# rvignav/diffusion-tts

Measured on AMD Instinct MI355X. Metric: candidate U-Net steps/sec, EDM ImageNet-64 eps-greedy N=64, higher is better.
Workload: dtype f16x3; 1 GPU; EDM ImageNet-64 (ADM 295.9M) eps-greedy search iteration, imagenet scorer, sigma step 5/18; candidates_total=64, candidates_per_gpu=64, scorer=imagenet, scorer_dtype=f16x3, denoiser_dtype=f16x3, graph_replay=True, parity_grade=True, parallelism=candidates sharded x1, 1 all-gather of rewards per step

## Files before the change

### diffusion_tts_amd/_lib.py

```python
import ctypes as C
import os

import torch

_HERE = os.path.dirname(os.path.abspath(__file__))
LIB_PATH = os.environ.get('DTS_LIB_PATH') or os.path.join(_HERE, 'libdts_hip.so')

DTS_F32, DTS_BF16, DTS_F16, DTS_F16X3 = 0, 1, 2, 3

_p, _i, _f, _d, _i64 = C.c_void_p, C.c_int, C.c_float, C.c_double, C.c_int64


class ConvArgs(C.Structure):
    _fields_ = [('x1', _p), ('c1', C.c_int32), ('x2', _p), ('c2', C.c_int32), ('w', _p), ('bias', _p),
                ('bias_nc', _p), ('ld_bias_nc', C.c_int32), ('residual', _p), ('out', _p),
                ('n', C.c_int32), ('hin', C.c_int32), ('win', C.c_int32), ('cout', C.c_int32),
                ('ksize', C.c_int32), ('up', C.c_int32), ('out_scale', C.c_float), ('dtype', C.c_int32),
                ('workspace', _p), ('workspace_bytes', C.c_int64), ('stats_out', _p), ('stats_written', C.c_int32),
                ('ev_start', _p), ('ev_stop', _p), ('gn_coef', _p), ('gn_silu', C.c_int32), ('acc_scale', C.c_float), ('out_split2', C.c_int32),
                ('skip_c', C.c_int32), ('skip_x', _p), ('skip_w', _p), ('skip_acc_scale', C.c_float), ('skip_up', C.c_int32)]


class ConvPlanInfo(C.Structure):
    _fields_ = [(f, C.c_int32) for f in ('kernel', 'tile', 'waves', 'stages', 'pf', 'gn', 'sk', 'dbg', 'splits', 'ks_per_split', 'n_ct', 'n_pt', 'nblk',
                                         'threads', 'lds_bytes', 'stats_in_kernel', 'stats_in_reduce', 'stats_written', 'epi_rows', 'fuses_gn',
                                         'folds_skip', 'refused', 'phases')]


SIGNATURES = {
    'dts_nchw_to_nhwc': [_p, _p, _i, _i, _i, _i, _i, _p],
    'dts_nhwc_to_nchw': [_p, _i, _p, _i, _i, _i, _i, _p],
    'dts_nchw_to_nhwc_pad': [_p, _p, _i, _i, _i, _i, _i, _i, _p],
    'dts_pack_conv_weight': [_p, _p, _i, _i, _i, _i, _i, _p, _p],
    'dts_conv2d': [C.POINTER(ConvArgs), _p],
    'dts_conv_in3': [_p, _p, _p, _p, _i, _i, _i, _i, _i, _p],
    'dts_conv_out3': [_p, _i, _p, _p, _p, _i, _i, _i, _i, _p],
    'dts_gn_coef': [_p, _i, _p, _i, _i, _i, _i, _i, _f, _p, _p, _p, _i, _p, _p, _p],
    'dts_gn_coef_strips': [_p, _i, _p, _i, _i, _i, _i, _i, _f, _p, _p, _p, _i, _p, _p],
    'dts_gn_apply': [_p, _i, _p, _i, _i, _p, _p, _i, _i, _i, _i, _i, _p],
    'dts_gn_apply_x3': [_p, _i, _p, _i, _p, _p, _p, _i, _i, _i, _i, _i, _p],
    'dts_gn_fused': [_p, _i, _p, _i, _i, _i, _i, _i, _f, _p, _p, _p, _i, _p, _i, _p],
    'dts_resample2x': [_p, _p, _i, _i, _i, _i, _i, _i, _p],
    'dts_resample_fir': [_p, _p, _i, _i, _i, _i, _i, _i, _i, _p],
    'dts_space_to_depth2': [_p, _i, _p, _i, _i, _i, _i, _i, _i, _i, _p],
    'dts_attention': [_p, _p, _i, _i, _i, _i, _i, _f, _p],
    'dts_attention_masked': [_p, _p, _i, _i, _i, _i, _i, _f, _i, _p, _p],
    'dts_cross_attention': [_p, _p, _p, _i, _p, _i, _i, _i, _i, _i, _i, _f, _p],
    'dts_layer_norm': [_p, _p, _i, _i64, _i, _f, _p, _p, _p],
    'dts_geglu': [_p, _p, _i, _i64, _i, _p],
    'dts_group_rows': [_p, _i, _i64, _p, _p, _p, _p, _p],
    'dts_patchify': [_p, _p, _i, _i, _i, _i, _i, _p],
    'dts_vit_tokens': [_p, _p, _p, _p, _i, _i, _i, _i, _p],
    'dts_text_tokens': [_p, _p, _p, _p, _i, _i, _i, _i, _i, _p],
    'dts_gelu': [_p, _p, _i, _i64, _i, _p],
    'dts_vit_head': [_p, _p, _i, _i, _i, _i, _f, _p, _p, _p],
    'dts_layer_norm_x3': [_p, _p, _p, _i64, _i, _f, _p, _p, _p],
    'dts_gelu_x3': [_p, _p, _i64, _i, _i, _p],
    'dts_patchify_x3': [_p, _p, _i, _i, _i, _i, _p],
    'dts_vit_tokens_f32': [_p, _p, _p, _p, _i, _i, _i, _p],
    'dts_vit_head_f32': [_p, _p, _i, _i, _i, _f, _p, _p, _p],
    'dts_linear': [_p, _i, _p, _p, _p, _i, _i, _i, _i, _i, _i, _i, _p],
    'dts_pos_embedding': [_p, _p, _p, _i, _i, _i, _p],
    'dts_edm_precond_in': [_p, _p, _i, _f, _p, _p, _i, _i, _p],
    'dts_edm_precond_out': [_p, _p, _p, _p, _i, _i, _p],
    'dts_split3_f16': [_p, _i, _p, _i, _p, _i64, _p],
    'dts_split2_f16': [_p, _i, _p, _i64, _p],
    'dts_attention_x3': [_p, _p, _i, _i, _i, _i, _i, _f, _p],
    'dts_cast_from_f32': [_p, _p, _i, _i64, _p],
    'dts_cast_to_f32': [_p, _i, _p, _i64, _p],
    'dts_heun_xhat': [_p, _i, _i, _p, _i, _d, _p, _i, _i, _p],
    'dts_heun_euler': [_p, _p, _d, _d, _p, _p, _i64, _p],
    'dts_heun_correct': [_p, _p, _p, _d, _d, _p, _i64, _p],
    'dts_quantize_u8': [_p, _i, _p, _i64, _p],
    'dts_brightness': [_p, _p, _i, _i, _p],
    'dts_u8_to_unit_f32': [_p, _p, _i64, _p],
    'dts_resample_u8': [_p, _p, _i, _i, _i, _i, _i, _p, _p, _i, _p],
    'dts_lut_u8_f32': [_p, _p, _p, _i, _i, _i, _p],
    'dts_jpeg_size': [_p, _p, _i, _i, _i, _p, _p, _i64, _p, _p],
    'dts_cosine_rows': [_p, _p, _i, _p, _i, _i, _p],
    'dts_attnpool_tokens': [_p, _p, _p, _i, _i, _i, _i, _p],
    'dts_take_token': [_p, _i, _p, _i, _i, _i, _i, _p],
    'dts_softmax_gather': [_p, _p, _p, _i, _i, _p],
    'dts_candidate_noise': [_p, _p, _p, _p, _p, _i, _i, _i, _p],
    'dts_candidate_noise_sd': [_p, _p, _p, _p, _p, _i, _i, _i64, _p],
    'dts_cfg_combine': [_p, _p, _f, _p, _i, _i64, _p],
    'dts_ddim_candidates': [_p, _p, _p, _p, _p, _i, _f, _f, _f, _i, _i64, _p],
}
OTHER = {'dts_version': ([], _i), 'dts_conv_fuses_gn': ([C.POINTER(ConvArgs)], _i), 'dts_conv_kernel': ([C.POINTER(ConvArgs)], _i), 'dts_conv_folds_skip': ([C.POINTER(ConvArgs)], _i), 'dts_conv_takes_phases': ([C.POINTER(ConvArgs)], _i), 'dts_conv_plan': ([C.POINTER(ConvArgs), C.POINTER(ConvPlanInfo)], _i), 'dts_set_tuning': ([_i, _i], _i), 'dts_get_tuning': ([_i], _i), 'dts_last_error': ([], C.c_char_p), 'dts_gn_ws_floats': ([_i, _i], _i64),
         'dts_jpeg_workspace_bytes': ([_i, _i, _i], _i64)}

_lib = None
ABI_VERSION = 120


def load():
    global _lib
    if _lib is not None:
        return _lib
    if not os.path.exists(LIB_PATH):
        raise RuntimeError(f'{LIB_PATH} not found: the HIP extension is required (no CPU fallback). '
                           f'Build it with `python -m diffusion_tts_amd.build` or __graft_entry__.build().')
    lib = C.CDLL(LIB_PATH)
    for name, argt in SIGNATURES.items():
        fn = getattr(lib, name)
        fn.argtypes, fn.restype = argt, _i
    for name, (argt, rest) in OTHER.items():
        fn = getattr(lib, name)
        fn.argtypes, fn.restype = argt, rest
    got = lib.dts_version()
    if got != ABI_VERSION or C.sizeof(ConvArgs) != 208:
        raise RuntimeError(f'{LIB_PATH} has ABI version {got}, this binding needs {ABI_VERSION}: rebuild with `python -m diffusion_tts_amd.build --force`')
    _lib = lib
    return lib


def check(status, what=''):
    if status != 0:
        msg = load().dts_last_error().decode(errors='replace')
        raise RuntimeError(f'libdts_hip {what} failed ({status}): {msg}')


KNOBS = {'att_xcd': 0, 'att_qt': 1, 'conv_tile': 2, 'conv_splits': 3, 'conv_variant': 4, 'gn_fuse': 5, 'att_db': 6, 'conv_stages': 7, 'conv_waves': 8, 'conv_half_round': 9, 'conv_epi32': 10, 'conv_skip_fold': 11, 'conv_up_phases': 12}


def set_tuning(name, value):
    check(load().dts_set_tuning(KNOBS[name], int(value)), 'dts_set_tuning')
```

### diffusion_tts_amd/classifier.py

```python
import math
from typing import Dict

import torch

from . import ops
from .config import ClassifierConfig, ClsLayer, classifier_layers


def _qkv_perm_legacy(heads: int, d: int) -> torch.Tensor:
    s, h, c = torch.meshgrid(torch.arange(3), torch.arange(heads), torch.arange(d), indexing='ij')
    return (h * 3 * d + s * d + c).reshape(-1).to(torch.int32)


class _P:
    pass


class EncoderUNetModel:
    def __init__(self, cfg: ClassifierConfig, state_dict: Dict[str, torch.Tensor], device='cuda', dtype=ops.F16X3):
        if not torch.cuda.is_available():
            raise RuntimeError('EncoderUNetModel (HIP) needs a GPU: there is no CPU fallback in this package')
        self.cfg, self.device, self.dtype = cfg, torch.device(device), dtype
        self.act_dtype = ops.act_dtype(dtype)
        self.x3 = dtype == ops.F16X3
        from .graphs import GraphCache
        self._graphs = GraphCache(self._device_forward)
        f = lambda t: t.detach().to(self.device, torch.float32).contiguous()
        sd, dt = state_dict, dtype
        mc = cfg.model_channels
        half = mc // 2
        self.freqs = torch.exp(-math.log(10000) * torch.arange(0, half, dtype=torch.float32) / half).to(self.device)
        self.te0_w, self.te0_b = f(sd['time_embed.0.weight']), f(sd['time_embed.0.bias'])
        self.te2_w, self.te2_b = f(sd['time_embed.2.weight']), f(sd['time_embed.2.bias'])
        self.layers, self.ch, self.res = classifier_layers(cfg)
        self.params: Dict[str, _P] = {}
        emb_w, emb_b, off = [], [], 0
        hc = cfg.num_head_channels
        for L in self.layers:
            P, p = _P(), L.prefix
            if L.kind == 'conv_in':
                P.w, P.b = f(sd[f'{p}.weight']), f(sd[f'{p}.bias'])
            elif L.kind == 'res':
                P.g0, P.b0 = f(sd[f'{p}.in_layers.0.weight']), f(sd[f'{p}.in_layers.0.bias'])
                P.w0, P.cb0 = ops.pack_conv_weight(f(sd[f'{p}.in_layers.2.weight']), dt), f(sd[f'{p}.in_layers.2.bias'])
                emb_w.append(sd[f'{p}.emb_layers.1.weight'])
                emb_b.append(sd[f'{p}.emb_layers.1.bias'])
                P.off, off = off, off + 2 * L.cout
                P.g1, P.b1 = f(sd[f'{p}.out_layers.0.weight']), f(sd[f'{p}.out_layers.0.bias'])
                P.w1, P.cb1 = ops.pack_conv_weight(f(sd[f'{p}.out_layers.3.weight']), dt), f(sd[f'{p}.out_layers.3.bias'])
                P.sw = P.sb = None
                if L.cin != L.cout:
                    P.sw, P.sb = ops.pack_conv_weight(f(sd[f'{p}.skip_connection.weight']), dt), f(sd[f'{p}.skip_connection.bias'])
                    P.cb1_skip = (P.cb1 + P.sb).contiguous()
            else:
                heads = L.cin // hc
                perm = _qkv_perm_legacy(heads, hc).to(self.device)
                P.g, P.b = f(sd[f'{p}.norm.weight']), f(sd[f'{p}.norm.bias'])
                P.wqkv = ops.pack_conv_weight(f(sd[f'{p}.qkv.weight']), dt, out_perm=perm)
                P.bqkv = f(sd[f'{p}.qkv.bias'])[perm.long()].contiguous()
                P.wproj, P.bproj = ops.pack_conv_weight(f(sd[f'{p}.proj_out.weight']), dt), f(sd[f'{p}.proj_out.bias'])
                P.heads = heads
            self.params[p] = P
        self.emb_w = ops.pack_conv_weight(f(torch.cat(emb_w, 0))[:, :, None, None].contiguous(), dt)
        self.emb_b = f(torch.cat(emb_b, 0))
        self.emb_total = off
        self.out_g, self.out_b = f(sd['out.0.weight']), f(sd['out.0.bias'])
        self.pos = f(sd['out.2.positional_embedding'])
        self.pool_wqkv = ops.pack_conv_weight(f(sd['out.2.qkv_proj.weight']), dt)
        self.pool_bqkv = f(sd['out.2.qkv_proj.bias'])
        self.cproj_w = f(sd['out.2.c_proj.weight']).reshape(cfg.out_channels, self.ch).contiguous()
        self.cproj_b = f(sd['out.2.c_proj.bias'])
        torch.cuda.synchronize(self.device)

    def _res(self, L: ClsLayer, x, emb_all):
        P = self.params[L.prefix]
        raw = self.x3 and P.sw is not None
        h = ops.group_norm(x, 32, 1e-5, P.g0, P.b0, silu=True, pool=L.down, split_out=self.x3, raw_split=raw)
        if raw:
            h, x = h
        elif L.down:
            x = ops.resample2x(x, up=False)
        h = ops.conv2d(h, P.w0, P.cb0, gn_stats=True)
        ss = emb_all[:, P.off:P.off + 2 * L.cout]
        h = ops.group_norm(h, 32, 1e-5, P.g1, P.b1, scale_shift=ss, silu=True, split_out=self.x3)
        if raw and ops.conv_folds_skip(h, P.w1, (x, P.sw, False)):
            return ops.conv2d(h, P.w1, P.cb1_skip, skip=(x, P.sw, False), gn_stats=True)
        sk = x if P.sw is None else ops.conv2d(x, P.sw, P.sb)
        return ops.conv2d(h, P.w1, P.cb1, residual=sk, gn_stats=True)

    def _attn(self, L: ClsLayer, x):
        P = self.params[L.prefix]
        n, hh, ww, c = x.shape
        hn = ops.group_norm(x, 32, 1e-5, P.g, P.b, silu=False, split_out=self.x3)
        fx3 = self.x3 and ops.attention_x3_ok(hh * ww, c // P.heads)
        qkv = ops.conv2d(hn, P.wqkv, P.bqkv, out_split2=fx3)
        a = ops.attention(qkv.view(n, hh * ww, 3 * c), P.heads, 1.0 / math.sqrt(c // P.heads), x3=self.x3, split_out=fx3)
        a = ops.SplitAct(a.data.view(n, hh, ww, 2 * c), c) if fx3 else a.view(n, hh, ww, c)
        return ops.conv2d(a, P.wproj, P.bproj, residual=x, gn_stats=True)

    @torch.no_grad()
    def __call__(self, x, timesteps):
        t = timesteps.to(self.device, torch.float32).contiguous()
        return self._graphs(x.to(self.device, torch.float32).contiguous(), t)

    @torch.no_grad()
    def _device_forward(self, x, t):
        n = x.shape[0]
        emb = ops.pos_embedding(t, self.freqs)
        emb = ops.linear(emb, self.te0_w, self.te0_b, act_out=True)
        emb = ops.linear(emb, self.te2_w, self.te2_b, act_out=True)
        e = ops.cast_from_f32(emb, self.act_dtype)
        emb_all = ops.conv2d(e.view(1, n, 1, -1), self.emb_w, self.emb_b).view(n, self.emb_total)
        h = None
        for L in self.layers:
            if L.kind == 'conv_in':
                P = self.params[L.prefix]
                h = ops.conv_in3(x.contiguous(), P.w, P.b, L.cout, self.act_dtype)
            elif L.kind == 'res':
                h = self._res(L, h, emb_all)
            else:
                h = self._attn(L, h)
        h = ops.group_norm(h, 32, 1e-5, self.out_g, self.out_b, silu=True)
        tok = ops.attnpool_tokens(h, self.pos)
        nt = tok.shape[1]
        qkv = ops.conv2d(tok.view(n, nt, 1, self.ch), self.pool_wqkv, self.pool_bqkv)
        heads = self.ch // self.cfg.num_head_channels
        a = ops.attention(qkv.view(n, nt, 3 * self.ch), heads, 1.0 / math.sqrt(self.cfg.num_head_channels), x3=self.x3)
        return ops.linear(ops.take_token(a, 0), self.cproj_w, self.cproj_b)
```

### diffusion_tts_amd/csrc/conv_igemm.hip

```cpp
#include "dts_common.h"
#include <hip/hip_ext.h>
#include <type_traits>

static_assert(sizeof(dts_conv_args) == 208, "dts_conv_args layout changed: bump DTS_ABI_VERSION and update the bindings (_lib.py ConvArgs)");

int dts_conv_launch_phase_form(const void* plan, const void* params, const void* call);

namespace {

struct ConvCall {
  hipStream_t st;
  hipEvent_t ev_start = nullptr, ev_stop = nullptr;
};

struct ConvP {
  const char* x1; const char* x2;
  const char* w;
  const float* bias;
  const char* bias_nc;
  const char* residual;
  char* out;
  int c1, c2, cin;
  int ld_bias_nc;
  int n, hin, win, hout, wout, cout;
  int taps;
  int up;
  int P;
  int n_ct;
  int n_pt;
  int splits;
  int ks_per_split;
  float* partial;
  float* stats;
  float out_scale;
  float acc_scale;
  int out_split2;
  int w_shift, hw_shift;
  const float* gn_coef;
  int gn_silu;
  int epi_rows;
  const char* sk_x; const char* sk_w;
  int sk_c, sk_up;
  float sk_ratio;
};

template <typename T> struct Mma;
template <> struct Mma<bf16_t> {
  static __device__ __forceinline__ void run(f32x4_t& acc, const uint4& a, const uint4& b) {
    acc = __builtin_amdgcn_mfma_f32_16x16x32_bf16(__builtin_bit_cast(bf16x8_t, a), __builtin_bit_cast(bf16x8_t, b), acc, 0, 0, 0);
  }
};
template <> struct Mma<f16_t> {
  static __device__ __forceinline__ void run(f32x4_t& acc, const uint4& a, const uint4& b) {
    acc = __builtin_amdgcn_mfma_f32_16x16x32_f16(__builtin_bit_cast(f16x8_t, a), __builtin_bit_cast(f16x8_t, b), acc, 0, 0, 0);
  }
};
template <> struct Mma<float> {
  static __device__ __forceinline__ void run(f32x4_t& acc, const uint4& a, const uint4& b) {
    acc = __builtin_amdgcn_mfma_f32_16x16x4f32(__builtin_bit_cast(float, a.x), __builtin_bit_cast(float, b.x), acc, 0, 0, 0);
    acc = __builtin_amdgcn_mfma_f32_16x16x4f32(__builtin_bit_cast(float, a.y), __builtin_bit_cast(float, b.y), acc, 0, 0, 0);
    acc = __builtin_amdgcn_mfma_f32_16x16x4f32(__builtin_bit_cast(float, a.z), __builtin_bit_cast(float, b.z), acc, 0, 0, 0);
    acc = __builtin_amdgcn_mfma_f32_16x16x4f32(__builtin_bit_cast(float, a.w), __builtin_bit_cast(float, b.w), acc, 0, 0, 0);
  }
};

__device__ __forceinline__ uint4 f16x8_mul_2m11(const uint4& v) {
  const f16x8_t h = __builtin_bit_cast(f16x8_t, v) * (_Float16)0x1p-11f;
  return __builtin_bit_cast(uint4, h);
}

template <typename T> struct Vec4;
template <> struct Vec4<float> {
  using type = float4;
  static __device__ __forceinline__ void unpack(const float4& v, float* f) { f[0] = v.x; f[1] = v.y; f[2] = v.z; f[3] = v.w; }
  static __device__ __forceinline__ float4 pack(const float* f) { return make_float4(f[0], f[1], f[2], f[3]); }
  static __device__ __forceinline__ void load(const float* p, float* f) {
    const float4 v = *reinterpret_cast<const float4*>(p);
    f[0] = v.x; f[1] = v.y; f[2] = v.z; f[3] = v.w;
  }
  static __device__ __forceinline__ void store(float* p, const float* f) {
    *reinterpret_cast<float4*>(p) = make_float4(f[0], f[1], f[2], f[3]);
  }
};
template <> struct Vec4<bf16_t> {
  using type = uint2;
  static __device__ __forceinline__ uint2 pack(const float* f) {
    return make_uint2(pack2_bf16(f[0], f[1]), pack2_bf16(f[2], f[3]));
  }
  static __device__ __forceinline__ void unpack(const uint2& v, float* f) {
    f[0] = __builtin_bit_cast(float, v.x << 16); f[1] = __builtin_bit_cast(float, v.x & 0xffff0000u);
    f[2] = __builtin_bit_cast(float, v.y << 16); f[3] = __builtin_bit_cast(float, v.y & 0xffff0000u);
  }
  static __device__ __forceinline__ void load(const bf16_t* p, float* f) {
    const uint2 v = *reinterpret_cast<const uint2*>(p);
    f[0] = bf16_bits_to_f32(v.x & 0xffffu); f[1] = bf16_bits_to_f32(v.x >> 16);
    f[2] = bf16_bits_to_f32(v.y & 0xffffu); f[3] = bf16_bits_to_f32(v.y >> 16);
  }
  static __device__ __forceinline__ void store(bf16_t* p, const float* f) {
    *reinterpret_cast<uint2*>(p) = make_uint2(pack2_bf16(f[0], f[1]), pack2_bf16(f[2], f[3]));
  }
};
template <> struct Vec4<f16_t> {
  using type = uint2;
  static __device__ __forceinline__ uint2 pack(const float* f) {
    return make_uint2(pack2_f16(f[0], f[1]), pack2_f16(f[2], f[3]));
  }
  static __device__ __forceinline__ void unpack(const uint2& v, float* f) {
    f[0] = f16_bits_to_f32(v.x & 0xffffu); f[1] = f16_bits_to_f32(v.x >> 16);
    f[2] = f16_bits_to_f32(v.y & 0xffffu); f[3] = f16_bits_to_f32(v.y >> 16);
  }
  static __device__ __forceinline__ void load(const f16_t* p, float* f) {
    const uint2 v = *reinterpret_cast<const uint2*>(p);
    f[0] = f16_bits_to_f32(v.x & 0xffffu); f[1] = f16_bits_to_f32(v.x >> 16);
    f[2] = f16_bits_to_f32(v.y & 0xffffu); f[3] = f16_bits_to_f32(v.y >> 16);
  }
  static __device__ __forceinline__ void store(f16_t* p, const float* f) {
    *reinterpret_cast<uint2*>(p) = make_uint2(pack2_f16(f[0], f[1]), pack2_f16(f[2], f[3]));
  }
};

#ifdef DTS_STAMPS
__device__ unsigned long long g_stamps[8192 * 8];
#define DTS_STAMP(slot_)                                                                                       \
  if (threadIdx.x == 0 && (blockIdx.x + blockIdx.y * gridDim.x) < 8192) {                                       \
    unsigned long long t_;                                                                                      \
    asm volatile("s_memtime %0\n\ts_waitcnt lgkmcnt(0)" : "=s"(t_)::"memory");                                 \
    g_stamps[(blockIdx.x + blockIdx.y * gridDim.x) * 8 + (slot_)] = t_;                                         \
  }
#define DTS_STAMP_RT(slot_)                                                                                    \
  if (threadIdx.x == 0 && (blockIdx.x + blockIdx.y * gridDim.x) < 8192) {                                       \
    unsigned long long t_;                                                                                      \
    asm volatile("s_memrealtime %0\n\ts_waitcnt lgkmcnt(0)" : "=s"(t_)::"memory");                             \
    g_stamps[(blockIdx.x + blockIdx.y * gridDim.x) * 8 + (slot_)] = t_;                                         \
  }
#define DTS_SEG_DECL unsigned long long seg_t_ = 0, seg_acc_[6] = {0, 0, 0, 0, 0, 0};
#define DTS_SEG_START { asm volatile("s_memtime %0\n\ts_waitcnt lgkmcnt(0)" : "=s"(seg_t_)::"memory"); }
#define DTS_SEG_MARK(i_)                                                                                       \
  {                                                                                                            \
    __builtin_amdgcn_sched_barrier(0);                                                                         \
    unsigned long long n_;                                                                                     \
    asm volatile("s_memtime %0\n\ts_waitcnt lgkmcnt(0)" : "=s"(n_)::"memory");                                \
    seg_acc_[i_] += n_ - seg_t_;                                                                               \
    seg_t_ = n_;                                                                                               \
    __builtin_amdgcn_sched_barrier(0);                                                                         \
  }
#define DTS_SEG_STORE                                                                                          \
  if ((threadIdx.x & 255) == 0 && (blockIdx.x + blockIdx.y * gridDim.x) < 4096) {                              \
    unsigned long long* d_ = g_seg + ((blockIdx.x + blockIdx.y * gridDim.x) * 2 + (threadIdx.x >> 8)) * 8;     \
    for (int i_ = 0; i_ < 6; ++i_) d_[i_] = seg_acc_[i_];                                                      \
  }
__device__ unsigned long long g_seg[4096 * 2 * 8];
#else
#define DTS_STAMP(slot_)
#define DTS_STAMP_RT(slot_)
#define DTS_SEG_DECL
#define DTS_SEG_START
#define DTS_SEG_MARK(i_)
#define DTS_SEG_STORE
#endif

__device__ uint4 g_zero16[2048];

__device__ __forceinline__ void glds16(const char* g, uint32_t lds_off) {
  asm volatile("s_mov_b32 m0, %1\n\ts_nop 0\n\tglobal_load_lds_dwordx4 %0, off" : : "v"(g), "s"(lds_off) : "memory", "m0");
}

typedef int dts_i32x4 __attribute__((ext_vector_type(4)));
__device__ __forceinline__ dts_i32x4 make_rsrc(const void* base, uint32_t bytes) {
  const uint64_t a = (uint64_t)(uintptr_t)base;
  return dts_i32x4{(int)(uint32_t)a, (int)(uint32_t)(a >> 32), (int)bytes, 0x00020000};
}
__device__ __forceinline__ void bdma16(uint32_t voff, dts_i32x4 rsrc, uint32_t soff, uint32_t lds_off) {
  asm volatile("s_mov_b32 m0, %3\n\ts_nop 0\n\tbuffer_load_dwordx4 %0, %1, %2 offen lds"
               : : "v"(voff), "s"(rsrc), "s"(soff), "s"(lds_off) : "memory", "m0");
}
#ifndef PP_LOAD_ORDER
#define PP_LOAD_ORDER 2
#endif
constexpr uint32_t DTS_OOR = 0x80000000u;

__device__ __forceinline__ int swz(int row, int chunk) { return row * 128 + ((chunk ^ (row & 7)) << 4); }

struct TileMap {
  int pn0;
  int patch;
  int porg;
  int w;
  int strip0;
  __device__ __forceinline__ int pix(int r) const { return patch ? porg + (r >> 4) * w + (r & 15) : pn0 + r; }
  __device__ __forceinline__ int strip(int wn) const { return strip0 + wn; }
};
__device__ __forceinline__ TileMap linear_tile(int pn0) { return TileMap{pn0, 0, 0, 0, pn0 >> 6}; }

struct PhaseTileMap {
  int pn0;
  int py, px;
// ... 12 lines not shown
      y = rem / lw; x = rem - y * lw;
    }
    return n * 4 * lhw + (2 * y + py) * 2 * lw + 2 * x + px;
  }
  __device__ __forceinline__ int strip(int wn) const {
    const int S = lhw >> 6, gs = (pn0 >> 6) + wn, n = gs / S;
    return n * 4 * S + (2 * py + px) * S + (gs - n * S);
  }
};

template <int BM, int NTHR>
__device__ __forceinline__ void issue_residual_pieces(const ConvP& kp, int cm0, const TileMap& tm, uint32_t stage, int tid, int u0, int u1) {
  constexpr int CPR = BM / 8;
  const char* resb = kp.residual + (size_t)cm0 * 2;
  const size_t rstride = (size_t)kp.cout * 2;
  const uint32_t wave_dst = __builtin_amdgcn_readfirstlane(stage + (tid >> 6) * 1024);
  for (int u = u0; u < u1; ++u) {
    const int slot = u * NTHR + tid, row = slot / CPR, c = slot - row * CPR;
    glds16(resb + (size_t)tm.pix(row) * rstride + ((c ^ (row & 7)) << 4), wave_dst + u * (NTHR * 16));
  }
}

__device__ __forceinline__ float row16_sum(float v) {
  v += __builtin_bit_cast(float, __builtin_amdgcn_update_dpp(0, __builtin_bit_cast(int, v), 0xB1, 0xf, 0xf, false));
  v += __builtin_bit_cast(float, __builtin_amdgcn_update_dpp(0, __builtin_bit_cast(int, v), 0x4E, 0xf, 0xf, false));
  v += __builtin_bit_cast(float, __builtin_amdgcn_update_dpp(0, __builtin_bit_cast(int, v), 0x141, 0xf, 0xf, false));
  v += __builtin_bit_cast(float, __builtin_amdgcn_update_dpp(0, __builtin_bit_cast(int, v), 0x140, 0xf, 0xf, false));
  return v;
}
__device__ __forceinline__ void row16_sum8(float (&a)[4], float (&b)[4]) {
#define DTS_DPP_STEP(ctrl_)                                                                     \
  "v_add_f32_dpp %0, %0, %0 " ctrl_ " row_mask:0xf bank_mask:0xf\n\t"                           \
  "v_add_f32_dpp %1, %1, %1 " ctrl_ " row_mask:0xf bank_mask:0xf\n\t"                           \
  "v_add_f32_dpp %2, %2, %2 " ctrl_ " row_mask:0xf bank_mask:0xf\n\t"                           \
  "v_add_f32_dpp %3, %3, %3 " ctrl_ " row_mask:0xf bank_mask:0xf\n\t"                           \
  "v_add_f32_dpp %4, %4, %4 " ctrl_ " row_mask:0xf bank_mask:0xf\n\t"                           \
  "v_add_f32_dpp %5, %5, %5 " ctrl_ " row_mask:0xf bank_mask:0xf\n\t"                           \
  "v_add_f32_dpp %6, %6, %6 " ctrl_ " row_mask:0xf bank_mask:0xf\n\t"                           \
  "v_add_f32_dpp %7, %7, %7 " ctrl_ " row_mask:0xf bank_mask:0xf\n\t"
  asm volatile("s_nop 1\n\t"
               DTS_DPP_STEP("quad_perm:[1,0,3,2]") DTS_DPP_STEP("quad_perm:[2,3,0,1]") DTS_DPP_STEP("row_half_mirror") DTS_DPP_STEP("row_mirror")
               : "+v"(a[0]), "+v"(a[1]), "+v"(a[2]), "+v"(a[3]), "+v"(b[0]), "+v"(b[1]), "+v"(b[2]), "+v"(b[3]));
#undef DTS_DPP_STEP
}

template <typename T, int MT, int NT, int BM, int BN, bool RES, bool BNC, bool STATS, int NTHR>
__device__ __forceinline__ void conv_epilogue_fast(const ConvP& kp, f32x4_t (&acc)[MT][NT], int cm0, const TileMap& tm, int wm, int wn, int lrow,
                                                   int lq, char* smem_ring, bool bias_in_acc, int stage_off, int early_u0,
                                                   int early_u1) {
  char* smem = smem_ring + stage_off;
  using V4 = typename Vec4<T>::type;
  constexpr int ROWB = BM * 2, CPR = BM / 8, DR = NTHR / CPR, DC = NTHR - DR * CPR, ITERS = BN * CPR / NTHR;
  static_assert(BN * CPR % NTHR == 0 && CPR % 8 == 0, "staged tile trips / swizzle groups");
  const int p_cout = kp.cout;
  const int prow0 = wn * 16 * NT + lrow;
  const int col0 = wm * 16 * MT + lq * 4;
  const T* __restrict__ bnc = reinterpret_cast<const T*>(kp.bias_nc);
  const size_t rstride = (size_t)p_cout * 2;
  const int tid = threadIdx.x;
  if constexpr (RES) {
    const uint32_t stage = (uint32_t)(uintptr_t)(__attribute__((address_space(3))) char*)smem;
    issue_residual_pieces<BM, NTHR>(kp, cm0, tm, stage, tid, 0, early_u0);
    issue_residual_pieces<BM, NTHR>(kp, cm0, tm, stage, tid, early_u1, ITERS);
  }
  float4 bv[MT];
#pragma unroll
  for (int mt = 0; mt < MT; ++mt) bv[mt] = make_float4(0.f, 0.f, 0.f, 0.f);
  (void)bias_in_acc; (void)bv;
  const T* np[NT];
  if constexpr (BNC) {
    const int hw = kp.hout * kp.wout;
#pragma unroll
    for (int nt = 0; nt < NT; ++nt) {
      const int pp = tm.pix(prow0 + nt * 16);
      np[nt] = bnc + (size_t)(kp.hw_shift >= 0 ? pp >> kp.hw_shift : pp / hw) * kp.ld_bias_nc + cm0 + col0;
    }
  }
  constexpr bool want_stats = STATS && NT == 4;
  float* sp = want_stats ? kp.stats + ((size_t)tm.strip(wn) * p_cout + cm0 + col0) * 2 : nullptr;
  char* sw = smem + prow0 * ROWB + (lq & 1) * 8;
  int coff[MT];
#pragma unroll
  for (int mt = 0; mt < MT; ++mt) coff[mt] = (((wm * 2 * MT + 2 * mt + (lq >> 1)) ^ (lrow & 7)) << 4);
  const float osc = kp.out_scale;
  if constexpr (RES) {
    if (early_u0 > 0 || early_u1 < ITERS) {
      asm volatile("s_waitcnt vmcnt(0)" ::: "memory");
      __syncthreads();
    }
  }
#pragma unroll
  for (int mt = 0; mt < MT; ++mt) {
    V4 nv[NT], rv[NT];
    if constexpr (BNC) {
#pragma unroll
      for (int nt = 0; nt < NT; ++nt) nv[nt] = *reinterpret_cast<const V4*>(np[nt] + mt * 16);
    }
    if constexpr (RES) {
#pragma unroll
      for (int nt = 0; nt < NT; ++nt) rv[nt] = *reinterpret_cast<const V4*>(sw + nt * 16 * ROWB + coff[mt]);
    }
    typedef float f32x2 __attribute__((ext_vector_type(2)));
    f32x2 ssa = {0.f, 0.f}, ssb = {0.f, 0.f}, sqa = {0.f, 0.f}, sqb = {0.f, 0.f};
#pragma unroll
    for (int nt = 0; nt < NT; ++nt) {
      f32x2 va = {acc[mt][nt][0], acc[mt][nt][1]}, vb = {acc[mt][nt][2], acc[mt][nt][3]};
      if constexpr (BNC) {
        float f[4];
        Vec4<T>::unpack(nv[nt], f);
        va += f32x2{f[0], f[1]}; vb += f32x2{f[2], f[3]};
      }
      if constexpr (RES) {
        float f[4];
        Vec4<T>::unpack(rv[nt], f);
        va += f32x2{f[0], f[1]}; vb += f32x2{f[2], f[3]};
      }
      va *= osc; vb *= osc;
      const float v[4] = {va.x, va.y, vb.x, vb.y};
      const V4 pk = Vec4<T>::pack(v);
      *reinterpret_cast<V4*>(sw + nt * 16 * ROWB + coff[mt]) = pk;
      if constexpr (want_stats) {
        float f[4];
        Vec4<T>::unpack(pk, f);
        const f32x2 fa = {f[0], f[1]}, fb = {f[2], f[3]};
        ssa += fa; ssb += fb;
        sqa = __builtin_elementwise_fma(fa, fa, sqa); sqb = __builtin_elementwise_fma(fb, fb, sqb);
      }
    }
    if constexpr (want_stats) {
      float ss4[4] = {ssa.x, ssa.y, ssb.x, ssb.y}, sq4[4] = {sqa.x, sqa.y, sqb.x, sqb.y};
      row16_sum8(ss4, sq4);
      if (lrow == 0) {
        float4* d = reinterpret_cast<float4*>(sp + mt * 32);
        d[0] = make_float4(ss4[0], sq4[0], ss4[1], sq4[1]);
        d[1] = make_float4(ss4[2], sq4[2], ss4[3], sq4[3]);
      }
    }
  }
  DTS_STAMP(6);
  __syncthreads();
  DTS_STAMP(7);
  int row = tid / CPR, c = tid - row * CPR;
  char* outb = kp.out + (size_t)cm0 * 2;
  typedef unsigned int u32x4_nt __attribute__((ext_vector_type(4)));
#pragma unroll
  for (int u = 0; u < ITERS; ++u) {
    const u32x4_nt v_ = *reinterpret_cast<const u32x4_nt*>(smem + row * ROWB + c * 16);
    __builtin_nontemporal_store(v_, reinterpret_cast<u32x4_nt*>(outb + (size_t)tm.pix(row) * rstride + ((c ^ (row & 7)) << 4)));
    row += DR; c += DC;
    if (c >= CPR) { c -= CPR; ++row; }
  }
}

template <int MT, int NT, typename TM = TileMap>
__device__ __forceinline__ void conv_epilogue_rows_f32(const ConvP& kp, f32x4_t (&acc)[MT][NT], int cm0, const TM& tm, int wm, int wn,
                                                       int lrow, int lq, char* smem, int wave) {
  static_assert(NT == 4, "64-pixel wave strips");
  constexpr int CW = 16 * MT;
  constexpr int LPR = 4 * MT;
  constexpr int RPI = LPR <= 8 ? 8 : (LPR <= 16 ? 4 : 2);
  constexpr int ITERS = 32 / RPI;
  constexpr int ROWB = CW * 4 + 16;
  char* const ws = smem + (size_t)wave * (32 * ROWB);
  const int lane = threadIdx.x & 63;
  const int rsub = lane / LPR, c4 = lane - rsub * LPR;
  const bool act = rsub < RPI;
  const int p_cout = kp.cout;
  const int co = cm0 + wm * CW + c4 * 4;
  const float* __restrict__ res = reinterpret_cast<const float*>(kp.residual);
  if (tm.pix(wn * 64) >= kp.P) return;
  float4 b4 = make_float4(0.f, 0.f, 0.f, 0.f), n4 = make_float4(0.f, 0.f, 0.f, 0.f);
  if (act) {
    if (kp.bias) b4 = *reinterpret_cast<const float4*>(kp.bias + co);
    if (kp.bias_nc) {
      const int pp0 = tm.pix(wn * 64), hw = kp.hout * kp.wout;
      n4 = *reinterpret_cast<const float4*>(reinterpret_cast<const float*>(kp.bias_nc) + (size_t)(kp.hw_shift >= 0 ? pp0 >> kp.hw_shift : pp0 / hw) * kp.ld_bias_nc + co);
    }
  }
  const float asc = kp.acc_scale, osc = kp.out_scale;
  const bool want_stats = kp.stats != nullptr;
  float ss4[4] = {0.f, 0.f, 0.f, 0.f}, sq4[4] = {0.f, 0.f, 0.f, 0.f};
  typedef float f32x4_nt __attribute__((ext_vector_type(4)));
  constexpr int CH = ITERS < 8 ? ITERS : 8;
#pragma unroll
  for (int half = 0; half < 2; ++half) {
#pragma unroll
    for (int n2 = 0; n2 < 2; ++n2)
#pragma unroll
      for (int mt = 0; mt < MT; ++mt)
        *reinterpret_cast<f32x4_t*>(ws + (n2 * 16 + lrow) * ROWB + (mt * 16 + lq * 4) * 4) = acc[mt][half * 2 + n2];
#pragma unroll
   for (int u0 = 0; u0 < ITERS; u0 += CH) {
    size_t prow[CH];
    float4 rv[CH];
#pragma unroll
    for (int u = 0; u < CH; ++u) {
      prow[u] = (size_t)tm.pix(wn * 64 + half * 32 + (u0 + u) * RPI + (act ? rsub : 0)) * p_cout + co;
      rv[u] = make_float4(0.f, 0.f, 0.f, 0.f);
      if (res && act) rv[u] = *reinterpret_cast<const float4*>(res + prow[u]);
    }
#pragma unroll
    for (int u = 0; u < CH; ++u) {
      if (!act) continue;
      const f32x4_t a = *reinterpret_cast<const f32x4_t*>(ws + ((u0 + u) * RPI + rsub) * ROWB + c4 * 16);
      float v[4] = {a[0] * asc + b4.x, a[1] * asc + b4.y, a[2] * asc + b4.z, a[3] * asc + b4.w};
      if (kp.bias_nc) { v[0] += n4.x; v[1] += n4.y; v[2] += n4.z; v[3] += n4.w; }
      if (res) { v[0] += rv[u].x; v[1] += rv[u].y; v[2] += rv[u].z; v[3] += rv[u].w; }
#pragma unroll
      for (int r = 0; r < 4; ++r) v[r] *= osc;
      if (kp.out_split2) {
        float hi[4], lo[4];
#pragma unroll
        for (int r = 0; r < 4; ++r) x2_split(v[r], hi[r], lo[r]);
        const uint2 h = make_uint2(pack2_f16(hi[0], hi[1]), pack2_f16(hi[2], hi[3])), l = make_uint2(pack2_f16(lo[0], lo[1]), pack2_f16(lo[2], lo[3]));
        const bool odd = (c4 & 1) != 0;
        const uint32_t rx = (uint32_t)__builtin_amdgcn_update_dpp(0, (int)(odd ? h.x : l.x), 0xB1, 0xf, 0xf, false);
        const uint32_t ry = (uint32_t)__builtin_amdgcn_update_dpp(0, (int)(odd ? h.y : l.y), 0xB1, 0xf, 0xf, false);
        if (kp.epi_rows == 2) {
          f16_t* o8 = reinterpret_cast<f16_t*>(kp.out) + 2 * (prow[u] - co) + co;
          *reinterpret_cast<uint2*>(o8) = h;
          *reinterpret_cast<uint2*>(o8 + p_cout) = l;
          continue;
        }
        f16_t* orow = reinterpret_cast<f16_t*>(kp.out) + 2 * (prow[u] - co) + (odd ? co - 4 + p_cout : co);
        *reinterpret_cast<uint4*>(orow) = odd ? make_uint4(rx, ry, l.x, l.y) : make_uint4(h.x, h.y, rx, ry);
      } else {
        const f32x4_nt o = {v[0], v[1], v[2], v[3]};
        __builtin_nontemporal_store(o, reinterpret_cast<f32x4_nt*>(reinterpret_cast<float*>(kp.out) + prow[u]));
      }
      if (want_stats) {
#pragma unroll
        for (int r = 0; r < 4; ++r) { ss4[r] += v[r]; sq4[r] += v[r] * v[r]; }
      }
    }
   }
  }
  if (want_stats) {
#pragma unroll
    for (int r = 0; r < 4; ++r) {
      float s_ = ss4[r], q_ = sq4[r];
#pragma unroll
      for (int k = 1; k < RPI; ++k) { s_ += __shfl(ss4[r], c4 + k * LPR, 64); q_ += __shfl(sq4[r], c4 + k * LPR, 64); }
      ss4[r] = s_; sq4[r] = q_;
    }
    if (rsub == 0) {
      float4* d = reinterpret_cast<float4*>(kp.stats + ((size_t)tm.strip(wn) * p_cout + co) * 2);
      d[0] = make_float4(ss4[0], sq4[0], ss4[1], sq4[1]);
      d[1] = make_float4(ss4[2], sq4[2], ss4[3], sq4[3]);
    }
  }
}

template <typename T, int MT, int NT, int BM, int BN, int NTHR, int RING, typename TM = TileMap>
__device__ __forceinline__ void conv_epilogue(const ConvP& kp, f32x4_t (&acc)[MT][NT], int cm0, const TM& tm, int split, int wm, int wn,
                                              int lrow, int lq, char* smem, bool bias_in_acc, int stage_off, int early_u0, int early_u1) {
  const int p_P = kp.P, p_cout = kp.cout, p_hout = kp.hout, p_wout = kp.wout;
  if (kp.splits > 1) {
    float* part = kp.partial + (size_t)split * p_P * p_cout;
#pragma unroll
    for (int nt = 0; nt < NT; ++nt) {
      const int pp = tm.pix(wn * 16 * NT + nt * 16 + lrow);
      if (pp >= p_P) continue;
#pragma unroll
      for (int mt = 0; mt < MT; ++mt) {
        const int co = cm0 + wm * 16 * MT + mt * 16 + lq * 4;
        *reinterpret_cast<float4*>(part + (size_t)pp * p_cout + co) =
            make_float4(acc[mt][nt][0], acc[mt][nt][1], acc[mt][nt][2], acc[mt][nt][3]);
      }
    }
    return;
  }
  if constexpr (sizeof(T) == 4 && NT == 4) {
    constexpr int NWV = NTHR / 64;
    static_assert(NWV * 32 * (16 * MT * 4 + 16) <= RING, "the waves' private transpose slices must fit the caller's LDS ring");
    if (kp.epi_rows && (p_hout * p_wout) % 64 == 0) {
      conv_epilogue_rows_f32<MT, NT>(kp, acc, cm0, tm, wm, wn, lrow, lq, smem, (int)(threadIdx.x >> 6));
      return;
    }
  }
  if constexpr (sizeof(T) == 2) {
    if (tm.pn0 + BN <= p_P) {
      const bool r_ = kp.residual != nullptr, b_ = kp.bias_nc != nullptr, s_ = NT == 4 && kp.stats != nullptr;
#define DTS_EPI(R_, B_, S_) conv_epilogue_fast<T, MT, NT, BM, BN, R_, B_, S_, NTHR>(kp, acc, cm0, tm, wm, wn, lrow, lq, smem, bias_in_acc, stage_off, early_u0, early_u1)
      if (r_) { if (b_) { if (s_) DTS_EPI(true, true, true); else DTS_EPI(true, true, false); }
                else    { if (s_) DTS_EPI(true, false, true); else DTS_EPI(true, false, false); } }
      else    { if (b_) { if (s_) DTS_EPI(false, true, true); else DTS_EPI(false, true, false); }
                else    { if (s_) DTS_EPI(false, false, true); else DTS_EPI(false, false, false); } }
#undef DTS_EPI
      return;
    }
  }
  const T* __restrict__ res = reinterpret_cast<const T*>(kp.residual);
  const T* __restrict__ bnc = reinterpret_cast<const T*>(kp.bias_nc);
  T* __restrict__ out = reinterpret_cast<T*>(kp.out);
  const int hw = p_hout * p_wout;
  using V4 = typename Vec4<T>::type;
  int ppv[NT], nsv[NT];
#pragma unroll
  for (int nt = 0; nt < NT; ++nt) {
    const int pp = tm.pix(wn * 16 * NT + nt * 16 + lrow);
    ppv[nt] = pp < p_P ? pp : -1;
    nsv[nt] = pp < p_P ? pp / hw : 0;
  }
  constexpr int RG = (sizeof(T) == 4 && MT > 4) ? 2 : MT;
  static_assert(MT % RG == 0, "residual slice groups");
  V4 rv[RG][NT], nv[NT];
  float4 bv[MT];
#pragma unroll
  for (int mt = 0; mt < MT; ++mt)
    bv[mt] = (kp.bias && !bias_in_acc) ? *reinterpret_cast<const float4*>(kp.bias + cm0 + wm * 16 * MT + mt * 16 + lq * 4) : make_float4(0.f, 0.f, 0.f, 0.f);
  const float asc = kp.acc_scale;
  constexpr bool VIA_LDS = sizeof(T) == 2;
  constexpr int ROWP = BM * 2 + 16;
  static_assert(!VIA_LDS || BN * ROWP <= RING, "staged tile must fit the caller's LDS ring");
  const bool want_stats = NT == 4 && kp.stats != nullptr;
  float* sp = want_stats ? kp.stats + ((size_t)tm.strip(wn) * p_cout) * 2 : nullptr;
#pragma unroll
  for (int mt = 0; mt < MT; ++mt) {
    const int co = cm0 + wm * 16 * MT + mt * 16 + lq * 4;
    const float4 bcur = bv[mt];
    if (res && mt % RG == 0) {
#pragma unroll
      for (int m2 = 0; m2 < RG; ++m2) {
        const int co_ = cm0 + wm * 16 * MT + (mt + m2) * 16 + lq * 4;
#pragma unroll
        for (int nt = 0; nt < NT; ++nt)
          if (ppv[nt] >= 0) rv[m2][nt] = *reinterpret_cast<const V4*>(res + (size_t)ppv[nt] * p_cout + co_);
      }
    }
    if (bnc) {
#pragma unroll
      for (int nt = 0; nt < NT; ++nt)
        if (ppv[nt] >= 0) nv[nt] = *reinterpret_cast<const V4*>(bnc + (size_t)nsv[nt] * kp.ld_bias_nc + co);
    }
    float ss4[4] = {0.f, 0.f, 0.f, 0.f}, sq4[4] = {0.f, 0.f, 0.f, 0.f};
#pragma unroll
    for (int nt = 0; nt < NT; ++nt) {
      if (ppv[nt] < 0) continue;
      float v[4];
      v[0] = acc[mt][nt][0] * asc + bcur.x; v[1] = acc[mt][nt][1] * asc + bcur.y;
      v[2] = acc[mt][nt][2] * asc + bcur.z; v[3] = acc[mt][nt][3] * asc + bcur.w;
      if (bnc) {
        float f[4];
        Vec4<T>::unpack(nv[nt], f);
#pragma unroll
        for (int r = 0; r < 4; ++r) v[r] += f[r];
      }
      if (res) {
        float f[4];
        Vec4<T>::unpack(rv[mt % RG][nt], f);
#pragma unroll
        for (int r = 0; r < 4; ++r) v[r] += f[r];
      }
#pragma unroll
      for (int r = 0; r < 4; ++r) v[r] *= kp.out_scale;
      const V4 pk = Vec4<T>::pack(v);
      if constexpr (VIA_LDS)
        *reinterpret_cast<V4*>(smem + (wn * 16 * NT + nt * 16 + lrow) * ROWP + (wm * 16 * MT + mt * 16 + lq * 4) * 2) = pk;
      else if (sizeof(T) == 4 && kp.out_split2) {
        float hi[4], lo[4];
#pragma unroll
        for (int r = 0; r < 4; ++r) x2_split(v[r], hi[r], lo[r]);
        f16_t* orow = reinterpret_cast<f16_t*>(kp.out) + (size_t)ppv[nt] * 2 * p_cout + co;
        *reinterpret_cast<uint2*>(orow) = make_uint2(pack2_f16(hi[0], hi[1]), pack2_f16(hi[2], hi[3]));
        *reinterpret_cast<uint2*>(orow + p_cout) = make_uint2(pack2_f16(lo[0], lo[1]), pack2_f16(lo[2], lo[3]));
      } else
        *reinterpret_cast<V4*>(out + (size_t)ppv[nt] * p_cout + co) = pk;
      if (want_stats) {
        float f[4];
        Vec4<T>::unpack(pk, f);
#pragma unroll
        for (int r = 0; r < 4; ++r) { ss4[r] += f[r]; sq4[r] += f[r] * f[r]; }
      }
    }
    if (want_stats) {
#pragma unroll
      for (int r = 0; r < 4; ++r) {
#pragma unroll
        for (int o = 1; o < 16; o <<= 1) { ss4[r] += __shfl_xor(ss4[r], o, 64); sq4[r] += __shfl_xor(sq4[r], o, 64); }
      }
      if (lrow == 0 && tm.pix(wn * 64) < p_P) {
        float4* d = reinterpret_cast<float4*>(sp + (size_t)co * 2);
        d[0] = make_float4(ss4[0], sq4[0], ss4[1], sq4[1]);
        d[1] = make_float4(ss4[2], sq4[2], ss4[3], sq4[3]);
      }
    }
  }
  if constexpr (VIA_LDS) {
// ... 838 lines not shown
  const int dev = current_device();
  if (!attr_done[dev]) {
    (void)hipFuncSetAttribute(reinterpret_cast<const void*>(KERNEL), hipFuncAttributeMaxDynamicSharedMemorySize, pl.lds_bytes);
    attr_done[dev] = true;
  }
  const dim3 grid(pl.nblk, pl.splits), block(pl.threads);
  if (call.ev_start != nullptr && call.ev_stop != nullptr)
    hipExtLaunchKernelGGL(KERNEL, grid, block, (size_t)pl.lds_bytes, call.st, call.ev_start, call.ev_stop, 0, q);
  else
    hipLaunchKernelGGL(KERNEL, grid, block, (size_t)pl.lds_bytes, call.st, q);
  DTS_CHECK_LAUNCH(pl.kernel != 0 ? "dts_conv2d(ping-pong)" : "dts_conv2d");
  return DTS_OK;
}

template <typename T, typename OT, int MT, int WM, int WN, bool PF, bool PH = false>
int conv_launch_igemm(const ConvPlan& pl, const ConvP& q, const ConvCall& call) {
#define DTS_IGEMM(MT_, WM_, STAGES_) conv_launch<&conv_igemm_kernel<T, MT_, 4, WM_, WN, PF, STAGES_, OT, PH>>(pl, q, call)
  if constexpr (sizeof(T) == 2) {
    if (pl.waves == 8) return pl.stages == 3 ? DTS_IGEMM(MT / 2, WM * 2, 3) : DTS_IGEMM(MT / 2, WM * 2, 2);
    if (pl.stages == 3) return DTS_IGEMM(MT, WM, 3);
    if constexpr (std::is_same<T, OT>::value)
      if (pl.stages == 4) return DTS_IGEMM(MT, WM, 4);
  }
  return DTS_IGEMM(MT, WM, 2);
#undef DTS_IGEMM
}

int igemm_splits(int nblk, int nk, double slab, bool can8, bool x3, bool ws, long long ws_bytes, int forced) {
  const int slots = 512;
  int splits = 1;
  if (ws && nblk < (slots * 3) / 4 && nk >= 16) {
    int smax = 8;
    if (smax > nk / 8) smax = nk / 8;
    while (smax > 1 && (long long)smax * (long long)slab > ws_bytes) --smax;
    if (smax < 1) smax = 1;
    const double KS = x3 ? 1.5 : 1.0;
    auto est = [&](int s_) {
      const int steps = (nk + s_ - 1) / s_;
      double t;
      if (can8 && (long long)nblk * s_ <= 256) t = 5.0 + steps * 0.75 * KS;
      else t = (double)((nblk * s_ + slots - 1) / slots) * (5.5 + steps * 1.25 * KS);
      if (s_ > 1) t += 3.0 + (s_ + 0.5) * slab / 4.0e6;
      return t;
    };
    int best = 1;
    for (int s_ = 2; s_ <= smax; ++s_)
      if (est(s_) < est(best)) best = s_;
    splits = best;
  }
  const int f8 = forced > 8 ? 8 : forced;
  if (f8 > 0 && ws && nk >= 2 * f8 && (long long)f8 * (long long)slab <= ws_bytes) splits = f8;
  return splits;
}

inline bool pp_considers_split(long long nblk) { return nblk < 192; }

int pp_splits(int nblk, int nk, double slab, bool x3, bool ws, long long ws_bytes, int forced) {
  int splits = 1;
  if (!ws || nk < 16) return splits;
  if (forced > 0) splits = forced;
  else if (pp_considers_split(nblk)) {
    const int nchunk = nk / 9;
    double best = 1e30;
    for (int s_ = 1; s_ <= 8 && s_ <= nchunk; ++s_) {
      const int cps = (nchunk + s_ - 1) / s_, se = (nchunk + cps - 1) / cps;
      if (se != s_ || nblk * se > 256) continue;
      double t = 5.0 + cps * 9 * (x3 ? 1.4 : 1.05);
      if (se > 1) t += 3.0 + (se + 0.5) * slab / 4.0e6;
      if (t < best) { best = t; splits = se; }
    }
  }
  if (splits > 8) splits = 8;
  if (forced > 0 && splits > nk / 8) splits = nk / 8;
  if (splits > nk / 9) splits = nk / 9;
  while (splits > 1 && (long long)splits * (long long)slab > ws_bytes) --splits;
  if (splits < 1) splits = 1;
  return splits;
}

bool conv_pp_eligible(int dtype, int ksize, int cout, int c1, int c2, int n, int hin, int win, int up) {
  const int ho = up ? 2 * hin : hin, wo = up ? 2 * win : win;
  const long long P = (long long)n * ho * wo;
  return dtype != DTS_F32 && cout % 192 == 0 && ho == wo && wo >= 16 && (wo & (wo - 1)) == 0 && P % 256 == 0 && P < (1ll << 30) &&
         (long long)n * hin * win * (c1 > c2 ? c1 : c2) * 2 < (1ll << 31) && (long long)cout * ksize * ksize * (c1 + c2) * 2 < (1ll << 31) &&
         (c1 % 64 == 0) && (c2 % 64 == 0);
}

int conv_pick_pp(const ConvKnobs& k, bool f32, const ConvP& p, bool x3) {
  if (f32 || k.variant == 0 || k.tile > 0) return 0;
  if (p.taps != 9) return 0;
  const int mt = p.cout % 192 == 0 ? 6 : (p.cout % 128 == 0 ? 4 : 0);
  if (mt == 0 || !conv_pp_eligible(DTS_BF16, 3, 192, p.c1, p.c2, p.n, p.hin, p.win, p.up)) return 0;
  if ((long long)p.cout * p.taps * p.cin * 2 >= (1ll << 31)) return 0;
  if (p.gn_coef != nullptr) return (mt == 6 && !p.up) ? 6 : 0;
  if (k.variant >= 1) return mt;
  const long long blocks_pp = (long long)(p.cout / (32 * mt)) * ((p.P + 255) / 256);
  const bool short_small = blocks_pp <= 128 && p.taps * (p.cin / 64) <= 27;
  const bool half_round_128 = mt == 4 && blocks_pp > 64 && blocks_pp <= 128 && p.wout >= 32 && p.cout <= 256 && (x3 ? k.half_round == 1 : k.half_round != 0);
  const bool auto_pp = !short_small && !half_round_128;
  return (auto_pp && blocks_pp >= 64) ? mt : 0;
}

int conv_pp_dbg(int variant) {
  if (variant <= 1) return 0;
#ifdef DTS_DIAG_KERNELS
  const int d = variant / 10;
  return (variant % 10 == 1 && d >= 1 && d <= 9 && d != 3) ? d : 0;
#else
  return -1;
#endif
}

template <typename T, typename OT = T>
int conv_launch_plan(const ConvPlan& pl, const ConvP& q, const ConvCall& call) {
  if constexpr (sizeof(T) == 2) {
#define DTS_PP(DBG_, GN_, MT_, SK_) conv_launch<&conv_pp_kernel<T, 9, DBG_, GN_, MT_, OT, SK_>>(pl, q, call)
    if constexpr (!std::is_same<T, OT>::value) {
      if (pl.phases) return dts_conv_launch_phase_form(&pl, &q, &call);
      if (pl.kernel == 6 && pl.sk) return DTS_PP(0, false, 6, true);
      if (pl.kernel == 4 && pl.sk) return DTS_PP(0, false, 4, true);
    } else if (pl.kernel == 6) {
      if (pl.gn) return DTS_PP(0, true, 6, false);
#ifdef DTS_DIAG_KERNELS
      switch (pl.dbg) {
        case 1: return DTS_PP(1, false, 6, false);
        case 2: return DTS_PP(2, false, 6, false);
        case 4: return DTS_PP(4, false, 6, false);
        case 5: return DTS_PP(5, false, 6, false);
        case 6: return DTS_PP(6, false, 6, false);
        case 7: return DTS_PP(7, false, 6, false);
        case 8: return DTS_PP(8, false, 6, false);
        case 9: return DTS_PP(9, false, 6, false);
      }
#endif
    }
    if (pl.kernel == 6) return DTS_PP(0, false, 6, false);
    if (pl.kernel == 4) return DTS_PP(0, false, 4, false);
#undef DTS_PP
  }
  switch (pl.tile) {
    case 192: return pl.pf ? conv_launch_igemm<T, OT, 6, 2, 2, true>(pl, q, call) : conv_launch_igemm<T, OT, 6, 2, 2, false>(pl, q, call);
    case 128: return pl.pf ? conv_launch_igemm<T, OT, 4, 2, 2, true>(pl, q, call) : conv_launch_igemm<T, OT, 4, 2, 2, false>(pl, q, call);
    default: return pl.pf ? conv_launch_igemm<T, OT, 4, 1, 4, true>(pl, q, call) : conv_launch_igemm<T, OT, 4, 1, 4, false>(pl, q, call);
  }
}

void conv_shape_from_args(const dts_conv_args* a, ConvP& p) {
  p.c1 = a->c1; p.c2 = a->c2; p.cin = a->c1 + a->c2;
  p.n = a->n; p.hin = a->hin; p.win = a->win;
  p.hout = a->up ? 2 * a->hin : a->hin; p.wout = a->up ? 2 * a->win : a->win;
  p.cout = a->cout; p.taps = a->ksize * a->ksize; p.up = a->up;
  p.P = (int)((long long)p.n * p.hout * p.wout);
  p.residual = (const char*)a->residual; p.gn_coef = a->gn_coef;
  p.out_split2 = a->out_split2;
}

ConvPlan conv_plan(const dts_conv_args* a) {
  ConvPlan pl{};
  pl.kernel = -1; pl.splits = 1;
  auto refuse = [&](const char* fmt, int v0 = 0, int v1 = 0, int v2 = 0) { pl.refused = 1; snprintf(pl.refuse, sizeof(pl.refuse), fmt, v0, v1, v2); return pl; };
  if (a == nullptr) return refuse("dts_conv2d: null args");
  const ConvKnobs k = conv_knobs();
  const bool f32 = a->dtype == DTS_F32, x3 = a->dtype == DTS_F16X3;
  pl.fuses_gn = a->ksize == 3 && k.variant != 0 && k.tile <= 0 && !a->up &&
                conv_pp_eligible(a->dtype, a->ksize, a->cout, a->c1, a->c2, a->n, a->hin, a->win, a->up) &&
                (k.variant == 1 || (long long)(a->cout / 192) * (((long long)a->n * a->hin * a->win + 255) / 256) >= 64);
  if (a->ksize != 1 && a->ksize != 3) return refuse("dts_conv2d: ksize %d", a->ksize);
  if (a->n <= 0 || a->hin <= 0 || a->win <= 0) return refuse("dts_conv2d: bad shape");
  if (a->cout <= 0) return refuse("dts_conv2d: cout %d must be a multiple of 64", a->cout);
  if ((long long)a->n * a->hin * a->win * (a->up ? 4 : 1) >= (1ll << 30)) return refuse("dts_conv2d: too many pixels");
  ConvP p;
  conv_shape_from_args(a, p);
  const bool ph = a->up == 2;
  if (ph) p.taps = 4;
  const int mt = ph ? 0 : conv_pick_pp(k, f32, p, x3);
  pl.kernel = mt;
  int unit = 1;
  if (mt != 0) {
    pl.n_ct = p.cout / (32 * mt); pl.n_pt = (p.P + 255) / 256;
    pl.threads = 512;
    pl.lds_bytes = (6 * 16 * mt + 2 * 328) * 128;
    unit = 9;
  } else {
    pl.tile = (p.cout % 192 == 0) ? 192 : (p.cout % 128 == 0 ? 128 : 64);
    if (f32 && pl.tile == 192 && !k.f32_tile192) pl.tile = (p.cout % 128 == 0) ? 128 : 64;
    if (k.tile > 0 && p.cout % k.tile == 0) pl.tile = (k.tile == 192 || k.tile == 128) ? k.tile : 64;
    pl.n_ct = p.cout / pl.tile; pl.n_pt = (p.P + (pl.tile == 64 ? 255 : 127)) / (pl.tile == 64 ? 256 : 128);
    if (ph) pl.n_pt = (p.P / 4 + 127) / 128;
    pl.pf = a->ksize == 3 && !f32;
  }
  pl.nblk = pl.n_ct * pl.n_pt * (ph ? 4 : 1);
  const int bke = f32 ? 32 : 64, nk = p.taps * (p.cin / bke);
  pl.gn = a->gn_coef != nullptr;
  {
    const int su = a->skip_up ? 1 : 0;
    pl.folds_skip = x3 && mt != 0 && !a->up && a->residual == nullptr && !a->out_split2 && a->gn_coef == nullptr &&
                    a->skip_c > 0 && a->skip_c % 64 == 0 && k.skip_fold != 0 && k.splits <= 0 && !(su && ((a->hin | a->win) & 1)) &&
                    (!pp_considers_split(pl.nblk) || k.variant == 1) &&
                    (long long)a->n * (a->hin >> su) * (a->win >> su) * a->skip_c * 2 < (1ll << 31) && (long long)a->cout * a->skip_c * 2 < (1ll << 31);
  }
  if (a->cout % 64 != 0) return refuse("dts_conv2d: cout %d must be a multiple of 64", a->cout);
  if (a->c1 <= 0 || a->c1 % bke != 0 || a->c2 % bke != 0) return refuse("dts_conv2d: channels (%d,%d) must be multiples of %d", a->c1, a->c2, bke);
  if ((long long)p.cin * (f32 ? 4 : 2) + 128 > (long long)sizeof(g_zero16))
    return refuse("dts_conv2d: %d input channels exceed the zero-row page (%d bytes)", p.cin, (int)sizeof(g_zero16));
  if (p.hout >= 32768 || p.wout >= 32768) return refuse("dts_conv2d: spatial size too large");
  if (a->out_split2 && !(x3 && a->stats_out == nullptr)) return refuse("dts_conv2d: out_split2 is the split-precision mode's, without strip statistics");
  if (a->acc_scale != 0.f && a->acc_scale != 1.f && !x3) return refuse("dts_conv2d: acc_scale is the split-precision mode's (DTS_F16X3)");
  if (pl.gn && !pl.fuses_gn) return refuse("dts_conv2d: gn_coef given for a launch that cannot fuse the GroupNorm apply (ask dts_conv_fuses_gn first)");
  if (a->skip_c != 0 || a->skip_w != nullptr || a->skip_x != nullptr) {
    if (a->skip_w == nullptr || a->skip_x == nullptr || !pl.folds_skip)
      return refuse("dts_conv2d: skip_* given for a launch that cannot fold the 1x1 skip convolution (ask dts_conv_folds_skip first)");
    pl.sk = true;
  }
  if (pl.gn && x3) return refuse("dts_conv2d: gn_coef is not available in the split-precision mode");
  if (a->dtype < DTS_F32 || a->dtype > DTS_F16X3) return refuse("bad dtype %d", a->dtype);
  if (ph) {
    if (!x3) return refuse("dts_conv2d: up = 2 (phase-packed weights) is the split-precision mode's (DTS_F16X3), dtype %d", a->dtype);
    if (a->ksize != 3) return refuse("dts_conv2d: up = 2 needs ksize 3, got %d", a->ksize);
    if (a->c2 != 0 || a->x2 != nullptr) return refuse("dts_conv2d: up = 2 takes no second input");
    if (a->gn_coef != nullptr || pl.sk || a->out_split2) return refuse("dts_conv2d: up = 2 takes no gn_coef, skip_* or out_split2");
    if (pl.tile == 64) return refuse("dts_conv2d: up = 2 needs cout %d to be a multiple of 128 or 192", a->cout);
    if (a->stats_out != nullptr && (a->hin * a->win) % 64 != 0)
      return refuse("dts_conv2d: up = 2 with strip statistics needs hin*win = %d to be a multiple of 64 (a wave's strip is 64 low-resolution pixels)", a->hin * a->win);
    if (k.up_phases == 0) return refuse("dts_conv2d: up = 2 while DTS_CONV_UP_PHASES=0");
  }
  if (mt == 6 && !x3 && !pl.gn) {
    pl.dbg = conv_pp_dbg(k.variant);
    if (pl.dbg < 0) return refuse("dts_conv2d: DTS_CONV_VARIANT=%d selects a diagnostic kernel that this library was built without (-DDTS_DIAG_KERNELS)", k.variant);
  }
  const bool ws = a->workspace != nullptr && !a->out_split2 && !pl.sk;
  const double slab = (double)p.P * p.cout * 4.0;
  pl.splits = mt != 0 ? pp_splits(pl.nblk, nk, slab, x3, ws, (long long)a->workspace_bytes, k.splits)
                      : igemm_splits(pl.nblk, nk, slab, !f32, x3, ws, (long long)a->workspace_bytes, k.splits);
  {
    const int nunit = nk / unit, per = (nunit + pl.splits - 1) / pl.splits;
    pl.ks_per_split = per * unit;
    pl.splits = (nunit + per - 1) / per;
  }
  if (ph) {
    if (pl.splits > 1) return refuse("dts_conv2d: up = 2 with a K split of %d (the phase form takes none: use the fused-gather route)", pl.splits);
    pl.phases = 1;
  }
  pl.stats_in_kernel = a->stats_out != nullptr && pl.splits == 1;
  pl.stats_in_reduce = a->stats_out != nullptr && pl.splits > 1 && (p.hout * p.wout) % 64 == 0 && p.cout % 4 == 0;
  pl.stats_written = pl.stats_in_kernel || pl.stats_in_reduce;
  pl.epi_rows = k.epi32 < 0 ? (x3 ? 1 : 0) : (k.epi32 == 2 ? 2 : (k.epi32 != 0));
  if (ph && (a->hin * a->win) % 64 != 0) pl.epi_rows = 0;
  if (mt != 0) return pl;
  const bool one_per_cu = (long long)pl.nblk * pl.splits <= 256;
  pl.stages = (one_per_cu && pl.ks_per_split >= 3) ? 3 : 2;
  if (k.stages >= 2 && k.stages <= 4) pl.stages = k.stages;
  if (f32) pl.stages = 2;
  const int stage_bytes = (pl.tile + (pl.tile == 64 ? 256 : 128)) * 128;
  if (pl.stages * stage_bytes > 160 * 1024) pl.stages = 3;
  pl.waves = (!f32 && (k.waves == 8 || (k.waves != 4 && one_per_cu))) ? 8 : 4;
  if (pl.stages == 4 && (pl.waves == 8 || x3)) pl.stages = 3;
  pl.threads = 64 * pl.waves;
  pl.lds_bytes = pl.stages * stage_bytes;
  return pl;
}

}

#ifdef DTS_CONV_PHASE_TU
int dts_conv_launch_phase_form(const void* plan, const void* params, const void* call) {
  const ConvPlan& pl = *static_cast<const ConvPlan*>(plan);
  const ConvP& q = *static_cast<const ConvP*>(params);
  const ConvCall& c = *static_cast<const ConvCall*>(call);
  return pl.tile == 192 ? conv_launch_igemm<f16_t, float, 6, 2, 2, true, true>(pl, q, c) : conv_launch_igemm<f16_t, float, 4, 2, 2, true, true>(pl, q, c);
}
#else

#ifdef DTS_STAMPS
extern "C" int dts_debug_read_stamps(unsigned long long* host, int count) {
  return (int)hipMemcpyFromSymbol(host, HIP_SYMBOL(g_stamps), sizeof(unsigned long long) * (size_t)count);
}
extern "C" int dts_debug_clear_stamps(void) {
  void* p = nullptr;
  if (hipGetSymbolAddress(&p, HIP_SYMBOL(g_stamps)) != hipSuccess) return -1;
  if (hipMemset(p, 0, sizeof(g_stamps)) != hipSuccess) return -1;
  if (hipGetSymbolAddress(&p, HIP_SYMBOL(g_seg)) != hipSuccess) return -1;
  return (int)hipMemset(p, 0, sizeof(g_seg));
}
extern "C" int dts_debug_read_segments(unsigned long long* host, int count) {
  return (int)hipMemcpyFromSymbol(host, HIP_SYMBOL(g_seg), sizeof(unsigned long long) * (size_t)count);
}
#endif

extern "C" int dts_conv_kernel(const dts_conv_args* a) { return conv_plan(a).kernel; }

extern "C" int dts_conv_fuses_gn(const dts_conv_args* a) { return conv_plan(a).fuses_gn ? 1 : 0; }

extern "C" int dts_conv_folds_skip(const dts_conv_args* a) { return conv_plan(a).folds_skip ? 1 : 0; }

extern "C" int dts_conv_takes_phases(const dts_conv_args* a) {
  if (a == nullptr || a->up != 2) return 0;
  const ConvPlan pl = conv_plan(a);
  return (!pl.refused && pl.phases) ? 1 : 0;
}

extern "C" int dts_conv_plan(const dts_conv_args* a, dts_conv_plan_info* out) {
  DTS_CHECK_ARG(out != nullptr, "dts_conv_plan: null output");
  const ConvPlan pl = conv_plan(a);
  *out = pl;
  if (pl.refused) dts_set_error("%s", pl.refuse);
  return pl.kernel < 0 ? DTS_ERR_ARG : DTS_OK;
}

extern "C" int dts_conv2d(dts_conv_args* a, dts_stream s) {
  const ConvPlan pl = conv_plan(a);
  DTS_CHECK_ARG(!pl.refused, "%s", pl.refuse);
  DTS_CHECK_ARG(a->x1 && a->w && a->out, "dts_conv2d: null tensor");
  DTS_CHECK_ARG(a->c2 == 0 || a->x2 != nullptr, "dts_conv2d: c2 without x2");
  DTS_CHECK_ARG(a->bias_nc == nullptr || a->ld_bias_nc >= a->cout, "dts_conv2d: ld_bias_nc");
  ConvP p;
  conv_shape_from_args(a, p);
  if (pl.phases) p.taps = 4;
  DTS_CHECK_ARG(a->stats_out == nullptr || ((p.hout * p.wout) % 64 == 0 && (uintptr_t)a->stats_out % 16 == 0),
                "dts_conv2d: strip statistics need hout*wout to be a multiple of 64 and a 16-byte aligned buffer");
  DTS_CHECK_ARG(a->workspace == nullptr || ((uintptr_t)a->workspace % 16 == 0 && a->workspace_bytes >= 0), "dts_conv2d: workspace");
  p.x1 = (const char*)a->x1; p.x2 = (const char*)a->x2; p.w = (const char*)a->w;
  p.bias = a->bias; p.bias_nc = (const char*)a->bias_nc; p.out = (char*)a->out;
  p.ld_bias_nc = a->ld_bias_nc;
  p.out_scale = a->out_scale; p.acc_scale = a->acc_scale == 0.f ? 1.f : a->acc_scale;
  p.w_shift = p.hw_shift = -1;
  {
    const int hw = p.hout * p.wout;
    if ((p.wout & (p.wout - 1)) == 0 && (hw & (hw - 1)) == 0) { p.w_shift = __builtin_ctz(p.wout); p.hw_shift = __builtin_ctz(hw); }
  }
  p.gn_silu = a->gn_silu;
  p.sk_x = p.sk_w = nullptr; p.sk_c = p.sk_up = 0; p.sk_ratio = 1.f;
  if (pl.sk) {
    const float ss = a->skip_acc_scale == 0.f ? 1.f : a->skip_acc_scale;
    p.sk_x = (const char*)a->skip_x; p.sk_w = (const char*)a->skip_w; p.sk_c = a->skip_c; p.sk_up = a->skip_up ? 1 : 0;
    p.sk_ratio = p.acc_scale / ss; p.acc_scale = ss;
  }
  p.n_ct = pl.n_ct; p.n_pt = pl.n_pt; p.splits = pl.splits; p.ks_per_split = pl.ks_per_split; p.epi_rows = pl.epi_rows;
  p.partial = (float*)a->workspace;
  p.stats = pl.stats_in_kernel ? a->stats_out : nullptr;
  ConvCall call;
  call.st = to_stream(s); call.ev_start = (hipEvent_t)a->ev_start; call.ev_stop = (hipEvent_t)a->ev_stop;
  int rc = DTS_OK;
  if (a->dtype == DTS_F16X3) rc = conv_launch_plan<f16_t, float>(pl, p, call);
  else DTS_DISPATCH_DTYPE(a->dtype, rc = conv_launch_plan<T>(pl, p, call));
  if (rc == DTS_OK && pl.splits > 1) {
    if (pl.stats_in_reduce) p.stats = a->stats_out;
    DTS_DISPATCH_DTYPE(a->dtype == DTS_F16X3 ? DTS_F32 : a->dtype, rc = launch_reduce<T>(p, pl.stats_in_reduce, call.st));
  }
  a->stats_written = pl.stats_written ? 1 : 0;
  return rc;
}
#endif
```

### diffusion_tts_amd/csrc/conv_small.hip

```cpp
#include "dts_common.h"
#include <type_traits>

namespace {

template <typename T>
__global__ __launch_bounds__(256) void conv_in3_kernel(const float* __restrict__ x, const float* __restrict__ w,
                                                        const float* __restrict__ bias, T* __restrict__ out, int n_total, int h,
                                                        int wd, int cout) {
  constexpr int EPV = ET<T>::EPV;
  extern __shared__ float sw[];
  for (int i = threadIdx.x; i < 27 * cout; i += blockDim.x) {
    const int co = i / 27, k = i - co * 27;
    sw[k * cout + co] = w[i];
  }
  for (int i = threadIdx.x; i < cout; i += blockDim.x) sw[27 * cout + i] = bias ? bias[i] : 0.f;
  __syncthreads();
  const int nchunk = cout / EPV;
  const long long npix = (long long)n_total * h * wd;
  constexpr int GRP = 8;
  char* stage = reinterpret_cast<char*>(sw + 28 * cout);
  for (long long pbase = (long long)blockIdx.x * 256; pbase < npix; pbase += (long long)gridDim.x * 256) {
    const long long pix0 = pbase + threadIdx.x;
    const bool live = pix0 < npix;
    long long pix = live ? pix0 : 0;
    const int xo = (int)(pix % wd); pix /= wd;
    const int yo = (int)(pix % h);
    const int n = (int)(pix / h);
    float in[27];
#pragma unroll
    for (int ci = 0; ci < 3; ++ci)
#pragma unroll
      for (int kh = 0; kh < 3; ++kh)
#pragma unroll
        for (int kw = 0; kw < 3; ++kw) {
          const int yy = yo + kh - 1, xx = xo + kw - 1;
          float v = 0.f;
          if (live && (unsigned)yy < (unsigned)h && (unsigned)xx < (unsigned)wd) v = x[(((size_t)n * 3 + ci) * h + yy) * wd + xx];
          in[ci * 9 + kh * 3 + kw] = v;
        }
    for (int c0 = 0; c0 < nchunk; c0 += GRP) {
      __syncthreads();
#pragma unroll
      for (int g = 0; g < GRP; ++g) {
        const int chunk = c0 + g;
        if (chunk >= nchunk) break;
        float acc[EPV];
#pragma unroll
        for (int e = 0; e < EPV; ++e) acc[e] = sw[27 * cout + chunk * EPV + e];
#pragma unroll
        for (int k = 0; k < 27; ++k) {
          const float* wr = sw + k * cout + chunk * EPV;
#pragma unroll
          for (int e = 0; e < EPV; ++e) acc[e] += in[k] * wr[e];
        }
        *reinterpret_cast<uint4*>(stage + threadIdx.x * (GRP * 16) + (((g + threadIdx.x) % GRP) << 4)) = pack16<T>(acc);
      }
      __syncthreads();
      const int ng = min(GRP, nchunk - c0);
      for (int t = threadIdx.x; t < 256 * ng; t += 256) {
        const int pl = t / ng, g = t - pl * ng;
        const long long pg = pbase + pl;
        if (pg < npix)
          *reinterpret_cast<uint4*>(out + (size_t)pg * cout + (size_t)(c0 + g) * EPV) =
              *reinterpret_cast<const uint4*>(stage + pl * (GRP * 16) + (((g + pl) % GRP) << 4));
      }
    }
  }
}

template <typename T, int NT>
__global__ __launch_bounds__(256) void conv_in3_mfma_kernel(const float* __restrict__ x, const float* __restrict__ w,
                                                             const float* __restrict__ bias, T* __restrict__ out, int nseg, int h,
                                                             int wd) {
  constexpr int ES = sizeof(T) == 4 ? 4 : 2;
  constexpr int COUT = NT * 16, ROWB = COUT * ES + 16, TG = 4;
  static_assert(NT % TG == 0, "tile groups");
  __shared__ __attribute__((aligned(16))) char stage_all[4 * 16 * ROWB];
  const int lane = threadIdx.x & 63, wave = threadIdx.x >> 6, p = lane & 15, kq = lane >> 4;
  char* stage = stage_all + wave * 16 * ROWB;
  float a[NT][7];
  int dci[7], dy[7], dx[7];
#pragma unroll
  for (int s = 0; s < 7; ++s) {
    const int k = 4 * s + kq;
    const int kk = k < 27 ? k : 0;
    dci[s] = k < 27 ? kk / 9 : -1;
    dy[s] = (kk % 9) / 3 - 1;
    dx[s] = kk % 3 - 1;
#pragma unroll
    for (int t = 0; t < NT; ++t) a[t][s] = k < 27 ? w[(16 * t + p) * 27 + k] : 0.f;
  }
  f32x4_t b0[NT];
#pragma unroll
  for (int t = 0; t < NT; ++t) {
    const float4 q = bias ? *reinterpret_cast<const float4*>(bias + 16 * t + 4 * kq) : make_float4(0.f, 0.f, 0.f, 0.f);
    b0[t][0] = q.x; b0[t][1] = q.y; b0[t][2] = q.z; b0[t][3] = q.w;
  }
  const int spr = wd >> 4;
  const size_t plane = (size_t)h * wd;
  for (int seg = blockIdx.x * 4 + wave; seg < nseg; seg += gridDim.x * 4) {
    const int xs = seg % spr, rest = seg / spr;
    const int y = rest % h, n = rest / h;
    float bv[7];
#pragma unroll
    for (int s = 0; s < 7; ++s) {
      const int yy = y + dy[s], xx = xs * 16 + p + dx[s];
      const bool ok = dci[s] >= 0 && (unsigned)yy < (unsigned)h && (unsigned)xx < (unsigned)wd;
      const size_t idx = ok ? ((size_t)n * 3 + dci[s]) * plane + (size_t)yy * wd + xx : 0;
      const float v = x[idx];
      bv[s] = ok ? v : 0.f;
    }
#pragma unroll
    for (int t0 = 0; t0 < NT; t0 += TG) {
      f32x4_t acc[TG];
#pragma unroll
      for (int u = 0; u < TG; ++u) acc[u] = b0[t0 + u];
#pragma unroll
      for (int s = 0; s < 7; ++s)
#pragma unroll
        for (int u = 0; u < TG; ++u) acc[u] = __builtin_amdgcn_mfma_f32_16x16x4f32(a[t0 + u][s], bv[s], acc[u], 0, 0, 0);
#pragma unroll
      for (int u = 0; u < TG; ++u) {
        if constexpr (std::is_same<T, float>::value) {
          *reinterpret_cast<f32x4_t*>(stage + p * ROWB + (16 * (t0 + u) + 4 * kq) * 4) = acc[u];
        } else {
          uint2 o;
          if (std::is_same<T, bf16_t>::value) { o.x = pack2_bf16(acc[u][0], acc[u][1]); o.y = pack2_bf16(acc[u][2], acc[u][3]); }
          else { o.x = pack2_f16(acc[u][0], acc[u][1]); o.y = pack2_f16(acc[u][2], acc[u][3]); }
          *reinterpret_cast<uint2*>(stage + p * ROWB + (16 * (t0 + u) + 4 * kq) * 2) = o;
        }
      }
    }
    char* dst = reinterpret_cast<char*>(out + (size_t)seg * 16 * COUT);
#pragma unroll
    for (int c = lane; c < COUT * ES; c += 64) {
      const int px = c / (COUT * ES / 16), ch = c - px * (COUT * ES / 16);
      *reinterpret_cast<uint4*>(dst + (size_t)c * 16) = *reinterpret_cast<const uint4*>(stage + px * ROWB + ch * 16);
    }
  }
}

template <typename T>
__global__ __launch_bounds__(256) void conv_out3_kernel(const T* __restrict__ x, const float* __restrict__ w,
                                                         const float* __restrict__ bias, float* __restrict__ out, int n_total, int h,
                                                         int wd, int c) {
  constexpr int EPV = ET<T>::EPV;
  extern __shared__ float sw[];
  for (int i = threadIdx.x; i < 27 * c; i += blockDim.x) sw[i] = w[i];
  __syncthreads();
  const int nchunk = c / EPV;
  const long long npix = (long long)n_total * h * wd;
  const int sub = threadIdx.x & 3;
  for (long long pix0 = ((long long)blockIdx.x * blockDim.x + threadIdx.x) >> 2; pix0 < ((npix + 63) / 64) * 64;
       pix0 += ((long long)gridDim.x * blockDim.x) >> 2) {
    const bool valid = pix0 < npix;
    long long pix = valid ? pix0 : 0;
    const int xo = (int)(pix % wd); pix /= wd;
    const int yo = (int)(pix % h);
    const int n = (int)(pix / h);
    float a0 = 0.f, a1 = 0.f, a2 = 0.f;
    if (valid) {
      for (int kh = 0; kh < 3; ++kh) {
        const int yy = yo + kh - 1;
        if ((unsigned)yy >= (unsigned)h) continue;
        for (int kw = 0; kw < 3; ++kw) {
          const int xx = xo + kw - 1;
          if ((unsigned)xx >= (unsigned)wd) continue;
          const T* row = x + (((size_t)n * h + yy) * wd + xx) * c;
          const float* w0 = sw + (kh * 3 + kw) * c;
          for (int ch = sub; ch < nchunk; ch += 4) {
            const uint4 v = *reinterpret_cast<const uint4*>(row + ch * EPV);
            float f[EPV];
            unpack16<T>(v, f);
#pragma unroll
            for (int e = 0; e < EPV; ++e) {
              a0 += f[e] * w0[ch * EPV + e];
              a1 += f[e] * w0[9 * c + ch * EPV + e];
              a2 += f[e] * w0[18 * c + ch * EPV + e];
            }
          }
        }
      }
    }
    a0 += __shfl_xor(a0, 1, 64); a0 += __shfl_xor(a0, 2, 64);
    a1 += __shfl_xor(a1, 1, 64); a1 += __shfl_xor(a1, 2, 64);
    a2 += __shfl_xor(a2, 1, 64); a2 += __shfl_xor(a2, 2, 64);
    if (valid && sub == 0) {
      const size_t hw = (size_t)h * wd;
      float* o = out + (size_t)n * 3 * hw + (size_t)yo * wd + xo;
      o[0] = a0 + (bias ? bias[0] : 0.f);
      o[hw] = a1 + (bias ? bias[1] : 0.f);
      o[2 * hw] = a2 + (bias ? bias[2] : 0.f);
    }
  }
}

template <typename T>
__global__ __launch_bounds__(256) void conv_out3_tiled_kernel(const T* __restrict__ x, const float* __restrict__ w, const float* __restrict__ bias,
                                                               float* __restrict__ out, int h, int wd, int c) {
  constexpr int EPV = ET<T>::EPV, VPC = 4, CC = VPC * EPV;
  static_assert(CC == VPC * EPV, "chunk = 4 vectors");
  constexpr int PITCH = VPC * 16 + 16;
  __shared__ __attribute__((aligned(16))) char halo[18 * 18 * PITCH];
  const int tpr = wd >> 4, tin = blockIdx.x % (tpr * (h >> 4)), n = blockIdx.x / (tpr * (h >> 4));
  const int y0 = (tin / tpr) << 4, x0 = (tin % tpr) << 4;
  const int ty = threadIdx.x >> 4, tx = threadIdx.x & 15;
  float a0 = 0.f, a1 = 0.f, a2 = 0.f;
  for (int c0 = 0; c0 < c; c0 += CC) {
    __syncthreads();
    for (int i = threadIdx.x; i < 18 * 18 * VPC; i += 256) {
      const int hp = i / VPC, v = i - hp * VPC;
      const int hy = hp / 18, hx = hp - hy * 18;
      const int yy = y0 + hy - 1, xx = x0 + hx - 1;
      uint4 val = make_uint4(0, 0, 0, 0);
      if ((unsigned)yy < (unsigned)h && (unsigned)xx < (unsigned)wd)
        val = *reinterpret_cast<const uint4*>(x + (((size_t)n * h + yy) * wd + xx) * c + c0 + v * EPV);
      *reinterpret_cast<uint4*>(halo + hp * PITCH + v * 16) = val;
    }
    __syncthreads();
#pragma unroll
    for (int kh = 0; kh < 3; ++kh)
#pragma unroll
      for (int kw = 0; kw < 3; ++kw) {
        const char* hp = halo + ((ty + kh) * 18 + tx + kw) * PITCH;
        const float* w0 = w + (size_t)(kh * 3 + kw) * c + c0;
#pragma unroll
        for (int v = 0; v < VPC; ++v) {
          float f[EPV];
          unpack16<T>(*reinterpret_cast<const uint4*>(hp + v * 16), f);
#pragma unroll
          for (int e = 0; e < EPV; ++e) {
            a0 += f[e] * w0[v * EPV + e];
            a1 += f[e] * w0[(size_t)9 * c + v * EPV + e];
            a2 += f[e] * w0[(size_t)18 * c + v * EPV + e];
          }
        }
      }
  }
  const size_t hw = (size_t)h * wd;
  float* o = out + (size_t)n * 3 * hw + (size_t)(y0 + ty) * wd + x0 + tx;
  o[0] = a0 + (bias ? bias[0] : 0.f);
  o[hw] = a1 + (bias ? bias[1] : 0.f);
  o[2 * hw] = a2 + (bias ? bias[2] : 0.f);
}

}

extern "C" int dts_conv_in3(const float* x, const float* w, const float* bias, void* out, int dtype, int n, int h, int w_, int cout,
                            dts_stream s) {
  DTS_CHECK_ARG(x && w && out, "dts_conv_in3: null pointer");
  DTS_CHECK_ARG(n > 0 && h > 0 && w_ > 0 && cout % 8 == 0 && cout <= 512, "dts_conv_in3: bad shape (cout=%d)", cout);
  hipStream_t st = to_stream(s);
  const long long nseg = (long long)n * h * (w_ / 16);
  if (w_ % 16 == 0 && (cout == 192 || cout == 128 || cout == 64) && nseg < (1ll << 31) &&
      (bias == nullptr || ((uintptr_t)bias & 15) == 0)) {
    long long spw = nseg / 2048;
    if (spw < 1) spw = 1;
    if (spw > 8) spw = 8;
    long long g = (nseg + 4 * spw - 1) / (4 * spw);
    if (g > 2048) g = 2048;
#define DTS_IN3_MFMA(TT, NT_)                                                                                                    \
  hipLaunchKernelGGL((conv_in3_mfma_kernel<TT, NT_>), dim3((int)g), dim3(256), 0, st, x, w, bias, (TT*)out, (int)nseg, h, w_)
    if (dtype == DTS_BF16) {
      if (cout == 192) DTS_IN3_MFMA(bf16_t, 12); else if (cout == 128) DTS_IN3_MFMA(bf16_t, 8); else DTS_IN3_MFMA(bf16_t, 4);
    } else if (dtype == DTS_F32) {
      if (cout == 192) DTS_IN3_MFMA(float, 12); else if (cout == 128) DTS_IN3_MFMA(float, 8); else DTS_IN3_MFMA(float, 4);
    } else {
      if (cout == 192) DTS_IN3_MFMA(f16_t, 12); else if (cout == 128) DTS_IN3_MFMA(f16_t, 8); else DTS_IN3_MFMA(f16_t, 4);
    }
#undef DTS_IN3_MFMA
    DTS_CHECK_LAUNCH("dts_conv_in3");
    return DTS_OK;
  }
  DTS_DISPATCH_DTYPE(dtype, {
    const long long total = (long long)n * h * w_;
    long long g = (total + 255) / 256;
    if (g > 4096) g = 4096;
    hipLaunchKernelGGL((conv_in3_kernel<T>), dim3((int)g), dim3(256), 28 * cout * sizeof(float) + 256 * 8 * 16, st, x, w, bias, (T*)out, n,
                       h, w_, cout);
    DTS_CHECK_LAUNCH("dts_conv_in3");
  });
  return DTS_OK;
}

extern "C" int dts_conv_out3(const void* x, int dtype, const float* w, const float* bias, float* out, int n, int h, int w_, int c,
                             dts_stream s) {
  DTS_CHECK_ARG(x && w && out, "dts_conv_out3: null pointer");
  DTS_CHECK_ARG(n > 0 && h > 0 && w_ > 0 && c % 8 == 0 && 27 * c * 4 <= 64 * 1024, "dts_conv_out3: bad shape (c=%d)", c);
  hipStream_t st = to_stream(s);
  if (h % 16 == 0 && w_ % 16 == 0 && c % (dtype == DTS_F32 ? 16 : 32) == 0 && (long long)n * (h / 16) * (w_ / 16) < (1ll << 31)) {
    DTS_DISPATCH_DTYPE(dtype, {
      hipLaunchKernelGGL((conv_out3_tiled_kernel<T>), dim3((unsigned)(n * (h / 16) * (w_ / 16))), dim3(256), 0, st, (const T*)x, w, bias, out, h, w_, c);
      DTS_CHECK_LAUNCH("dts_conv_out3");
    });
    return DTS_OK;
  }
  DTS_DISPATCH_DTYPE(dtype, {
    const long long total = (long long)n * h * w_ * 4;
    long long g = (total + 255) / 256;
    if (g > 8192) g = 8192;
    hipLaunchKernelGGL((conv_out3_kernel<T>), dim3((int)g), dim3(256), 27 * c * sizeof(float), st, (const T*)x, w, bias, out, n, h,
                       w_, c);
    DTS_CHECK_LAUNCH("dts_conv_out3");
  });
  return DTS_OK;
}
```

### diffusion_tts_amd/csrc/dts_common.h

```cpp
#pragma once
#include <hip/hip_runtime.h>
#include <stdint.h>
#include <stdio.h>
#include "../../include/dts.h"

typedef __attribute__((ext_vector_type(8))) __bf16 bf16x8_t;
typedef __attribute__((ext_vector_type(8))) _Float16 f16x8_t;
typedef __attribute__((ext_vector_type(4))) float f32x4_t;
typedef __attribute__((ext_vector_type(4))) short s16x4_t;

struct bf16_t { uint16_t v; };
struct f16_t { uint16_t v; };

void dts_set_error(const char* fmt, ...);

#define DTS_CHECK_ARG(cond, ...)                 \
  do {                                           \
    if (!(cond)) {                               \
      dts_set_error(__VA_ARGS__);                \
      return DTS_ERR_ARG;                        \
    }                                            \
  } while (0)

#define DTS_CHECK_LAUNCH(what)                                              \
  do {                                                                      \
    hipError_t e__ = hipGetLastError();                                     \
    if (e__ != hipSuccess) {                                                \
      dts_set_error("%s: launch failed: %s", what, hipGetErrorString(e__)); \
      return DTS_ERR_LAUNCH;                                                \
    }                                                                       \
  } while (0)

static inline hipStream_t to_stream(dts_stream s) { return reinterpret_cast<hipStream_t>(s); }

enum dts_knob {
  DTS_KNOB_ATT_XCD = 0,
  DTS_KNOB_ATT_QT = 1,
  DTS_KNOB_CONV_TILE = 2,
  DTS_KNOB_CONV_SPLITS = 3,
  DTS_KNOB_CONV_VARIANT = 4,
  DTS_KNOB_GN_FUSE = 5,
  DTS_KNOB_ATT_DB = 6,
  DTS_KNOB_CONV_STAGES = 7,
  DTS_KNOB_CONV_WAVES = 8,
  DTS_KNOB_CONV_HALF_ROUND = 9,
  DTS_KNOB_CONV_EPI32 = 10,
  DTS_KNOB_CONV_SKIP_FOLD = 11,
  DTS_KNOB_CONV_UP_PHASES = 12,
  DTS_KNOB_COUNT = 16
};
int dts_knob_get(int knob);

template <typename T> struct ET;
template <> struct ET<float> {
  static constexpr int EPV = 4;
  static constexpr int DT = DTS_F32;
};
template <> struct ET<bf16_t> {
  static constexpr int EPV = 8;
  static constexpr int DT = DTS_BF16;
};
template <> struct ET<f16_t> {
  static constexpr int EPV = 8;
  static constexpr int DT = DTS_F16;
};

__device__ __forceinline__ float bf16_bits_to_f32(uint32_t b) { return __builtin_bit_cast(float, b << 16); }
__device__ __forceinline__ uint32_t f32_to_bf16_bits(float f) {
  __bf16 h = (__bf16)f;
  return (uint32_t)__builtin_bit_cast(uint16_t, h);
}
typedef __bf16 dts_bf16x2_t __attribute__((ext_vector_type(2)));
typedef _Float16 dts_f16x2_t __attribute__((ext_vector_type(2)));
typedef float dts_f32x2_t __attribute__((ext_vector_type(2)));
__device__ __forceinline__ uint32_t pack2_bf16(float lo, float hi) {
  const dts_f32x2_t v = {lo, hi};
  return __builtin_bit_cast(uint32_t, __builtin_convertvector(v, dts_bf16x2_t));
}
__device__ __forceinline__ uint32_t pack2_f16(float lo, float hi) {
  const dts_f32x2_t v = {lo, hi};
  return __builtin_bit_cast(uint32_t, __builtin_convertvector(v, dts_f16x2_t));
}
__device__ __forceinline__ float f16_bits_to_f32(uint32_t b) {
  return (float)__builtin_bit_cast(_Float16, (uint16_t)b);
}
__device__ __forceinline__ uint32_t f32_to_f16_bits(float f) {
  _Float16 h = (_Float16)f;
  return (uint32_t)__builtin_bit_cast(uint16_t, h);
}

__device__ __forceinline__ void x3_split(float x, float& hi, float& lo) {
  if (fabsf(x) > 65504.0f) x = copysignf(65504.0f, x);
  float h = (float)(_Float16)x;
  if (fabsf(h) < 6.103515625e-05f) h = 0.f;
  hi = h;
  lo = (x - h) * 2048.0f;
}
__device__ __forceinline__ int x3_off(int c) { return ((c >> 5) << 6) + (c & 31); }
__device__ __forceinline__ void x2_split(float x, float& hi, float& lo) {
  float y = x * 64.0f;
  if (fabsf(y) > 65504.0f) y = copysignf(65504.0f, y);
  hi = (float)(_Float16)y;
  lo = y - hi;
}

template <typename T> __device__ __forceinline__ float ld1(const T* p);
template <> __device__ __forceinline__ float ld1<float>(const float* p) { return *p; }
template <> __device__ __forceinline__ float ld1<bf16_t>(const bf16_t* p) { return bf16_bits_to_f32(p->v); }
template <> __device__ __forceinline__ float ld1<f16_t>(const f16_t* p) { return f16_bits_to_f32(p->v); }
template <typename T> __device__ __forceinline__ void st1(T* p, float f);
template <> __device__ __forceinline__ void st1<float>(float* p, float f) { *p = f; }
template <> __device__ __forceinline__ void st1<bf16_t>(bf16_t* p, float f) { p->v = (uint16_t)f32_to_bf16_bits(f); }
template <> __device__ __forceinline__ void st1<f16_t>(f16_t* p, float f) { p->v = (uint16_t)f32_to_f16_bits(f); }

template <typename T> __device__ __forceinline__ void unpack16(const uint4& v, float* f);
template <> __device__ __forceinline__ void unpack16<float>(const uint4& v, float* f) {
  f[0] = __builtin_bit_cast(float, v.x); f[1] = __builtin_bit_cast(float, v.y);
  f[2] = __builtin_bit_cast(float, v.z); f[3] = __builtin_bit_cast(float, v.w);
}
template <> __device__ __forceinline__ void unpack16<bf16_t>(const uint4& v, float* f) {
  f[0] = bf16_bits_to_f32(v.x & 0xffffu); f[1] = bf16_bits_to_f32(v.x >> 16);
  f[2] = bf16_bits_to_f32(v.y & 0xffffu); f[3] = bf16_bits_to_f32(v.y >> 16);
  f[4] = bf16_bits_to_f32(v.z & 0xffffu); f[5] = bf16_bits_to_f32(v.z >> 16);
  f[6] = bf16_bits_to_f32(v.w & 0xffffu); f[7] = bf16_bits_to_f32(v.w >> 16);
}
template <> __device__ __forceinline__ void unpack16<f16_t>(const uint4& v, float* f) {
  f[0] = f16_bits_to_f32(v.x & 0xffffu); f[1] = f16_bits_to_f32(v.x >> 16);
  f[2] = f16_bits_to_f32(v.y & 0xffffu); f[3] = f16_bits_to_f32(v.y >> 16);
  f[4] = f16_bits_to_f32(v.z & 0xffffu); f[5] = f16_bits_to_f32(v.z >> 16);
  f[6] = f16_bits_to_f32(v.w & 0xffffu); f[7] = f16_bits_to_f32(v.w >> 16);
}
template <typename T> __device__ __forceinline__ uint4 pack16(const float* f);
template <> __device__ __forceinline__ uint4 pack16<float>(const float* f) {
  return make_uint4(__builtin_bit_cast(uint32_t, f[0]), __builtin_bit_cast(uint32_t, f[1]),
                    __builtin_bit_cast(uint32_t, f[2]), __builtin_bit_cast(uint32_t, f[3]));
}
template <> __device__ __forceinline__ uint4 pack16<bf16_t>(const float* f) {
  return make_uint4(pack2_bf16(f[0], f[1]), pack2_bf16(f[2], f[3]), pack2_bf16(f[4], f[5]), pack2_bf16(f[6], f[7]));
}
template <> __device__ __forceinline__ uint4 pack16<f16_t>(const float* f) {
  return make_uint4(pack2_f16(f[0], f[1]), pack2_f16(f[2], f[3]), pack2_f16(f[4], f[5]), pack2_f16(f[6], f[7]));
}

__device__ __forceinline__ float silu_f(float x) { return x / (1.0f + __expf(-x)); }

template <typename F> __device__ __forceinline__ F wave_sum(F v) {
#pragma unroll
  for (int o = 32; o > 0; o >>= 1) v += __shfl_xor(v, o, 64);
  return v;
}

#define DTS_DISPATCH_DTYPE(dtype, ...)                                   \
  switch (dtype) {                                                       \
    case DTS_F32: { using T = float; __VA_ARGS__; } break;               \
    case DTS_BF16: { using T = bf16_t; __VA_ARGS__; } break;             \
    case DTS_F16: { using T = f16_t; __VA_ARGS__; } break;               \
    default: dts_set_error("bad dtype %d", (int)(dtype)); return DTS_ERR_ARG; \
  }
```

### diffusion_tts_amd/csrc/groupnorm.hip

```cpp
#include "dts_common.h"

namespace {

constexpr int GN_SPLITS = 32;

template <typename T>
__global__ __launch_bounds__(256) void gn_partial_kernel(const T* __restrict__ x1, int c1, const T* __restrict__ x2, int c2,
                                                          int hw, int groups, int splits, float* __restrict__ partial) {
  constexpr int EPV = ET<T>::EPV;
  extern __shared__ float sm[];
  const int C = c1 + c2, cg = C / groups;
  const int nchunk = C / EPV;
  const int slots = nchunk < 256 ? nchunk : 256;
  const int planes = 256 / slots;
  const int n = blockIdx.y, split = blockIdx.x;
  const int per = (hw + splits - 1) / splits;
  const int p0 = split * per, p1 = min(hw, p0 + per);
  const int tid = threadIdx.x;
  const int plane = tid / slots, slot = tid - plane * slots;
  if (plane < planes) {
    for (int chunk = slot; chunk < nchunk; chunk += slots) {
      float s[EPV], ss[EPV];
#pragma unroll
      for (int e = 0; e < EPV; ++e) s[e] = ss[e] = 0.f;
// ... 208 lines not shown
#pragma unroll
    for (int e = 0; e < EPV; ++e) { const float y0 = f0[e] * A[e] + B[e]; f0[e] = silu ? silu_t<T>(y0) : y0; }
    if constexpr (SPLIT) DTS_STORE_SPLIT(dst3 + (size_t)p * 2 * C, f0)
    else *reinterpret_cast<uint4*>(dst + (size_t)p * C) = pack16<T>(f0);
  }
}
#undef DTS_STORE_SPLIT

template <typename T, bool POOL, bool SPLIT = false>
__global__ __launch_bounds__(256) void gn_apply_kernel(const T* __restrict__ x1, int c1, const T* __restrict__ x2, int c2,
                                                        const float* __restrict__ coef, T* __restrict__ out,
                                                        int n_total, int h, int w, int silu, f16_t* __restrict__ raw = nullptr) {
  constexpr int EPV = ET<T>::EPV;
  const int C = c1 + c2, nchunk = C / EPV;
  const int ho = POOL ? h / 2 : h, wo = POOL ? w / 2 : w;
  const long long total = (long long)n_total * ho * wo * nchunk;
  for (long long idx = (long long)blockIdx.x * blockDim.x + threadIdx.x; idx < total; idx += (long long)gridDim.x * blockDim.x) {
    const int chunk = (int)(idx % nchunk);
    long long pix = idx / nchunk;
    const int xo = (int)(pix % wo); pix /= wo;
    const int yo = (int)(pix % ho);
    const int n = (int)(pix / ho);
    const int c0 = chunk * EPV;
    const T* base; int cs, co;
    if (c0 < c1) { base = x1; cs = c1; co = c0; } else { base = x2; cs = c2; co = c0 - c1; }
    float A[EPV], B[EPV];
#pragma unroll
    for (int e = 0; e < EPV; e += 2) {
      const float4 q = *reinterpret_cast<const float4*>(coef + ((size_t)n * C + c0 + e) * 2);
      A[e] = q.x; B[e] = q.y; A[e + 1] = q.z; B[e + 1] = q.w;
    }
    float r[EPV], rr[EPV];
    if (!POOL) {
      const uint4 v = *reinterpret_cast<const uint4*>(base + (((size_t)n * h + yo) * w + xo) * cs + co);
      float f[EPV];
      unpack16<T>(v, f);
#pragma unroll
      for (int e = 0; e < EPV; ++e) { rr[e] = f[e]; const float y = f[e] * A[e] + B[e]; r[e] = silu ? silu_t<T>(y) : y; }
    } else {
#pragma unroll
      for (int e = 0; e < EPV; ++e) { r[e] = 0.f; rr[e] = 0.f; }
#pragma unroll
      for (int dy = 0; dy < 2; ++dy)
#pragma unroll
        for (int dx = 0; dx < 2; ++dx) {
          const uint4 v = *reinterpret_cast<const uint4*>(base + (((size_t)n * h + 2 * yo + dy) * w + 2 * xo + dx) * cs + co);
          float f[EPV];
          unpack16<T>(v, f);
#pragma unroll
          for (int e = 0; e < EPV; ++e) { rr[e] += 0.25f * f[e]; const float y = f[e] * A[e] + B[e]; r[e] += 0.25f * (silu ? silu_t<T>(y) : y); }
        }
    }
    if constexpr (SPLIT) {
      store_split4(reinterpret_cast<f16_t*>(out) + (((size_t)n * ho + yo) * wo + xo) * 2 * C, c0, r);
      if (raw) store_split4(raw + (((size_t)n * ho + yo) * wo + xo) * 2 * C, c0, rr);
    } else
      *reinterpret_cast<uint4*>(out + (((size_t)n * ho + yo) * wo + xo) * C + c0) = pack16<T>(r);
  }
}

template <typename T> struct Pair;
template <> struct Pair<float> {
  static __device__ __forceinline__ void load(const float* p, float& a, float& b) { const float2 v = *reinterpret_cast<const float2*>(p); a = v.x; b = v.y; }
  static __device__ __forceinline__ void store(float* p, float a, float b) { *reinterpret_cast<float2*>(p) = make_float2(a, b); }
};
template <> struct Pair<bf16_t> {
  static __device__ __forceinline__ void load(const bf16_t* p, float& a, float& b) {
    const uint32_t v = *reinterpret_cast<const uint32_t*>(p); a = bf16_bits_to_f32(v & 0xffffu); b = bf16_bits_to_f32(v >> 16);
  }
  static __device__ __forceinline__ void store(bf16_t* p, float a, float b) {
    *reinterpret_cast<uint32_t*>(p) = pack2_bf16(a, b);
  }
};
template <> struct Pair<f16_t> {
  static __device__ __forceinline__ void load(const f16_t* p, float& a, float& b) {
    const uint32_t v = *reinterpret_cast<const uint32_t*>(p); a = f16_bits_to_f32(v & 0xffffu); b = f16_bits_to_f32(v >> 16);
  }
  static __device__ __forceinline__ void store(f16_t* p, float a, float b) {
    *reinterpret_cast<uint32_t*>(p) = pack2_f16(a, b);
  }
};

template <typename T>
__global__ __launch_bounds__(256) void gn_fused_kernel(const T* __restrict__ x1, int c1, const T* __restrict__ x2, int c2, int hw,
                                                        int groups, float eps, const float* __restrict__ gamma,
                                                        const float* __restrict__ beta, const T* __restrict__ ss, int ld_ss,
                                                        T* __restrict__ out, int silu) {
  __shared__ double red[2][4];
  __shared__ float sAB[2][64];
  const int C = c1 + c2, cg = C / groups, hp = cg / 2;
  const int g = blockIdx.x, n = blockIdx.y, tid = threadIdx.x;
  const int npair = hw * hp;
  float s = 0.f, q = 0.f;
  for (int e = tid; e < npair; e += 256) {
    const int p = e / hp, c = g * cg + (e - p * hp) * 2;
    const T* src = c < c1 ? x1 + ((size_t)n * hw + p) * c1 + c : x2 + ((size_t)n * hw + p) * c2 + (c - c1);
    float a, b;
    Pair<T>::load(src, a, b);
    s += a + b;
    q += a * a + b * b;
  }
  double ds = wave_sum((double)s), dq = wave_sum((double)q);
  if ((tid & 63) == 0) { red[0][tid >> 6] = ds; red[1][tid >> 6] = dq; }
  __syncthreads();
  if (tid < cg) {
    const double cnt = (double)hw * cg;
    const double mean = (red[0][0] + red[0][1] + red[0][2] + red[0][3]) / cnt;
    double var = (red[1][0] + red[1][1] + red[1][2] + red[1][3]) / cnt - mean * mean;
    if (var < 0.0) var = 0.0;
    const float rstd = (float)(1.0 / sqrt(var + (double)eps));
    const int c = g * cg + tid;
    float A = rstd * (gamma ? gamma[c] : 1.f);
    float B = (beta ? beta[c] : 0.f) - (float)mean * A;
    if (ss) {
      const float sc = 1.f + ld1<T>(ss + (size_t)n * ld_ss + c);
      const float sh = ld1<T>(ss + (size_t)n * ld_ss + C + c);
      A = A * sc;
      B = B * sc + sh;
    }
    sAB[0][tid] = A;
    sAB[1][tid] = B;
  }
  __syncthreads();
  for (int e = tid; e < npair; e += 256) {
    const int p = e / hp, cl = (e - p * hp) * 2, c = g * cg + cl;
    const T* src = c < c1 ? x1 + ((size_t)n * hw + p) * c1 + c : x2 + ((size_t)n * hw + p) * c2 + (c - c1);
    float a, b;
    Pair<T>::load(src, a, b);
    a = a * sAB[0][cl] + sAB[1][cl];
    b = b * sAB[0][cl + 1] + sAB[1][cl + 1];
    if (silu) { a = silu_t<T>(a); b = silu_t<T>(b); }
    Pair<T>::store(out + ((size_t)n * hw + p) * C + c, a, b);
  }
}

template <typename T>
__global__ __launch_bounds__(256) void resample_kernel(const T* __restrict__ x, T* __restrict__ out, int n_total, int h, int w,
                                                        int c, int mode) {
  constexpr int EPV = ET<T>::EPV;
  const int nchunk = c / EPV;
  const int ho = mode ? 2 * h : h / 2, wo = mode ? 2 * w : w / 2;
  const long long total = (long long)n_total * ho * wo * nchunk;
  for (long long idx = (long long)blockIdx.x * blockDim.x + threadIdx.x; idx < total; idx += (long long)gridDim.x * blockDim.x) {
    const int chunk = (int)(idx % nchunk);
    long long pix = idx / nchunk;
    const int xo = (int)(pix % wo); pix /= wo;
    const int yo = (int)(pix % ho);
    const int n = (int)(pix / ho);
    uint4 o;
    if (mode) {
      o = *reinterpret_cast<const uint4*>(x + (((size_t)n * h + (yo >> 1)) * w + (xo >> 1)) * c + chunk * EPV);
    } else {
      float r[EPV];
#pragma unroll
      for (int e = 0; e < EPV; ++e) r[e] = 0.f;
#pragma unroll
      for (int dy = 0; dy < 2; ++dy)
#pragma unroll
        for (int dx = 0; dx < 2; ++dx) {
          const uint4 v = *reinterpret_cast<const uint4*>(x + (((size_t)n * h + 2 * yo + dy) * w + 2 * xo + dx) * c + chunk * EPV);
          float f[EPV];
          unpack16<T>(v, f);
#pragma unroll
          for (int e = 0; e < EPV; ++e) r[e] += 0.25f * f[e];
        }
      o = pack16<T>(r);
    }
    *reinterpret_cast<uint4*>(out + (((size_t)n * ho + yo) * wo + xo) * c + chunk * EPV) = o;
  }
}

inline int gn_splits(int hw) {
  int s = hw / 64;
  if (s < 1) s = 1;
  if (s > GN_SPLITS) s = GN_SPLITS;
  return s;
}

inline int grid_for(long long total, int block) {
  long long g = (total + block - 1) / block;
  if (g > 256 * 16) g = 256 * 16;
  if (g < 1) g = 1;
  return (int)g;
}

}

extern "C" int64_t dts_gn_ws_floats(int n, int groups) { return (int64_t)n * GN_SPLITS * groups * 2; }

extern "C" int dts_gn_coef(const void* x1, int c1, const void* x2, int c2, int dtype, int n, int hw, int groups, float eps,
                           const float* gamma, const float* beta, const void* scale_shift, int ld_ss,
                           float* coef, float* ws, dts_stream s) {
  const int C = c1 + c2;
  DTS_CHECK_ARG(x1 && coef && ws, "dts_gn_coef: null pointer");
  DTS_CHECK_ARG(n > 0 && hw > 0 && groups > 0 && C % groups == 0, "dts_gn_coef: C=%d groups=%d", C, groups);
  DTS_CHECK_ARG(c2 == 0 || x2, "dts_gn_coef: c2 without x2");
  const int epv = dtype == DTS_F32 ? 4 : 8;
  DTS_CHECK_ARG(c1 % epv == 0 && c2 % epv == 0, "dts_gn_coef: channels (%d,%d) unsupported", c1, c2);
  DTS_CHECK_ARG(scale_shift == nullptr || ld_ss >= 2 * C, "dts_gn_coef: ld_ss=%d < 2*C=%d", ld_ss, 2 * C);
  const int splits = gn_splits(hw);
  hipStream_t st = to_stream(s);
  DTS_DISPATCH_DTYPE(dtype, {
    const int nchunk = C / ET<T>::EPV;
    const int planes = 256 / (nchunk < 256 ? nchunk : 256);
    const size_t lds = (size_t)planes * C * 2 * sizeof(float);
    hipLaunchKernelGGL((gn_partial_kernel<T>), dim3(splits, n), dim3(256), lds, st, (const T*)x1, c1, (const T*)x2, c2, hw,
                       groups, splits, ws);
    DTS_CHECK_LAUNCH("dts_gn_coef(partial)");
    const int total = n * C;
    hipLaunchKernelGGL((gn_coef_kernel<T>), dim3((total + 255) / 256), dim3(256), 0, st, ws, splits, groups, C, hw, eps, gamma,
                       beta, (const T*)scale_shift, ld_ss, coef, n);
    DTS_CHECK_LAUNCH("dts_gn_coef(coef)");
  });
  return DTS_OK;
}

extern "C" int dts_gn_coef_strips(const float* st1, int c1, const float* st2, int c2, int dtype, int n, int hw, int groups, float eps,
                                  const float* gamma, const float* beta, const void* scale_shift, int ld_ss, float* coef,
                                  dts_stream s) {
  const int C = c1 + c2;
  DTS_CHECK_ARG(st1 && coef, "dts_gn_coef_strips: null pointer");
  DTS_CHECK_ARG(n > 0 && hw > 0 && hw % 64 == 0 && groups > 0 && C % groups == 0, "dts_gn_coef_strips: hw=%d C=%d groups=%d", hw, C,
                groups);
  DTS_CHECK_ARG(c2 == 0 || st2, "dts_gn_coef_strips: c2 without st2");
  DTS_CHECK_ARG(C / groups <= 128, "dts_gn_coef_strips: %d channels per group (max 128)", C / groups);
  DTS_CHECK_ARG(scale_shift == nullptr || ld_ss >= 2 * C, "dts_gn_coef_strips: ld_ss=%d < 2*C=%d", ld_ss, 2 * C);
  DTS_CHECK_ARG(n <= 65535, "dts_gn_coef_strips: n too large for grid.y");
  hipStream_t st = to_stream(s);
  DTS_DISPATCH_DTYPE(dtype, {
    const int threads = (long long)(hw / 64) * (C / groups) > 4096 ? 256 : 64;
    hipLaunchKernelGGL((gn_coef_strips_kernel<T>), dim3(groups, n), dim3(threads), 0, st, st1, c1, st2, c2, hw / 64, groups, hw, eps,
                       gamma, beta, (const T*)scale_shift, ld_ss, coef);
    DTS_CHECK_LAUNCH("dts_gn_coef_strips");
  });
  return DTS_OK;
}

static int gn_apply_impl(const void* x1, int c1, const void* x2, int c2, int dtype, const float* coef, void* out, int n, int h,
                         int w, int silu, int pool, bool split, dts_stream s, void* raw_out = nullptr);
extern "C" int dts_gn_apply(const void* x1, int c1, const void* x2, int c2, int dtype, const float* coef, void* out, int n, int h,
                            int w, int silu, int pool, dts_stream s) {
  return gn_apply_impl(x1, c1, x2, c2, dtype, coef, out, n, h, w, silu, pool, false, s);
}
extern "C" int dts_gn_apply_x3(const float* x1, int c1, const float* x2, int c2, const float* coef, void* out, void* raw_out, int n, int h,
                               int w, int silu, int pool, dts_stream s) {
  DTS_CHECK_ARG((c1 + c2) % 32 == 0, "dts_gn_apply_x3: %d channels are not a multiple of 32", c1 + c2);
  return gn_apply_impl(x1, c1, x2, c2, DTS_F32, coef, out, n, h, w, silu, pool, true, s, raw_out);
}
static int gn_apply_impl(const void* x1, int c1, const void* x2, int c2, int dtype, const float* coef, void* out, int n, int h,
                         int w, int silu, int pool, bool split, dts_stream s, void* raw_out) {
  const int C = c1 + c2;
  DTS_CHECK_ARG(x1 && coef && out, "dts_gn_apply: null pointer");
  DTS_CHECK_ARG(n > 0 && h > 0 && w > 0 && C > 0, "dts_gn_apply: n=%d h=%d w=%d C=%d", n, h, w, C);
  DTS_CHECK_ARG(c2 == 0 || x2, "dts_gn_apply: c2 without x2");
  const int epv = dtype == DTS_F32 ? 4 : 8;
  DTS_CHECK_ARG(c1 % epv == 0 && c2 % epv == 0, "dts_gn_apply: channels (%d,%d) unsupported", c1, c2);
  DTS_CHECK_ARG(!pool || (h % 2 == 0 && w % 2 == 0), "dts_gn_apply: pool needs even h,w");
  hipStream_t st = to_stream(s);
  const long long total = (long long)n * (pool ? h / 2 : h) * (pool ? w / 2 : w) * (C / epv);
  if (split) {
    using T = float;
    if (pool)
      hipLaunchKernelGGL((gn_apply_kernel<T, true, true>), dim3(grid_for(total, 256)), dim3(256), 0, st, (const T*)x1, c1, (const T*)x2,
                         c2, coef, (T*)out, n, h, w, silu, (f16_t*)raw_out);
    else if (C / epv <= 256 && n <= 65535) {
      const int nchunk = C / epv, k = 256 / nchunk, hw = h * w;
      long long ppb = ((long long)n * hw + 4095) / 4096;
      ppb = ((ppb + 2 * k - 1) / (2 * k)) * (2 * k);
      if (c1 % 8 == 0 && dts_knob_get(DTS_KNOB_GN_FUSE) != 2)
        hipLaunchKernelGGL((gn_apply_rows_kernel<T, true, true>), dim3((unsigned)((hw + ppb - 1) / ppb), n), dim3(k * nchunk), 0, st, (const T*)x1, c1,
                           (const T*)x2, c2, coef, (T*)out, hw, (int)ppb, silu, (f16_t*)raw_out);
      else
      hipLaunchKernelGGL((gn_apply_rows_kernel<T, true>), dim3((unsigned)((hw + ppb - 1) / ppb), n), dim3(k * nchunk), 0, st, (const T*)x1, c1,
                         (const T*)x2, c2, coef, (T*)out, hw, (int)ppb, silu, (f16_t*)raw_out);
    } else
      hipLaunchKernelGGL((gn_apply_kernel<T, false, true>), dim3(grid_for(total, 256)), dim3(256), 0, st, (const T*)x1, c1, (const T*)x2,
                         c2, coef, (T*)out, n, h, w, silu, (f16_t*)raw_out);
    DTS_CHECK_LAUNCH("dts_gn_apply_x3");
    return DTS_OK;
  }
  DTS_DISPATCH_DTYPE(dtype, {
    if (pool)
      hipLaunchKernelGGL((gn_apply_kernel<T, true>), dim3(grid_for(total, 256)), dim3(256), 0, st, (const T*)x1, c1, (const T*)x2,
                         c2, coef, (T*)out, n, h, w, silu);
    else if (C / epv <= 256 && n <= 65535) {
      const int nchunk = C / epv, k = 256 / nchunk, hw = h * w;
      long long ppb = ((long long)n * hw + 4095) / 4096;
      ppb = ((ppb + 2 * k - 1) / (2 * k)) * (2 * k);
      hipLaunchKernelGGL((gn_apply_rows_kernel<T>), dim3((unsigned)((hw + ppb - 1) / ppb), n), dim3(k * nchunk), 0, st, (const T*)x1, c1,
                         (const T*)x2, c2, coef, (T*)out, hw, (int)ppb, silu);
    } else
      hipLaunchKernelGGL((gn_apply_kernel<T, false>), dim3(grid_for(total, 256)), dim3(256), 0, st, (const T*)x1, c1, (const T*)x2,
                         c2, coef, (T*)out, n, h, w, silu);
    DTS_CHECK_LAUNCH("dts_gn_apply");
  });
  return DTS_OK;
}

extern "C" int dts_gn_fused(const void* x1, int c1, const void* x2, int c2, int dtype, int n, int hw, int groups, float eps,
                            const float* gamma, const float* beta, const void* scale_shift, int ld_ss, void* out, int silu,
                            dts_stream s) {
  const int C = c1 + c2;
  DTS_CHECK_ARG(x1 && out, "dts_gn_fused: null pointer");
  DTS_CHECK_ARG(n > 0 && hw > 0 && groups > 0 && C % groups == 0, "dts_gn_fused: C=%d groups=%d", C, groups);
  const int cg = C / groups;
  DTS_CHECK_ARG(cg % 2 == 0 && cg <= 64 && c1 % 2 == 0, "dts_gn_fused: channels per group %d unsupported", cg);
  DTS_CHECK_ARG(c2 == 0 || x2, "dts_gn_fused: c2 without x2");
  DTS_CHECK_ARG(scale_shift == nullptr || ld_ss >= 2 * C, "dts_gn_fused: ld_ss=%d < 2*C=%d", ld_ss, 2 * C);
  DTS_CHECK_ARG(n <= 65535, "dts_gn_fused: n too large for grid.y");
  hipStream_t st = to_stream(s);
  DTS_DISPATCH_DTYPE(dtype, {
    hipLaunchKernelGGL((gn_fused_kernel<T>), dim3(groups, n), dim3(256), 0, st, (const T*)x1, c1, (const T*)x2, c2, hw, groups, eps,
                       gamma, beta, (const T*)scale_shift, ld_ss, (T*)out, silu);
    DTS_CHECK_LAUNCH("dts_gn_fused");
  });
  return DTS_OK;
}

// ... 14 lines not shown
```

### diffusion_tts_amd/networks.py

```python
import math
import os
from typing import Dict, Optional

import numpy as np
import torch

from . import ops
from .config import EDMConfig, Block, edm_blocks


def _qkv_perm_edm(heads: int, d: int) -> torch.Tensor:
    s, h, c = torch.meshgrid(torch.arange(3), torch.arange(heads), torch.arange(d), indexing='ij')
    return (h * 3 * d + c * 3 + s).reshape(-1).to(torch.int32)


class _BlockParams:
    pass


class EDMPrecond:

    def __init__(self, cfg: EDMConfig, state_dict: Dict[str, torch.Tensor], device='cuda', dtype=ops.F16X3):
        if not torch.cuda.is_available():
            raise RuntimeError('EDMPrecond (HIP) needs a GPU: there is no CPU fallback in this package')
# ... 12 lines not shown
            if cfg.embedding_type not in ('positional', 'fourier') or cfg.encoder_type not in ('standard', 'residual') \
                    or list(cfg.resample_filter) not in ([1, 1], [1, 3, 3, 1]):
                raise NotImplementedError(f'SongUNet options embedding_type={cfg.embedding_type!r}, encoder_type={cfg.encoder_type!r}, '
                                          f'resample_filter={cfg.resample_filter!r}')
        self.fir = (not self.adm) and cfg.fir
        self.evals = 0
        self.fuse_gn = os.environ.get('DTS_GN_FUSE', '0') == '1'
        from .graphs import GraphCache
        self._graphs = GraphCache(self._device_forward)
        sd = {k[len('model.'):]: v for k, v in state_dict.items() if k.startswith('model.')}
        self._load(sd)

    def _dev(self, t):
        return t.detach().to(self.device, torch.float32).contiguous()

    def _load(self, sd):
        cfg, dev, dt = self.cfg, self.device, self.dtype
        f = self._dev
        mc = cfg.model_channels
        self.map0_w, self.map0_b = f(sd['map_layer0.weight']), f(sd['map_layer0.bias'])
        self.map1_w, self.map1_b = f(sd['map_layer1.weight']), f(sd['map_layer1.bias'])
        if cfg.label_dim:
            self.label_w = f(sd['map_label.weight'])
            self.label_b = f(sd['map_label.bias']) if 'map_label.bias' in sd else None
        if not self.adm and cfg.embedding_type == 'fourier':
            if 'map_noise.freqs' not in sd:
                raise KeyError('map_noise.freqs: a Fourier-embedding network carries its frequencies in the state dict')
            self.freqs = (2 * np.pi * sd['map_noise.freqs'].detach().to('cpu', torch.float32)).to(dev).contiguous()
            if self.freqs.numel() != cfg.noise_channels // 2:
                raise ValueError(f'map_noise.freqs has {self.freqs.numel()} entries, expected {cfg.noise_channels // 2}')
        else:
            half = mc // 2
            freqs = torch.arange(0, half, dtype=torch.float32)
            freqs = freqs / (half - (0 if self.adm else 1))
            self.freqs = ((1 / 10000) ** freqs).to(dev)
        enc, dec, cfin = edm_blocks(cfg)
        self.enc, self.dec = enc, dec
        first = enc[0]
        self.conv_in_w, self.conv_in_b = f(sd[f'{first.name}.weight']), f(sd[f'{first.name}.bias'])
        self.blocks: Dict[str, _BlockParams] = {}
        aff_w, aff_b, off = [], [], 0
        for b in enc[1:] + dec:
            P = _BlockParams()
            n = b.name
            g = lambda k: sd[f'{n}.{k}']
            if b.kind == 'aux_residual':
                P.cpad = -(-4 * b.cin // ops.conv_cin_granule(dt)) * ops.conv_cin_granule(dt)
                P.w = ops.pack_conv_weight(ops.fused_down_weight(f(g('weight')), list(cfg.resample_filter), cpad=P.cpad), dt)
                P.b = f(g('bias'))
                self.blocks[n] = P
                continue
            P.g0, P.b0 = f(g('norm0.weight')), f(g('norm0.bias'))
            ph0 = self.x3 and b.up and not self.fir
            P.w0, P.cb0 = ops.pack_conv_weight(f(g('conv0.weight')), dt, up_phases=ph0), f(g('conv0.bias'))
            caff = b.cout * (2 if self.adm else 1)
            aff_w.append(g('affine.weight'))
            aff_b.append(g('affine.bias'))
            P.aff_off, P.caff = off, caff
            off += caff
            P.g1, P.b1 = f(g('norm1.weight')), f(g('norm1.bias'))
            P.w1, P.cb1 = ops.pack_conv_weight(f(g('conv1.weight')), dt), f(g('conv1.bias'))
            P.skip_w = P.skip_b = None
            if f'{n}.skip.weight' in sd:
                P.skip_w, P.skip_b = ops.pack_conv_weight(f(g('skip.weight')), dt), f(g('skip.bias'))
                P.cb1_skip = (P.cb1 + P.skip_b).contiguous()
            if b.heads:
                d = b.cout // b.heads
                perm = _qkv_perm_edm(b.heads, d).to(dev)
                P.g2, P.b2 = f(g('norm2.weight')), f(g('norm2.bias'))
                P.wqkv = ops.pack_conv_weight(f(g('qkv.weight')), dt, out_perm=perm)
                P.bqkv = f(g('qkv.bias'))[perm.long()].contiguous()
                P.wproj, P.bproj = ops.pack_conv_weight(f(g('proj.weight')), dt), f(g('proj.bias'))
            self.blocks[n] = P
        self.aff_w = ops.pack_conv_weight(f(torch.cat(aff_w, 0))[:, :, None, None].contiguous(), dt)
        self.aff_b = f(torch.cat(aff_b, 0))
        self.aff_total = off
        r = cfg.img_resolution
        on, oc = ('out_norm', 'out_conv') if self.adm else (f'dec.{r}x{r}_aux_norm', f'dec.{r}x{r}_aux_conv')
        self.out_g, self.out_b = f(sd[f'{on}.weight']), f(sd[f'{on}.bias'])
        self.out_w = f(sd[f'{oc}.weight']).permute(0, 2, 3, 1).contiguous()
        self.out_cb = f(sd[f'{oc}.bias'])
        self.cfin = cfin
        torch.cuda.synchronize(dev)

    def to(self, device):
        return self

    def eval(self):
        return self

    def round_sigma(self, sigma):
        return torch.as_tensor(sigma)

    @staticmethod
    def _groups(c):
        return min(32, c // 4)

    def _embedding(self, c_noise, class_labels, n):
        cfg = self.cfg
        emb = ops.pos_embedding(c_noise, self.freqs, swap=not self.adm)
        if self.adm:
            h = ops.linear(emb, self.map0_w, self.map0_b, act_out=True)
            if not cfg.label_dim:
                return ops.linear(h, self.map1_w, self.map1_b, act_out=True)
            h = ops.linear(h, self.map1_w, self.map1_b)
            lab = self._labels(class_labels, n)
            return ops.linear(lab, self.label_w, None, out=h, accumulate=True, act_out=True)
        if cfg.label_dim:
            lab = self._labels(class_labels, n) * math.sqrt(cfg.label_dim)
            ops.linear(lab.contiguous(), self.label_w, self.label_b, out=emb, accumulate=True)
        h = ops.linear(emb, self.map0_w, self.map0_b, act_out=True)
        return ops.linear(h, self.map1_w, self.map1_b, act_out=True)

    def _labels(self, class_labels, n):
        L = self.cfg.label_dim
        if class_labels is None:
            lab = torch.zeros([1, L], device=self.device)
        else:
            lab = class_labels.to(self.device, torch.float32).reshape(-1, L)
        if lab.shape[0] == 1 and n > 1:
            lab = lab.expand(n, L)
        if lab.shape[0] != n:
            raise ValueError(f'class_labels rows {lab.shape[0]} != batch {n}')
        return lab.contiguous()

    def _block(self, b: Block, x1, x2, aff):
        P = self.blocks[b.name]
        G = self._groups
        ss = aff[:, P.aff_off:P.aff_off + P.caff]
        bnc = None if self.adm else ss
        skip_src = None
        fir = self.fir and (b.up or b.down)
        up = b.up and not fir
        if fir:
            h = ops.group_norm(x1, G(b.cin), self.eps, P.g0, P.b0, x2=x2, silu=True)
            h = ops.conv2d(ops.resample_fir(h, b.up, split_out=self.x3), P.w0, P.cb0, bias_nc=bnc, gn_stats=True)
            if x2 is not None:
                raise NotImplementedError('a resampling block with a concatenated input')
            skip_src = ops.resample_fir(x1, b.up, split_out=self.x3)
        elif self.fuse_gn and not b.down and ops.conv_fuses_gn(x1, P.w0, x2=x2, up=b.up):
            coef = ops.gn_coefficients(x1, G(b.cin), self.eps, P.g0, P.b0, x2=x2)
            h = ops.conv2d(x1, P.w0, P.cb0, x2=x2, up=b.up, bias_nc=bnc, gn_stats=True, gn_coef=coef, gn_silu=True)
        else:
            raw = self.x3 and P.skip_w is not None and os.environ.get('DTS_X3_RAW_SPLIT', '1') != '0'
            h = ops.group_norm(x1, G(b.cin), self.eps, P.g0, P.b0, x2=x2, silu=True, pool=b.down, split_out=self.x3, raw_split=raw)
            if raw:
                h, skip_src = h
            h = ops.conv2d(h, P.w0, P.cb0, up=b.up, bias_nc=bnc, gn_stats=True)
        fuse1 = self.fuse_gn and ops.conv_fuses_gn(h, P.w1)
        if fuse1:
            coef1 = ops.gn_coefficients(h, G(b.cout), self.eps, P.g1, P.b1, scale_shift=ss if self.adm else None)
        else:
            h = ops.group_norm(h, G(b.cout), self.eps, P.g1, P.b1, scale_shift=ss if self.adm else None, silu=True, split_out=self.x3)
        if P.skip_w is not None and skip_src is not None and ops.conv_folds_skip(h, P.w1, (skip_src, P.skip_w, up)):
            sk = None
        elif P.skip_w is not None and skip_src is not None:
            sk = ops.conv2d(skip_src, P.skip_w, P.skip_b, up=up)
        elif P.skip_w is not None:
            src1, src2 = (ops.resample2x(x1, up=False), None) if b.down else (x1, x2)
            sk = ops.conv2d(src1, P.skip_w, P.skip_b, x2=src2, up=b.up)
        elif b.up or b.down:
            sk = ops.resample2x(x1, up=b.up)
        else:
            sk = x1
        if sk is None:
            x = ops.conv2d(h, P.w1, P.cb1_skip, skip=(skip_src, P.skip_w, up), out_scale=self.skip_scale, gn_stats=True)
        else:
            x = ops.conv2d(h, P.w1, P.cb1, residual=sk, out_scale=self.skip_scale, gn_stats=True,
                           gn_coef=coef1 if fuse1 else None, gn_silu=True)
        if b.heads:
            n, hh, ww, c = x.shape
            hn = ops.group_norm(x, G(c), self.eps, P.g2, P.b2, silu=False, split_out=self.x3)
            fx3 = self.x3 and ops.attention_x3_ok(hh * ww, c // b.heads)
            qkv = ops.conv2d(hn, P.wqkv, P.bqkv, out_split2=fx3)
            a = ops.attention(qkv.view(n, hh * ww, 3 * c), b.heads, 1.0 / math.sqrt(c // b.heads), x3=self.x3, split_out=fx3)
            a = ops.SplitAct(a.data.view(n, hh, ww, 2 * c), c) if fx3 else a.view(n, hh, ww, c)
            x = ops.conv2d(a, P.wproj, P.bproj, residual=x, out_scale=self.skip_scale, gn_stats=True)
        return x

    @torch.no_grad()
    def unet(self, xin, c_noise, class_labels):
        n = xin.shape[0]
        emb = self._embedding(c_noise, class_labels, n)
        e = ops.cast_from_f32(emb, self.act_dtype)
        aff = ops.conv2d(e.view(1, n, 1, -1), self.aff_w, self.aff_b).view(n, self.aff_total)
        x = ops.conv_in3(xin, self.conv_in_w, self.conv_in_b, self.enc[0].cout, self.act_dtype)
        skips = [x]
        aux, aux_nchw = xin, True
        for b in self.enc[1:]:
            if b.kind == 'aux_residual':
                P = self.blocks[b.name]
                s2d = ops.space_to_depth2(aux, self.dtype, nchw=aux_nchw, cpad=P.cpad)
                x = ops.conv2d(s2d, P.w, P.b, residual=x, out_scale=math.sqrt(0.5), gn_stats=True)
                skips[-1] = aux = x
                aux_nchw = False
                continue
            x = self._block(b, x, None, aff)
            skips.append(x)
        for b in self.dec:
            x2 = skips.pop() if x.shape[-1] != b.cin else None
            x = self._block(b, x, x2, aff)
        h = ops.group_norm(x, self._groups(self.cfin), 1e-5 if self.adm else 1e-6, self.out_g, self.out_b, silu=True)
        return ops.conv_out3(h, self.out_w, self.out_cb)

    @torch.no_grad()
    def _device_forward(self, x, sigma, class_labels):
        xin, coef = ops.edm_precond_in(x, sigma, self.sigma_data)
        F = self.unet(xin, coef[:, 3].contiguous(), class_labels)
        return ops.edm_precond_out(x, F, coef)

    @torch.no_grad()
    def __call__(self, x, sigma, class_labels=None, force_fp32=False, **model_kwargs):
        if force_fp32 and self.dtype == torch.float16:
            raise ValueError('force_fp32=True: this network was built with dtype=float16; build it with dtype=ops.F16X3 (default) or float32')
        aug = model_kwargs.pop('augment_labels', None)
        if aug is not None:
            raise NotImplementedError('augment_labels: training-time augmentation conditioning is outside the sampling path (networks.py:330-331)')
        if model_kwargs:
            raise TypeError(f'unexpected keyword arguments {sorted(model_kwargs)} (the reference U-Nets would raise too)')
        x = x.to(self.device, torch.float64).contiguous()
        n = x.shape[0]
        sigma = torch.as_tensor(sigma).to(self.device, torch.float64).reshape(-1).contiguous()
        if sigma.numel() not in (1, n):
            raise ValueError(f'sigma has {sigma.numel()} entries for batch {n}')
        if class_labels is not None:
            class_labels = class_labels.to(self.device, torch.float32).contiguous()
        self.evals += n
        return self._graphs(x, sigma, class_labels)
```

### diffusion_tts_amd/ops.py

```python
import ctypes as C
import math
import os

import torch

from . import _lib as L

_DT = {torch.float32: L.DTS_F32, torch.bfloat16: L.DTS_BF16, torch.float16: L.DTS_F16}

F16X3 = 'f16x3'


def act_dtype(dtype):
    return torch.float32 if dtype == F16X3 else dtype


def dtype_name(dtype):
    return dtype if isinstance(dtype, str) else {torch.float32: 'f32', torch.bfloat16: 'bf16', torch.float16: 'f16'}[dtype]


class X3Weight:

    def __init__(self, packed, acc_scale, shape):
        self.packed, self.acc_scale, self.shape = packed, float(acc_scale), tuple(shape)
# ... 67 lines not shown
    if not t.is_cuda:
        raise RuntimeError(f'{name} must be a GPU tensor (the HIP path has no CPU fallback)')
    if t.dim() != 2 or t.stride(1) != 1 or t.dtype != dtype:
        raise ValueError(f'{name}: expected a 2-D {dtype} view with unit inner stride')
    return t.data_ptr(), t.stride(0)


def _call(name, *args):
    lib = L.load()
    L.check(getattr(lib, name)(*args, _stream()), name)


def nchw_to_nhwc(x, dtype):
    n, c, h, w = x.shape
    out = torch.empty((n, h, w, c), dtype=dtype, device=x.device)
    _call('dts_nchw_to_nhwc', _ptr(x, 'x', torch.float32), _ptr(out), dt_code(dtype), n, c, h, w)
    return out


def nchw_to_nhwc_pad(x, dtype, cpad):
    n, c, h, w = x.shape
    out = torch.empty((n, h, w, cpad), dtype=dtype, device=x.device)
    _call('dts_nchw_to_nhwc_pad', _ptr(x, 'x', torch.float32), _ptr(out), dt_code(dtype), n, c, h, w, cpad)
    return out


def nhwc_to_nchw(x):
    n, h, w, c = x.shape
    out = torch.empty((n, c, h, w), dtype=torch.float32, device=x.device)
    _call('dts_nhwc_to_nchw', _ptr(x), dt_code(x.dtype), _ptr(out), n, c, h, w)
    return out


def _x3_split_pack(w_ohwi):
    O, kh, kw, I = w_ohwi.shape
    amax = float(w_ohwi.abs().max())
    k = 0 if amax == 0.0 else max(-24, min(24, int(math.floor(math.log2(16384.0 / amax)))))
    ws = (w_ohwi * (2.0 ** k)).contiguous()
    hi = ws.to(torch.float16)
    lo = (ws - hi.to(torch.float32)).to(torch.float16)
    packed = torch.stack([hi.view(O, kh, kw, I // 32, 32), lo.view(O, kh, kw, I // 32, 32)], dim=-2)
    return packed.reshape(O, kh, kw, 2 * I).contiguous(), 2.0 ** -k


UP_PHASE_ROWS = (((1, 0, 0), (0, 1, 1)), ((1, 1, 0), (0, 0, 1)))


def up_phase_weights(w):
    R = torch.tensor(UP_PHASE_ROWS, dtype=torch.float64, device=w.device)
    ph = torch.einsum('ayh,bxw,oihw->aboyxi', R, R, w.to(torch.float64))
    O, I = w.shape[:2]
    return ph.reshape(4, O, 2, 2, I).to(w.dtype)


def pack_conv_weight(w, dtype, out_perm=None, up_phases=False):
    if w.dim() == 3:
        w = w.unsqueeze(-1)
    w = w.contiguous()
    O, I, kh, kw = w.shape
    if up_phases and (dtype != F16X3 or (kh, kw) != (3, 3)):
        raise ValueError('pack_conv_weight: up_phases is the split-precision mode\'s, for 3x3 weights')
    if dtype == F16X3:
        wp = w if out_perm is None else w[out_perm.long()]
        if I % 32:
            raise ValueError(f'pack_conv_weight(F16X3): {I} input channels are not a multiple of 32 (one K step of the split image)')
        packed, acc_scale = _x3_split_pack(wp.permute(0, 2, 3, 1))
        xw = X3Weight(packed, acc_scale, (O, kh, kw, I))
        if up_phases:
            pp, xw.phase_acc_scale = _x3_split_pack(up_phase_weights(wp).reshape(4 * O, 2, 2, I))
            xw.phases = pp.reshape(4, O, 2, 2, 2 * I)
        return xw
    out = torch.empty((O, kh, kw, I), dtype=dtype, device=w.device)
    _call('dts_pack_conv_weight', _ptr(w, 'w', torch.float32), _ptr(out), dt_code(dtype), O, I, kh, kw,
          _ptr(out_perm, 'perm', torch.int32))
    return out


_CONV_WS = {}
CONV_WS_BYTES = 96 << 20


def _conv_workspace(device):
    key = (device.type, device.index)
    ws = _CONV_WS.get(key)
    if ws is None:
        ws = _CONV_WS[key] = torch.empty(CONV_WS_BYTES, dtype=torch.uint8, device=device)
    return ws


def _conv_args(x1, w, x2, up):
    n, hin, win, c1 = x1.shape
    a = L.ConvArgs()
    a.c1, a.c2 = c1, 0 if x2 is None else x2.shape[-1]
    a.n, a.hin, a.win, a.cout, a.ksize = n, hin, win, w.shape[0], w.shape[1]
    a.up, a.dtype = int(up), dt_code(x1.dtype)
    return a


def conv_kernel(x1, w, x2=None, up=False, residual=None, gn_coef=None, gn_stats=False):
    a = _conv_args(x1, w, x2, up)
    if isinstance(w, X3Weight):
        a.c1, a.c2, a.dtype = 2 * (a.c1 + a.c2), 0, L.DTS_F16X3
    a.residual = _ptr(residual)
    a.gn_coef = _ptr(gn_coef, 'gn_coef', torch.float32)
    if up and x2 is None and getattr(w, 'phases', None) is not None:
        a.workspace, a.workspace_bytes = 16, CONV_WS_BYTES
        if gn_stats and (4 * a.hin * a.win) % 64 == 0:
            a.stats_out = 16
        _route_phases(a, w, None)
    return int(L.load().dts_conv_kernel(C.byref(a)))


def _route_phases(a, w, phases):
    if phases is False or getattr(w, 'phases', None) is None or a.up != 1:
        return False
    keep = (a.up, a.w, a.acc_scale)
    a.up, a.w, a.acc_scale = 2, (w.phases.data_ptr() if w.phases.is_cuda else None), w.phase_acc_scale
    if phases is None and not L.load().dts_conv_takes_phases(C.byref(a)):
        a.up, a.w, a.acc_scale = keep
        return False
    return True


def conv_takes_phases(x1, w, bias=None, **kw):
    kw.pop('up', None)
    a, *_keep = _conv2d_args(x1, w, bias, up=True, **kw)
    return a.up == 2


def conv_fuses_gn(x1, w, *, x2=None, up=False):
    return bool(L.load().dts_conv_fuses_gn(C.byref(_conv_args(x1, w, x2, up))))


def _skip_fields(a, skip, n, ho, wo, cout):
    src, sw, sup = skip
    if not isinstance(src, SplitAct) or not isinstance(sw, X3Weight):
        raise ValueError('conv2d: skip = (SplitAct, X3Weight, up)')
    sh = (n, ho // 2, wo // 2) if sup else (n, ho, wo)
    if tuple(src.shape[:3]) != sh or tuple(sw.shape) != (cout, 1, 1, src.shape[3]):
        raise ValueError(f'conv2d: skip source {tuple(src.shape)} / weight {tuple(sw.shape)} do not match an output of {(n, ho, wo, cout)} (up={bool(sup)})')
    a.skip_c, a.skip_x, a.skip_w = src.data.shape[-1], _ptr(src.data, 'skip_x', torch.float16), _ptr(sw.packed, 'skip_w', torch.float16)
    a.skip_acc_scale, a.skip_up = sw.acc_scale, int(bool(sup))


def conv_folds_skip(x1, w, skip):
    if not isinstance(w, X3Weight) or skip is None or not isinstance(skip[0], SplitAct):
        return False
    a = _conv_args(x1, w, None, False)
    a.c1, a.c2, a.dtype = 2 * a.c1, 0, L.DTS_F16X3
    _skip_fields(a, skip, a.n, a.hin, a.win, a.cout)
    return bool(L.load().dts_conv_folds_skip(C.byref(a)))


def _conv2d_args(x1, w, bias=None, *, x2=None, bias_nc=None, residual=None, up=False, out_scale=1.0, out=None, gn_stats=False,
                 timing_events=None, gn_coef=None, gn_silu=True, out_split2=False, skip=None, phases=None):
    n, hin, win, c1 = x1.shape
    c2 = 0 if x2 is None else x2.shape[-1]
    cout, kh, kw, cin = w.shape
    if cin != c1 + c2 or kh != kw:
        raise ValueError(f'conv2d: weight {tuple(w.shape)} does not match inputs ({c1}+{c2})')
    ho, wo = (2 * hin, 2 * win) if up else (hin, win)
    x3 = isinstance(w, X3Weight)
    if x3 and (x1.dtype != torch.float32 or gn_coef is not None):
        raise ValueError('conv2d: a split-precision weight takes float32 activations (and no fused input GroupNorm)')
    if isinstance(x1, SplitAct) and (not x3 or x2 is not None):
        raise ValueError('conv2d: a split activation feeds a split-precision weight, alone')
    out_split2 = bool(out_split2) and x3 and not gn_stats
    if out_split2:
        out = torch.empty((n, ho, wo, 2 * cout), dtype=torch.float16, device=x1.device)
    elif out is None:
        out = torch.empty((n, ho, wo, cout), dtype=x1.dtype, device=x1.device)
    a, xs = L.ConvArgs(), None
    a.out_split2 = int(out_split2)
    dt_in = x1.dtype
    if x3:
        xs = x1.data if isinstance(x1, SplitAct) else split3_f16(x1, x2)
        a.x1, a.c1, a.x2, a.c2 = _ptr(xs, 'x1', torch.float16), 2 * (c1 + c2), None, 0
        a.w, a.acc_scale = _ptr(w.packed, 'w', torch.float16), w.acc_scale
    else:
        a.x1, a.c1 = _ptr(x1, 'x1'), c1
        a.x2, a.c2 = _ptr(x2, 'x2', x1.dtype), c2
        a.w = _ptr(w, 'w', x1.dtype)
    a.bias = _ptr(bias, 'bias', torch.float32)
    a.bias_nc, a.ld_bias_nc = _rows(bias_nc, 'bias_nc', x1.dtype)
    a.residual = _ptr(residual, 'residual', x1.dtype)
    if residual is not None and tuple(residual.shape) != (n, ho, wo, cout):
        raise ValueError(f'conv2d: residual shape {tuple(residual.shape)} != {(n, ho, wo, cout)}')
    a.out = _ptr(out, 'out', torch.float16 if out_split2 else x1.dtype)
    a.n, a.hin, a.win, a.cout, a.ksize = n, hin, win, cout, kh
    a.up, a.out_scale, a.dtype = int(up), float(out_scale), (L.DTS_F16X3 if x3 else dt_code(x1.dtype))
    ws = _conv_workspace(x1.device)
    a.workspace, a.workspace_bytes = ws.data_ptr(), ws.numel()
    st = None
    if gn_stats and (ho * wo) % 64 == 0:
        st = torch.empty(((n * ho * wo) // 64, cout, 2), dtype=torch.float32, device=x1.device)
        a.stats_out = st.data_ptr()
    if timing_events is not None:
        a.ev_start, a.ev_stop = timing_events
    if skip is not None:
        if not x3 or residual is not None or up:
            raise ValueError('conv2d: skip= is the split-precision mode\'s, without residual / upsample')
        _skip_fields(a, skip, n, ho, wo, cout)
    if gn_coef is not None:
        if tuple(gn_coef.shape) != (n, c1 + c2, 2):
            raise ValueError(f'conv2d: gn_coef shape {tuple(gn_coef.shape)} != {(n, c1 + c2, 2)}')
        a.gn_coef, a.gn_silu = _ptr(gn_coef, 'gn_coef', torch.float32), int(gn_silu)
    if x3 and up:
        _route_phases(a, w, phases)
    return a, out, st, out_split2, (xs, ws)


def conv_plan(*args, **kw):
    a, *_keep = _conv2d_args(*args, **kw)
    info = L.ConvPlanInfo()
    _call('dts_conv_plan', C.byref(a), C.byref(info))
    return {f: int(getattr(info, f)) for f, _ in L.ConvPlanInfo._fields_}


def conv2d(x1, w, bias=None, *, x2=None, bias_nc=None, residual=None, up=False, out_scale=1.0, out=None, gn_stats=False,
           timing_events=None, gn_coef=None, gn_silu=True, out_split2=False, skip=None, phases=None):
    a, out, st, out_split2, _keep = _conv2d_args(x1, w, bias, x2=x2, bias_nc=bias_nc, residual=residual, up=up, out_scale=out_scale, out=out,
                                                 gn_stats=gn_stats, timing_events=timing_events, gn_coef=gn_coef, gn_silu=gn_silu,
                                                 out_split2=out_split2, skip=skip, phases=phases)
    _call('dts_conv2d', C.byref(a))
    if out_split2:
        return SplitQKV(out, (out.shape[0], out.shape[1], out.shape[2], out.shape[3] // 2))
    out._gn_stats = st if (st is not None and a.stats_written) else None
    return out


def split3_f16(x1, x2=None):
    n, h, w, c1 = x1.shape
    c2 = 0 if x2 is None else x2.shape[-1]
    out = torch.empty((n, h, w, 2 * (c1 + c2)), dtype=torch.float16, device=x1.device)
    _call('dts_split3_f16', _ptr(x1, 'x1', torch.float32), c1, _ptr(x2, 'x2', torch.float32), c2, _ptr(out), n * h * w)
    return out


def split2_f16(x):
    c = x.shape[-1]
    out = torch.empty(tuple(x.shape[:-1]) + (2 * c,), dtype=torch.float16, device=x.device)
    _call('dts_split2_f16', _ptr(x, 'x', torch.float32), c, _ptr(out), x.numel() // c)
    return out


def conv_in3(x, w, bias, cout, dtype):
    n, c, h, wd = x.shape
    assert c == 3
    out = torch.empty((n, h, wd, cout), dtype=dtype, device=x.device)
    _call('dts_conv_in3', _ptr(x, 'x', torch.float32), _ptr(w, 'w', torch.float32), _ptr(bias, 'bias', torch.float32),
          _ptr(out), dt_code(dtype), n, h, wd, cout)
    return out


def conv_out3(x, w_ohwi, bias):
    n, h, wd, c = x.shape
    out = torch.empty((n, 3, h, wd), dtype=torch.float32, device=x.device)
    _call('dts_conv_out3', _ptr(x), dt_code(x.dtype), _ptr(w_ohwi, 'w', torch.float32), _ptr(bias, 'bias', torch.float32),
          _ptr(out), n, h, wd, c)
    return out


def gn_coef(x1, groups, eps, gamma, beta, *, x2=None, scale_shift=None):
    n, h, w, c1 = x1.shape
    c2 = 0 if x2 is None else x2.shape[-1]
    C_ = c1 + c2
    lib = L.load()
    ws = torch.empty((lib.dts_gn_ws_floats(n, groups),), dtype=torch.float32, device=x1.device)
    coef = torch.empty((n, C_, 2), dtype=torch.float32, device=x1.device)
    ss_ptr, ss_ld = _rows(scale_shift, 'scale_shift', x1.dtype)
    _call('dts_gn_coef', _ptr(x1, 'x1'), c1, _ptr(x2, 'x2', x1.dtype), c2, dt_code(x1.dtype), n, h * w, groups, float(eps),
          _ptr(gamma, 'gamma', torch.float32), _ptr(beta, 'beta', torch.float32), ss_ptr, ss_ld, _ptr(coef), _ptr(ws))
    return coef


def gn_apply(x1, coef, *, x2=None, silu=True, pool=False, split_out=False, raw_split=False):
    n, h, w, c1 = x1.shape
    c2 = 0 if x2 is None else x2.shape[-1]
    ho, wo = (h // 2, w // 2) if pool else (h, w)
    if split_out:
        out = torch.empty((n, ho, wo, 2 * (c1 + c2)), dtype=torch.float16, device=x1.device)
        raw = torch.empty_like(out) if raw_split else None
        _call('dts_gn_apply_x3', _ptr(x1, 'x1', torch.float32), c1, _ptr(x2, 'x2', torch.float32), c2, _ptr(coef, 'coef', torch.float32),
              _ptr(out), _ptr(raw), n, h, w, int(silu), int(pool))
        return (SplitAct(out, c1 + c2), SplitAct(raw, c1 + c2)) if raw_split else SplitAct(out, c1 + c2)
    out = torch.empty((n, ho, wo, c1 + c2), dtype=x1.dtype, device=x1.device)
    _call('dts_gn_apply', _ptr(x1, 'x1'), c1, _ptr(x2, 'x2', x1.dtype), c2, dt_code(x1.dtype),
          _ptr(coef, 'coef', torch.float32), _ptr(out), n, h, w, int(silu), int(pool))
    return out


GN_FUSED_MAX_HW = 64


def _coef_from_strips(x1, x2, groups, eps, gamma, beta, scale_shift):
    n, h, w, c1 = x1.shape
    c2 = 0 if x2 is None else x2.shape[-1]
    st1 = getattr(x1, '_gn_stats', None)
    st2 = None if x2 is None else getattr(x2, '_gn_stats', None)
    if st1 is None or (x2 is not None and st2 is None) or (h * w) % 64 != 0:
        return None
    coef = torch.empty((n, c1 + c2, 2), dtype=torch.float32, device=x1.device)
    ss_ptr, ss_ld = _rows(scale_shift, 'scale_shift', x1.dtype)
    _call('dts_gn_coef_strips', _ptr(st1, 'st1', torch.float32), c1, _ptr(st2, 'st2', torch.float32), c2, dt_code(x1.dtype), n,
          h * w, groups, float(eps), _ptr(gamma, 'gamma', torch.float32), _ptr(beta, 'beta', torch.float32), ss_ptr, ss_ld,
          _ptr(coef))
    return coef


def gn_coefficients(x1, groups, eps, gamma, beta, *, x2=None, scale_shift=None):
    coef = _coef_from_strips(x1, x2, groups, eps, gamma, beta, scale_shift)
    return coef if coef is not None else gn_coef(x1, groups, eps, gamma, beta, x2=x2, scale_shift=scale_shift)


def group_norm(x1, groups, eps, gamma, beta, *, x2=None, scale_shift=None, silu=True, pool=False, path=None, split_out=False, raw_split=False):
    n, h, w, c1 = x1.shape
    c2 = 0 if x2 is None else x2.shape[-1]
    cg = (c1 + c2) // groups
    fused_ok = (not pool) and cg % 2 == 0 and cg <= 64
    if path in (None, 'strips'):
        coef = _coef_from_strips(x1, x2, groups, eps, gamma, beta, scale_shift)
        if coef is not None:
            return gn_apply(x1, coef, x2=x2, silu=silu, pool=pool, split_out=split_out, raw_split=raw_split)
    if path == 'strips':
        raise ValueError('strip statistics are not attached to the input(s)')
    if path is None:
        path = 'fused' if (fused_ok and h * w <= GN_FUSED_MAX_HW and not split_out) else 'split'
    if path == 'fused':
        if not fused_ok:
            raise ValueError('fused GroupNorm needs pool=False and an even number (<= 64) of channels per group')
        out = torch.empty((n, h, w, c1 + c2), dtype=x1.dtype, device=x1.device)
        ss_ptr, ss_ld = _rows(scale_shift, 'scale_shift', x1.dtype)
        _call('dts_gn_fused', _ptr(x1, 'x1'), c1, _ptr(x2, 'x2', x1.dtype), c2, dt_code(x1.dtype), n, h * w, groups, float(eps),
              _ptr(gamma, 'gamma', torch.float32), _ptr(beta, 'beta', torch.float32), ss_ptr, ss_ld, _ptr(out), int(silu))
        return out
    return gn_apply(x1, gn_coef(x1, groups, eps, gamma, beta, x2=x2, scale_shift=scale_shift), x2=x2, silu=silu, pool=pool,
                    split_out=split_out, raw_split=raw_split)


def resample2x(x, up):
    n, h, w, c = x.shape
    ho, wo = (2 * h, 2 * w) if up else (h // 2, w // 2)
    out = torch.empty((n, ho, wo, c), dtype=x.dtype, device=x.device)
    _call('dts_resample2x', _ptr(x), _ptr(out), dt_code(x.dtype), n, h, w, c, int(up))
    return out


FIR_TAPS = (1, 3, 3, 1)


def resample_fir(x, up, split_out=False):
    n, h, w, c = x.shape
    ho, wo = (2 * h, 2 * w) if up else (h // 2, w // 2)
    if split_out:
        out = torch.empty((n, ho, wo, 2 * c), dtype=torch.float16, device=x.device)
        _call('dts_resample_fir', _ptr(x, 'x', torch.float32), _ptr(out), L.DTS_F32, n, h, w, c, int(up), 1)
        return SplitAct(out, c)
    out = torch.empty((n, ho, wo, c), dtype=x.dtype, device=x.device)
    _call('dts_resample_fir', _ptr(x), _ptr(out), dt_code(x.dtype), n, h, w, c, int(up), 0)
    return out


def conv_cin_granule(dtype):
    return 32 if dtype in (F16X3, torch.float32) else 64


def space_to_depth2(x, dtype, nchw=False, cpad=None):
    if nchw:
        n, c, h, w = x.shape
    else:
        n, h, w, c = x.shape
    g = conv_cin_granule(dtype)
    cpad = -(-4 * c // g) * g if cpad is None else cpad
    x3, adt = dtype == F16X3, act_dtype(dtype)
    if x.dtype != (torch.float32 if nchw else adt):
        raise ValueError(f'space_to_depth2: input dtype {x.dtype} in compute mode {dtype_name(dtype)}')
    out = torch.empty((n, h // 2, w // 2, 2 * cpad if x3 else cpad), dtype=torch.float16 if x3 else adt, device=x.device)
    _call('dts_space_to_depth2', _ptr(x), int(nchw), _ptr(out), dt_code(adt), n, h, w, c, cpad, int(x3))
    return SplitAct(out, cpad) if x3 else out


def fused_down_weight(w, taps=FIR_TAPS, cpad=None, out_dtype=torch.float32):
    O, Cin, kh, kw = w.shape
    if (kh, kw) != (3, 3) or len(taps) != 4:
        raise ValueError('fused_down_weight: a 3x3 weight and a 4-tap filter')
    k = torch.tensor(list(taps), dtype=torch.float64, device=w.device)
    F2 = torch.outer(k, k) / k.sum() ** 2
    w64 = w.detach().to(torch.float64)
    w6 = torch.zeros((O, Cin, 6, 6), dtype=torch.float64, device=w.device)
    for a in range(4):
        for b in range(4):
            w6[:, :, a:a + 3, b:b + 3] += F2[a, b] * w64
    w3 = w6.view(O, Cin, 3, 2, 3, 2).permute(0, 3, 5, 1, 2, 4).reshape(O, 4 * Cin, 3, 3)
    cpad = 4 * Cin if cpad is None else cpad
    out = torch.zeros((O, cpad, 3, 3), dtype=out_dtype, device=w.device)
    out[:, :4 * Cin] = w3.to(out_dtype)
    return out


def attention(qkv, heads, scale, x3=False, split_out=False):
    n, t, c3 = qkv.shape
    c = c3 // 3
    d = c // heads
    pre = isinstance(qkv, SplitQKV)
# ... 492 lines not shown
```

### include/dts.h

```cpp
#ifndef DTS_H_
#define DTS_H_

#include <stdint.h>

#ifdef __cplusplus
extern "C" {
#endif

typedef void* dts_stream;

enum dts_dtype { DTS_F32 = 0, DTS_BF16 = 1, DTS_F16 = 2,
                 DTS_F16X3 = 3 };
enum dts_status { DTS_OK = 0, DTS_ERR_ARG = -1, DTS_ERR_LAUNCH = -2, DTS_ERR_UNSUPPORTED = -3 };

#define DTS_ABI_VERSION 120
int dts_version(void);
const char* dts_last_error(void);
int dts_set_tuning(int knob, int value);
int dts_get_tuning(int knob);

int dts_nchw_to_nhwc(const float* src, void* dst, int dtype, int n, int c, int h, int w, dts_stream s);
int dts_nhwc_to_nchw(const void* src, int dtype, float* dst, int n, int c, int h, int w, dts_stream s);
int dts_nchw_to_nhwc_pad(const float* src, void* dst, int dtype, int n, int c, int h, int w, int cpad, dts_stream s);
int dts_pack_conv_weight(const float* w_oihw, void* dst, int dtype, int O, int I, int kh, int kw,
                         const int32_t* out_perm, dts_stream s);

typedef struct dts_conv_args {
  const void* x1; int32_t c1;
  const void* x2; int32_t c2;
  const void* w;
  const float* bias;
  const void* bias_nc;
  int32_t ld_bias_nc;
  const void* residual;
  void* out;
  int32_t n, hin, win;
  int32_t cout;
  int32_t ksize;
  int32_t up;
  float out_scale;
  int32_t dtype;
  void* workspace;
  int64_t workspace_bytes;
  float* stats_out;
  int32_t stats_written;
  void* ev_start; void* ev_stop;
  const float* gn_coef;
  int32_t gn_silu;
  float acc_scale;
  int32_t out_split2;
  int32_t skip_c;
  const void* skip_x;
  const void* skip_w;
  float skip_acc_scale;
  int32_t skip_up;
} dts_conv_args;
int dts_conv_fuses_gn(const dts_conv_args* a);
int dts_conv_folds_skip(const dts_conv_args* a);
int dts_conv_takes_phases(const dts_conv_args* a);
int dts_conv_kernel(const dts_conv_args* a);
typedef struct dts_conv_plan_info {
  int32_t kernel;
  int32_t tile, waves, stages, pf;
  int32_t gn, sk, dbg;
  int32_t splits, ks_per_split;
  int32_t n_ct, n_pt, nblk;
  int32_t threads, lds_bytes;
  int32_t stats_in_kernel, stats_in_reduce, stats_written;
  int32_t epi_rows;
  int32_t fuses_gn, folds_skip;
  int32_t refused;
  int32_t phases;
} dts_conv_plan_info;
int dts_conv_plan(const dts_conv_args* a, dts_conv_plan_info* out);
int dts_conv2d(dts_conv_args* a, dts_stream s);

int dts_conv_in3(const float* x, const float* w, const float* bias, void* out, int dtype,
                 int n, int h, int w_, int cout, dts_stream s);
int dts_conv_out3(const void* x, int dtype, const float* w, const float* bias, float* out,
                  int n, int h, int w_, int c, dts_stream s);

int64_t dts_gn_ws_floats(int n, int groups);
int dts_gn_coef(const void* x1, int c1, const void* x2, int c2, int dtype, int n, int hw, int groups, float eps,
                const float* gamma, const float* beta, const void* scale_shift, int ld_ss,
                float* coef, float* ws, dts_stream s);
int dts_gn_coef_strips(const float* st1, int c1, const float* st2, int c2, int dtype, int n, int hw, int groups, float eps,
                       const float* gamma, const float* beta, const void* scale_shift, int ld_ss, float* coef, dts_stream s);
int dts_gn_apply(const void* x1, int c1, const void* x2, int c2, int dtype, const float* coef,
                 void* out, int n, int h, int w, int silu, int pool, dts_stream s);
int dts_gn_apply_x3(const float* x1, int c1, const float* x2, int c2, const float* coef, void* out, void* raw_out, int n, int h, int w, int silu,
                    int pool, dts_stream s);
int dts_gn_fused(const void* x1, int c1, const void* x2, int c2, int dtype, int n, int hw, int groups, float eps,
                 const float* gamma, const float* beta, const void* scale_shift, int ld_ss, void* out, int silu, dts_stream s);
int dts_resample2x(const void* x, void* out, int dtype, int n, int h, int w, int c, int mode, dts_stream s);
int dts_resample_fir(const void* x, void* out, int dtype, int n, int h, int w, int c, int up, int split_out, dts_stream s);
int dts_space_to_depth2(const void* x, int x_nchw_f32, void* out, int dtype, int n, int h, int w, int c, int cpad, int split_out, dts_stream s);

int dts_attention(const void* qkv, void* out, int dtype, int n, int t, int heads, int d, float scale, dts_stream s);
int dts_attention_x3(const void* qkv_split, void* out, int out_split3, int n, int t, int heads, int d, float scale, dts_stream s);
int dts_attention_masked(const void* qkv, void* out, int dtype, int n, int t, int heads, int d, float scale, int causal,
                         const int32_t* key_len, dts_stream s);

int dts_cross_attention(const void* q, const void* kv, const int32_t* kv_rows, int kv_n, void* out, int dtype, int n, int tq, int tk,
                        int heads, int d, float scale, dts_stream s);
int dts_layer_norm(const void* x, void* out, int dtype, int64_t rows, int c, float eps, const float* gamma, const float* beta, dts_stream s);
int dts_geglu(const void* x, void* out, int dtype, int64_t rows, int inner, dts_stream s);
int dts_group_rows(const void* rows, int n, int64_t row_bytes, void* workspace, int32_t* slot, int32_t* reps, int32_t* count, dts_stream s);

int dts_patchify(const float* x, void* out, int dtype, int n, int size, int patch, int kpad, dts_stream s);
int dts_vit_tokens(const void* patches, const float* cls, const float* pos, void* tokens, int dtype, int n, int t, int c, dts_stream s);
int dts_gelu(const void* x, void* out, int dtype, int64_t count, int kind, dts_stream s);
int dts_text_tokens(const int32_t* ids, const float* tok, const float* pos, void* out, int dtype, int n, int t, int c, int vocab, dts_stream s);
int dts_vit_head(const void* tokens, float* out, int dtype, int n, int t, int c, float eps, const float* gamma, const float* beta, dts_stream s);

int dts_layer_norm_x3(const float* x, float* out_f32, void* out_split, int64_t rows, int c, float eps, const float* gamma, const float* beta,
                      dts_stream s);
int dts_gelu_x3(const float* x, void* out_split, int64_t rows, int c, int kind, dts_stream s);
int dts_patchify_x3(const float* x, void* out_split, int n, int size, int patch, int kpad, dts_stream s);
int dts_vit_tokens_f32(const float* patches, const float* cls, const float* pos, float* tokens, int n, int t, int c, dts_stream s);
int dts_vit_head_f32(const float* tokens, float* out, int n, int t, int c, float eps, const float* gamma, const float* beta, dts_stream s);

int dts_linear(const float* x, int ldx, const float* w, const float* bias, float* y, int ldy,
               int m, int k, int n, int act_in, int act_out, int accumulate, dts_stream s);
int dts_pos_embedding(const float* v, const float* freqs, float* out, int n, int half, int swap, dts_stream s);
int dts_edm_precond_in(const double* x, const double* sigma, int nsigma, float sigma_data,
                       float* xin, float* coef, int n, int chw, dts_stream s);
int dts_edm_precond_out(const double* x, const float* F, const float* coef, float* D, int n, int chw, dts_stream s);
int dts_split3_f16(const float* x1, int c1, const float* x2, int c2, void* out, int64_t rows, dts_stream s);
int dts_split2_f16(const float* x, int c, void* out, int64_t rows, dts_stream s);
int dts_cast_from_f32(const float* src, void* dst, int dtype, int64_t count, dts_stream s);
int dts_cast_to_f32(const void* src, int dtype, float* dst, int64_t count, dts_stream s);

int dts_heun_xhat(const double* x_cur, int xb, int bcast, const void* eps, int eps_f32, double noise_coef,
                  double* x_hat, int nb, int chw, dts_stream s);
int dts_heun_euler(const double* x_hat, const float* D, double t_hat, double t_next,
                   double* d_cur, double* x_next, int64_t count, dts_stream s);
int dts_heun_correct(const double* x_hat, const float* D2, const double* d_cur, double t_hat, double t_next,
                     double* x_next, int64_t count, dts_stream s);

int dts_quantize_u8(const void* x, int is_f32, uint8_t* out, int64_t count, dts_stream s);
int dts_brightness(const uint8_t* img, float* rewards, int n, int hw, dts_stream s);
int dts_cosine_rows(const float* a, const float* b, int b_rows, float* out, int n, int d, dts_stream s);
int dts_resample_u8(const uint8_t* src, uint8_t* dst, int planes, int h, int w, int out_len, int axis, const int32_t* bounds,
                    const int32_t* coefs, int ksize, dts_stream s);
int dts_lut_u8_f32(const uint8_t* img, const float* lut, float* out, int n, int c, int hw, dts_stream s);
int dts_u8_to_unit_f32(const uint8_t* img, float* out, int64_t count, dts_stream s);

int64_t dts_jpeg_workspace_bytes(int n, int h, int w);
int dts_jpeg_size(const uint8_t* img, int32_t* sizes, int n, int h, int w, const uint16_t* qtab, void* workspace, int64_t workspace_bytes,
                  int16_t* coef_out, dts_stream s);

int dts_attnpool_tokens(const void* x, const float* pos, void* tokens, int dtype, int n, int hw, int c, dts_stream s);
int dts_take_token(const void* src, int dtype, float* out, int n, int t, int c, int token, dts_stream s);
int dts_softmax_gather(const float* logits, const int32_t* target, float* rewards, int n, int k, dts_stream s);

int dts_candidate_noise(const double* pivot, const double* g, const int32_t* mode, const float* scale,
                        double* cand, int nb, int b, int chw, dts_stream s);
int dts_candidate_noise_sd(const void* pivot, const void* u, const int32_t* mode, const float* scale, void* cand, int dtype, int n,
                           int64_t count, dts_stream s);

int dts_cfg_combine(const void* uncond, const void* cond, float guidance, void* out, int dtype, int64_t count, dts_stream s);
int dts_ddim_candidates(const void* x, const void* e, const void* z, void* prev, void* x0_out, int dtype,
                        float alpha_t, float alpha_prev, float sigma_t, int ncand, int64_t count, dts_stream s);

#ifdef __cplusplus
}
#endif
#endif
```

Baseline: 1521 candidate U-Net steps/sec.

## Fuse residual resampling into conv epilogue and GN into in/out 3-channel convs

Adds a residual_map mode so the conv epilogue reads the residual through a 2x2 mean or nearest-up mapping instead of launching a separate resample kernel. The stem conv_in3 now emits per-strip GroupNorm statistics, and the final GroupNorm+SiLU is folded into conv_out3 via precomputed coefficients. This removes several small kernel launches and full-tensor round trips through memory per U-Net and classifier pass, in exchange for more complex epilogues, extra gather loads, and fp-contract changes to the stats accumulation. Each path is guarded by env flags that are on by default and by plan-refusal checks.

Result: faster. 1538 candidate U-Net steps/sec (median of 6 runs) (+1.1%).

```diff
diff --git a/diffusion_tts_amd/_lib.py b/diffusion_tts_amd/_lib.py
--- a/diffusion_tts_amd/_lib.py
+++ b/diffusion_tts_amd/_lib.py
@@ -18,7 +18,8 @@
                 ('ksize', C.c_int32), ('up', C.c_int32), ('out_scale', C.c_float), ('dtype', C.c_int32),
                 ('workspace', _p), ('workspace_bytes', C.c_int64), ('stats_out', _p), ('stats_written', C.c_int32),
                 ('ev_start', _p), ('ev_stop', _p), ('gn_coef', _p), ('gn_silu', C.c_int32), ('acc_scale', C.c_float), ('out_split2', C.c_int32),
-                ('skip_c', C.c_int32), ('skip_x', _p), ('skip_w', _p), ('skip_acc_scale', C.c_float), ('skip_up', C.c_int32)]
+                ('skip_c', C.c_int32), ('skip_x', _p), ('skip_w', _p), ('skip_acc_scale', C.c_float), ('skip_up', C.c_int32),
+                ('residual_map', C.c_int32)]
 
 
 class ConvPlanInfo(C.Structure):
@@ -35,6 +36,8 @@
     'dts_conv2d': [C.POINTER(ConvArgs), _p],
     'dts_conv_in3': [_p, _p, _p, _p, _i, _i, _i, _i, _i, _p],
     'dts_conv_out3': [_p, _i, _p, _p, _p, _i, _i, _i, _i, _p],
+    'dts_conv_in3_stats': [_p, _p, _p, _p, _p, _i, _i, _i, _i, _p],
+    'dts_conv_out3_gn': [_p, _p, _i, _p, _p, _p, _i, _i, _i, _i, _p],
     'dts_gn_coef': [_p, _i, _p, _i, _i, _i, _i, _i, _f, _p, _p, _p, _i, _p, _p, _p],
     'dts_gn_coef_strips': [_p, _i, _p, _i, _i, _i, _i, _i, _f, _p, _p, _p, _i, _p, _p],
     'dts_gn_apply': [_p, _i, _p, _i, _i, _p, _p, _i, _i, _i, _i, _i, _p],
@@ -90,7 +93,7 @@
          'dts_jpeg_workspace_bytes': ([_i, _i, _i], _i64)}
 
 _lib = None
-ABI_VERSION = 120
+ABI_VERSION = 121
 
 
 def load():
@@ -108,7 +111,7 @@
         fn = getattr(lib, name)
         fn.argtypes, fn.restype = argt, rest
     got = lib.dts_version()
-    if got != ABI_VERSION or C.sizeof(ConvArgs) != 208:
+    if got != ABI_VERSION or C.sizeof(ConvArgs) != 216:
         raise RuntimeError(f'{LIB_PATH} has ABI version {got}, this binding needs {ABI_VERSION}: rebuild with `python -m diffusion_tts_amd.build --force`')
     _lib = lib
     return lib
diff --git a/diffusion_tts_amd/classifier.py b/diffusion_tts_amd/classifier.py
--- a/diffusion_tts_amd/classifier.py
+++ b/diffusion_tts_amd/classifier.py
@@ -78,15 +78,20 @@
         h = ops.group_norm(x, 32, 1e-5, P.g0, P.b0, silu=True, pool=L.down, split_out=self.x3, raw_split=raw)
         if raw:
             h, x = h
-        elif L.down:
-            x = ops.resample2x(x, up=False)
+        x_full = x if (L.down and not raw) else None
         h = ops.conv2d(h, P.w0, P.cb0, gn_stats=True)
         ss = emb_all[:, P.off:P.off + 2 * L.cout]
         h = ops.group_norm(h, 32, 1e-5, P.g1, P.b1, scale_shift=ss, silu=True, split_out=self.x3)
         if raw and ops.conv_folds_skip(h, P.w1, (x, P.sw, False)):
             return ops.conv2d(h, P.w1, P.cb1_skip, skip=(x, P.sw, False), gn_stats=True)
+        rmap = None
+        if x_full is not None:
+            if ops.residual_map_enabled('mean') and ops.conv_maps_residual(h, P.w1, x_full, 'mean'):
+                rmap = 'mean'
+            else:
+                x = ops.resample2x(x_full, up=False)
         sk = x if P.sw is None else ops.conv2d(x, P.sw, P.sb)
-        return ops.conv2d(h, P.w1, P.cb1, residual=sk, gn_stats=True)
+        return ops.conv2d(h, P.w1, P.cb1, residual=sk, residual_map=rmap, gn_stats=True)
 
     def _attn(self, L: ClsLayer, x):
         P = self.params[L.prefix]
@@ -115,7 +120,7 @@
         for L in self.layers:
             if L.kind == 'conv_in':
                 P = self.params[L.prefix]
-                h = ops.conv_in3(x.contiguous(), P.w, P.b, L.cout, self.act_dtype)
+                h = ops.conv_in3(x.contiguous(), P.w, P.b, L.cout, self.act_dtype, gn_stats=ops.in3_stats_enabled())
             elif L.kind == 'res':
                 h = self._res(L, h, emb_all)
             else:
diff --git a/diffusion_tts_amd/csrc/conv_igemm.hip b/diffusion_tts_amd/csrc/conv_igemm.hip
--- a/diffusion_tts_amd/csrc/conv_igemm.hip
+++ b/diffusion_tts_amd/csrc/conv_igemm.hip
@@ -2,7 +2,7 @@
 #include <hip/hip_ext.h>
 #include <type_traits>
 
-static_assert(sizeof(dts_conv_args) == 208, "dts_conv_args layout changed: bump DTS_ABI_VERSION and update the bindings (_lib.py ConvArgs)");
+static_assert(sizeof(dts_conv_args) == 216, "dts_conv_args layout changed: bump DTS_ABI_VERSION and update the bindings (_lib.py ConvArgs)");
 
 int dts_conv_launch_phase_form(const void* plan, const void* params, const void* call);
 
@@ -42,6 +42,7 @@
   const char* sk_x; const char* sk_w;
   int sk_c, sk_up;
   float sk_ratio;
+  int residual_map;
 };
 
 template <typename T> struct Mma;
@@ -360,56 +361,74 @@
   }
 }
 
-template <int MT, int NT, typename TM = TileMap>
-__device__ __forceinline__ void conv_epilogue_rows_f32(const ConvP& kp, f32x4_t (&acc)[MT][NT], int cm0, const TM& tm, int wm, int wn,
-                                                       int lrow, int lq, char* smem, int wave) {
-  static_assert(NT == 4, "64-pixel wave strips");
-  constexpr int CW = 16 * MT;
-  constexpr int LPR = 4 * MT;
-  constexpr int RPI = LPR <= 8 ? 8 : (LPR <= 16 ? 4 : 2);
-  constexpr int ITERS = 32 / RPI;
-  constexpr int ROWB = CW * 4 + 16;
-  char* const ws = smem + (size_t)wave * (32 * ROWB);
-  const int lane = threadIdx.x & 63;
-  const int rsub = lane / LPR, c4 = lane - rsub * LPR;
-  const bool act = rsub < RPI;
+template <int MAP>
+__device__ __forceinline__ size_t residual_map_pixel(const ConvP& kp, int pp) {
+  int n, y, x;
+  if (kp.hw_shift >= 0) {
+    n = pp >> kp.hw_shift;
+    const int rem = pp & ((1 << kp.hw_shift) - 1);
+    y = rem >> kp.w_shift; x = rem & ((1 << kp.w_shift) - 1);
+  } else {
+    const int hw = kp.hout * kp.wout;
+    n = pp / hw;
+    const int rem = pp - n * hw;
+    y = rem / kp.wout; x = rem - y * kp.wout;
+  }
+  if constexpr (MAP == 1) return ((size_t)n * (kp.hout >> 1) + (y >> 1)) * (kp.wout >> 1) + (x >> 1);
+  else return ((size_t)n * (2 * kp.hout) + 2 * y) * (2 * kp.wout) + 2 * x;
+}
+
+template <int MT, int HALF, bool MEAN, typename TM>
+__device__ __forceinline__ void conv_epilogue_rows_half(const ConvP& kp, f32x4_t (&acc)[MT][4], const TM& tm, char* ws, int wn, int lrow, int lq,
+                                                        int rsub, int c4, bool act, int co, const float4& b4, const float4& n4, float (&ss4)[4],
+                                                        float (&sq4)[4]) {
+  constexpr int half = HALF, MAP = MEAN ? 2 : 0;
+  constexpr int LPR = 4 * MT, RPI = LPR <= 8 ? 8 : (LPR <= 16 ? 4 : 2), ITERS = 32 / RPI, ROWB = 16 * MT * 4 + 16;
+  constexpr int CH = ITERS < 8 ? ITERS : 8;
+  constexpr int CHM = MAP == 2 ? 2 : CH;
+  static_assert(ITERS % CHM == 0, "residual batches");
+  typedef float f32x4_nt __attribute__((ext_vector_type(4)));
   const int p_cout = kp.cout;
-  const int co = cm0 + wm * CW + c4 * 4;
   const float* __restrict__ res = reinterpret_cast<const float*>(kp.residual);
-  if (tm.pix(wn * 64) >= kp.P) return;
-  float4 b4 = make_float4(0.f, 0.f, 0.f, 0.f), n4 = make_float4(0.f, 0.f, 0.f, 0.f);
-  if (act) {
-    if (kp.bias) b4 = *reinterpret_cast<const float4*>(kp.bias + co);
-    if (kp.bias_nc) {
-      const int pp0 = tm.pix(wn * 64), hw = kp.hout * kp.wout;
-      n4 = *reinterpret_cast<const float4*>(reinterpret_cast<const float*>(kp.bias_nc) + (size_t)(kp.hw_shift >= 0 ? pp0 >> kp.hw_shift : pp0 / hw) * kp.ld_bias_nc + co);
-    }
-  }
   const float asc = kp.acc_scale, osc = kp.out_scale;
   const bool want_stats = kp.stats != nullptr;
-  float ss4[4] = {0.f, 0.f, 0.f, 0.f}, sq4[4] = {0.f, 0.f, 0.f, 0.f};
-  typedef float f32x4_nt __attribute__((ext_vector_type(4)));
-  constexpr int CH = ITERS < 8 ? ITERS : 8;
-#pragma unroll
-  for (int half = 0; half < 2; ++half) {
-#pragma unroll
-    for (int n2 = 0; n2 < 2; ++n2)
-#pragma unroll
-      for (int mt = 0; mt < MT; ++mt)
-        *reinterpret_cast<f32x4_t*>(ws + (n2 * 16 + lrow) * ROWB + (mt * 16 + lq * 4) * 4) = acc[mt][half * 2 + n2];
-#pragma unroll
-   for (int u0 = 0; u0 < ITERS; u0 += CH) {
-    size_t prow[CH];
-    float4 rv[CH];
-#pragma unroll
-    for (int u = 0; u < CH; ++u) {
-      prow[u] = (size_t)tm.pix(wn * 64 + half * 32 + (u0 + u) * RPI + (act ? rsub : 0)) * p_cout + co;
+  const bool near = std::is_same<TM, TileMap>::value && kp.residual_map == 1;
+#pragma unroll
+  for (int n2 = 0; n2 < 2; ++n2)
+#pragma unroll
+    for (int mt = 0; mt < MT; ++mt)
+      *reinterpret_cast<f32x4_t*>(ws + (n2 * 16 + lrow) * ROWB + (mt * 16 + lq * 4) * 4) = acc[mt][half * 2 + n2];
+#pragma unroll
+   for (int u0 = 0; u0 < ITERS; u0 += CHM) {
+    size_t prow[CHM];
+    float4 rv[CHM];
+    [[maybe_unused]] uint4 rq[MAP == 2 ? CHM : 1][4];
+#pragma unroll
+    for (int u = 0; u < CHM; ++u) {
+      const int pp = tm.pix(wn * 64 + half * 32 + (u0 + u) * RPI + (act ? rsub : 0));
+      prow[u] = (size_t)pp * p_cout + co;
       rv[u] = make_float4(0.f, 0.f, 0.f, 0.f);
-      if (res && act) rv[u] = *reinterpret_cast<const float4*>(res + prow[u]);
-    }
-#pragma unroll
-    for (int u = 0; u < CH; ++u) {
+      if (res && act) {
+        if constexpr (MAP == 0) {
+          rv[u] = *reinterpret_cast<const float4*>(res + (near ? residual_map_pixel<1>(kp, pp) * p_cout + co : prow[u]));
+        } else {
+          const float* r0 = res + residual_map_pixel<2>(kp, pp) * p_cout + co;
+          const float* r1 = r0 + (size_t)2 * kp.wout * p_cout;
+          rq[u][0] = *reinterpret_cast<const uint4*>(r0); rq[u][1] = *reinterpret_cast<const uint4*>(r0 + p_cout);
+          rq[u][2] = *reinterpret_cast<const uint4*>(r1); rq[u][3] = *reinterpret_cast<const uint4*>(r1 + p_cout);
+        }
+      }
+    }
+#pragma unroll
+    for (int u = 0; u < CHM; ++u) {
       if (!act) continue;
+      if constexpr (MAP == 2) {
+        if (res) {
+          float m[4];
+          mean2x2_vec<float>(rq[u][0], rq[u][1], rq[u][2], rq[u][3], m);
+          rv[u] = make_float4(m[0], m[1], m[2], m[3]);
+        }
+      }
       const f32x4_t a = *reinterpret_cast<const f32x4_t*>(ws + ((u0 + u) * RPI + rsub) * ROWB + c4 * 16);
       float v[4] = {a[0] * asc + b4.x, a[1] * asc + b4.y, a[2] * asc + b4.z, a[3] * asc + b4.w};
       if (kp.bias_nc) { v[0] += n4.x; v[1] += n4.y; v[2] += n4.z; v[3] += n4.w; }
@@ -438,10 +457,51 @@
       }
       if (want_stats) {
 #pragma unroll
-        for (int r = 0; r < 4; ++r) { ss4[r] += v[r]; sq4[r] += v[r] * v[r]; }
+        for (int r = 0; r < 4; ++r) {
+          {
+#pragma clang fp contract(off)
+            ss4[r] += v[r];
+          }
+          sq4[r] = __builtin_fmaf(v[r], v[r], sq4[r]);
+        }
       }
     }
    }
+}
+
+template <int MT, int NT, typename TM = TileMap>
+__device__ __forceinline__ void conv_epilogue_rows_f32(const ConvP& kp, f32x4_t (&acc)[MT][NT], int cm0, const TM& tm, int wm, int wn,
+                                                       int lrow, int lq, char* smem, int wave) {
+  static_assert(NT == 4, "64-pixel wave strips");
+  constexpr int CW = 16 * MT;
+  constexpr int LPR = 4 * MT;
+  constexpr int RPI = LPR <= 8 ? 8 : (LPR <= 16 ? 4 : 2);
+  constexpr int ROWB = CW * 4 + 16;
+  char* const ws = smem + (size_t)wave * (32 * ROWB);
+  const int lane = threadIdx.x & 63;
+  const int rsub = lane / LPR, c4 = lane - rsub * LPR;
+  const bool act = rsub < RPI;
+  const int p_cout = kp.cout;
+  const int co = cm0 + wm * CW + c4 * 4;
+  if (tm.pix(wn * 64) >= kp.P) return;
+  float4 b4 = make_float4(0.f, 0.f, 0.f, 0.f), n4 = make_float4(0.f, 0.f, 0.f, 0.f);
+  if (act) {
+    if (kp.bias) b4 = *reinterpret_cast<const float4*>(kp.bias + co);
+    if (kp.bias_nc) {
+      const int pp0 = tm.pix(wn * 64), hw = kp.hout * kp.wout;
+      n4 = *reinterpret_cast<const float4*>(reinterpret_cast<const float*>(kp.bias_nc) + (size_t)(kp.hw_shift >= 0 ? pp0 >> kp.hw_shift : pp0 / hw) * kp.ld_bias_nc + co);
+    }
+  }
+  const bool want_stats = kp.stats != nullptr;
+  float ss4[4] = {0.f, 0.f, 0.f, 0.f}, sq4[4] = {0.f, 0.f, 0.f, 0.f};
+  if (std::is_same<TM, TileMap>::value && kp.residual_map == 2) {
+    if constexpr (std::is_same<TM, TileMap>::value) {
+      conv_epilogue_rows_half<MT, 0, true>(kp, acc, tm, ws, wn, lrow, lq, rsub, c4, act, co, b4, n4, ss4, sq4);
+      conv_epilogue_rows_half<MT, 1, true>(kp, acc, tm, ws, wn, lrow, lq, rsub, c4, act, co, b4, n4, ss4, sq4);
+    }
+  } else {
+    conv_epilogue_rows_half<MT, 0, false>(kp, acc, tm, ws, wn, lrow, lq, rsub, c4, act, co, b4, n4, ss4, sq4);
+    conv_epilogue_rows_half<MT, 1, false>(kp, acc, tm, ws, wn, lrow, lq, rsub, c4, act, co, b4, n4, ss4, sq4);
   }
   if (want_stats) {
 #pragma unroll
@@ -1586,6 +1646,7 @@
   p.cout = a->cout; p.taps = a->ksize * a->ksize; p.up = a->up;
   p.P = (int)((long long)p.n * p.hout * p.wout);
   p.residual = (const char*)a->residual; p.gn_coef = a->gn_coef;
+  p.residual_map = a->residual_map;
   p.out_split2 = a->out_split2;
 }
 
@@ -1680,6 +1741,18 @@
   pl.stats_written = pl.stats_in_kernel || pl.stats_in_reduce;
   pl.epi_rows = k.epi32 < 0 ? (x3 ? 1 : 0) : (k.epi32 == 2 ? 2 : (k.epi32 != 0));
   if (ph && (a->hin * a->win) % 64 != 0) pl.epi_rows = 0;
+  if (a->residual_map != 0) {
+    if (a->residual_map != 1 && a->residual_map != 2) return refuse("dts_conv2d: residual_map %d (0 = none, 1 = nearest-up, 2 = 2x2 mean)", a->residual_map);
+    if (a->residual == nullptr) return refuse("dts_conv2d: residual_map %d without a residual", a->residual_map);
+    if (!f32 && !x3) return refuse("dts_conv2d: residual_map %d needs an f32 output (DTS_F32 / DTS_F16X3), dtype %d", a->residual_map, a->dtype);
+    if (a->out_split2) return refuse("dts_conv2d: residual_map %d with out_split2", a->residual_map);
+    if (ph) return refuse("dts_conv2d: residual_map %d with up = 2 (the phase form)", a->residual_map);
+    if (pl.splits > 1) return refuse("dts_conv2d: residual_map %d with a K split of %d (the reduce pass reads the residual unmapped)", a->residual_map, pl.splits);
+    if ((p.hout | p.wout) & 1) return refuse("dts_conv2d: residual_map %d needs even hout, wout (%d, %d)", a->residual_map, p.hout, p.wout);
+    if ((p.hout * p.wout) % 64 != 0 || !pl.epi_rows)
+      return refuse("dts_conv2d: residual_map %d needs the row-layout f32 epilogue: hout*wout = %d a multiple of 64, epi_rows = %d not 0", a->residual_map,
+                    p.hout * p.wout, pl.epi_rows);
+  }
   if (mt != 0) return pl;
   const bool one_per_cu = (long long)pl.nblk * pl.splits <= 256;
   pl.stages = (one_per_cu && pl.ks_per_split >= 3) ? 3 : 2;
diff --git a/diffusion_tts_amd/csrc/conv_small.hip b/diffusion_tts_amd/csrc/conv_small.hip
--- a/diffusion_tts_amd/csrc/conv_small.hip
+++ b/diffusion_tts_amd/csrc/conv_small.hip
@@ -68,14 +68,17 @@
   }
 }
 
-template <typename T, int NT>
+template <typename T, int NT, bool STATS = false>
 __global__ __launch_bounds__(256) void conv_in3_mfma_kernel(const float* __restrict__ x, const float* __restrict__ w,
                                                              const float* __restrict__ bias, T* __restrict__ out, int nseg, int h,
-                                                             int wd) {
+                                                             int wd, float* __restrict__ stats = nullptr) {
   constexpr int ES = sizeof(T) == 4 ? 4 : 2;
   constexpr int COUT = NT * 16, ROWB = COUT * ES + 16, TG = 4;
   static_assert(NT % TG == 0, "tile groups");
+  static_assert(!STATS || sizeof(T) == 4, "strip statistics are the f32 output's");
   __shared__ __attribute__((aligned(16))) char stage_all[4 * 16 * ROWB];
+  __shared__ float2 part[STATS ? 2 : 1][4][STATS ? COUT : 1];
+  [[maybe_unused]] int trip = 0;
   const int lane = threadIdx.x & 63, wave = threadIdx.x >> 6, p = lane & 15, kq = lane >> 4;
   char* stage = stage_all + wave * 16 * ROWB;
   float a[NT][7];
@@ -136,6 +139,28 @@
     for (int c = lane; c < COUT * ES; c += 64) {
       const int px = c / (COUT * ES / 16), ch = c - px * (COUT * ES / 16);
       *reinterpret_cast<uint4*>(dst + (size_t)c * 16) = *reinterpret_cast<const uint4*>(stage + px * ROWB + ch * 16);
+    }
+    if constexpr (STATS) {
+      float2 (*pb)[COUT] = part[trip & 1];
+      ++trip;
+#pragma unroll
+      for (int ch = lane; ch < COUT; ch += 64) {
+        float s_ = 0.f, q_ = 0.f;
+#pragma unroll
+        for (int px = 0; px < 16; ++px) {
+          const float v = *reinterpret_cast<const float*>(stage + px * ROWB + ch * 4);
+          s_ += v; q_ += v * v;
+        }
+        pb[wave][ch] = make_float2(s_, q_);
+      }
+      __syncthreads();
+      if (threadIdx.x < COUT) {
+        const int ch = threadIdx.x;
+        float2 t = pb[0][ch];
+#pragma unroll
+        for (int k = 1; k < 4; ++k) { t.x += pb[k][ch].x; t.y += pb[k][ch].y; }
+        *reinterpret_cast<float2*>(stats + ((size_t)(seg >> 2) * COUT + ch) * 2) = t;
+      }
     }
   }
 }
@@ -195,9 +220,11 @@
   }
 }
 
-template <typename T>
+template <typename T, bool GN = false>
 __global__ __launch_bounds__(256) void conv_out3_tiled_kernel(const T* __restrict__ x, const float* __restrict__ w, const float* __restrict__ bias,
-                                                               float* __restrict__ out, int h, int wd, int c) {
+                                                               float* __restrict__ out, int h, int wd, int c,
+                                                               const float* __restrict__ coef = nullptr, int silu = 0) {
+  static_assert(!GN || sizeof(T) == 4, "the fused norm reads f32 activations");
   constexpr int EPV = ET<T>::EPV, VPC = 4, CC = VPC * EPV;
   static_assert(CC == VPC * EPV, "chunk = 4 vectors");
   constexpr int PITCH = VPC * 16 + 16;
@@ -208,13 +235,30 @@
   float a0 = 0.f, a1 = 0.f, a2 = 0.f;
   for (int c0 = 0; c0 < c; c0 += CC) {
     __syncthreads();
+    [[maybe_unused]] float A[EPV], B[EPV];
+    if constexpr (GN) {
+      const float* cf = coef + ((size_t)n * c + c0 + (threadIdx.x & (VPC - 1)) * EPV) * 2;
+#pragma unroll
+      for (int e = 0; e < EPV; e += 2) {
+        const float4 q = *reinterpret_cast<const float4*>(cf + e * 2);
+        A[e] = q.x; B[e] = q.y; A[e + 1] = q.z; B[e + 1] = q.w;
+      }
+    }
     for (int i = threadIdx.x; i < 18 * 18 * VPC; i += 256) {
       const int hp = i / VPC, v = i - hp * VPC;
       const int hy = hp / 18, hx = hp - hy * 18;
       const int yy = y0 + hy - 1, xx = x0 + hx - 1;
       uint4 val = make_uint4(0, 0, 0, 0);
-      if ((unsigned)yy < (unsigned)h && (unsigned)xx < (unsigned)wd)
+      if ((unsigned)yy < (unsigned)h && (unsigned)xx < (unsigned)wd) {
         val = *reinterpret_cast<const uint4*>(x + (((size_t)n * h + yy) * wd + xx) * c + c0 + v * EPV);
+        if constexpr (GN) {
+          float f[EPV];
+          unpack16<T>(val, f);
+#pragma unroll
+          for (int e = 0; e < EPV; ++e) { const float y = f[e] * A[e] + B[e]; f[e] = silu ? silu_f(y) : y; }
+          val = pack16<T>(f);
+        }
+      }
       *reinterpret_cast<uint4*>(halo + hp * PITCH + v * 16) = val;
     }
     __syncthreads();
@@ -260,7 +304,7 @@
     long long g = (nseg + 4 * spw - 1) / (4 * spw);
     if (g > 2048) g = 2048;
 #define DTS_IN3_MFMA(TT, NT_)                                                                                                    \
-  hipLaunchKernelGGL((conv_in3_mfma_kernel<TT, NT_>), dim3((int)g), dim3(256), 0, st, x, w, bias, (TT*)out, (int)nseg, h, w_)
+  hipLaunchKernelGGL((conv_in3_mfma_kernel<TT, NT_>), dim3((int)g), dim3(256), 0, st, x, w, bias, (TT*)out, (int)nseg, h, w_, (float*)nullptr)
     if (dtype == DTS_BF16) {
       if (cout == 192) DTS_IN3_MFMA(bf16_t, 12); else if (cout == 128) DTS_IN3_MFMA(bf16_t, 8); else DTS_IN3_MFMA(bf16_t, 4);
     } else if (dtype == DTS_F32) {
@@ -283,6 +327,45 @@
   return DTS_OK;
 }
 
+extern "C" int dts_conv_in3_stats(const float* x, const float* w, const float* bias, float* out, float* stats, int n, int h, int w_, int cout,
+                                  dts_stream s) {
+  DTS_CHECK_ARG(x && w && out && stats, "dts_conv_in3_stats: null pointer");
+  DTS_CHECK_ARG(n > 0 && h > 0 && w_ > 0 && cout > 0, "dts_conv_in3_stats: bad shape (n=%d h=%d w=%d cout=%d)", n, h, w_, cout);
+  const long long nseg = (long long)n * h * (w_ / 16);
+  if (!(w_ % 16 == 0 && ((long long)h * w_) % 64 == 0 && (cout == 192 || cout == 128 || cout == 64) && nseg < (1ll << 31) &&
+        (bias == nullptr || ((uintptr_t)bias & 15) == 0) && ((uintptr_t)stats & 15) == 0)) {
+    dts_set_error("dts_conv_in3_stats: the matrix-core kernel only (w %% 16 == 0, h*w %% 64 == 0, cout 64 / 128 / 192, aligned bias and stats): h=%d w=%d cout=%d",
+                  h, w_, cout);
+    return DTS_ERR_UNSUPPORTED;
+  }
+  long long spw = nseg / 2048;
+  if (spw < 1) spw = 1;
+  if (spw > 8) spw = 8;
+  long long g = (nseg + 4 * spw - 1) / (4 * spw);
+  if (g > 2048) g = 2048;
+  hipStream_t st = to_stream(s);
+#define DTS_IN3_STATS(NT_) \
+  hipLaunchKernelGGL((conv_in3_mfma_kernel<float, NT_, true>), dim3((int)g), dim3(256), 0, st, x, w, bias, out, (int)nseg, h, w_, stats)
+  if (cout == 192) DTS_IN3_STATS(12); else if (cout == 128) DTS_IN3_STATS(8); else DTS_IN3_STATS(4);
+#undef DTS_IN3_STATS
+  DTS_CHECK_LAUNCH("dts_conv_in3_stats");
+  return DTS_OK;
+}
+
+extern "C" int dts_conv_out3_gn(const float* x, const float* coef, int silu, const float* w, const float* bias, float* out, int n, int h,
+                                int w_, int c, dts_stream s) {
+  DTS_CHECK_ARG(x && coef && w && out, "dts_conv_out3_gn: null pointer");
+  DTS_CHECK_ARG(n > 0 && h > 0 && w_ > 0 && c > 0, "dts_conv_out3_gn: bad shape (n=%d h=%d w=%d c=%d)", n, h, w_, c);
+  if (!(h % 16 == 0 && w_ % 16 == 0 && c % 16 == 0 && (long long)n * (h / 16) * (w_ / 16) < (1ll << 31) && ((uintptr_t)coef & 15) == 0)) {
+    dts_set_error("dts_conv_out3_gn: the tiled kernel only (h, w multiples of 16, c of 16, 16-byte aligned coef): h=%d w=%d c=%d", h, w_, c);
+    return DTS_ERR_UNSUPPORTED;
+  }
+  hipLaunchKernelGGL((conv_out3_tiled_kernel<float, true>), dim3((unsigned)(n * (h / 16) * (w_ / 16))), dim3(256), 0, to_stream(s), x, w, bias, out,
+                     h, w_, c, coef, silu);
+  DTS_CHECK_LAUNCH("dts_conv_out3_gn");
+  return DTS_OK;
+}
+
 extern "C" int dts_conv_out3(const void* x, int dtype, const float* w, const float* bias, float* out, int n, int h, int w_, int c,
                              dts_stream s) {
   DTS_CHECK_ARG(x && w && out, "dts_conv_out3: null pointer");
@@ -290,7 +373,8 @@
   hipStream_t st = to_stream(s);
   if (h % 16 == 0 && w_ % 16 == 0 && c % (dtype == DTS_F32 ? 16 : 32) == 0 && (long long)n * (h / 16) * (w_ / 16) < (1ll << 31)) {
     DTS_DISPATCH_DTYPE(dtype, {
-      hipLaunchKernelGGL((conv_out3_tiled_kernel<T>), dim3((unsigned)(n * (h / 16) * (w_ / 16))), dim3(256), 0, st, (const T*)x, w, bias, out, h, w_, c);
+      hipLaunchKernelGGL((conv_out3_tiled_kernel<T>), dim3((unsigned)(n * (h / 16) * (w_ / 16))), dim3(256), 0, st, (const T*)x, w, bias, out, h, w_, c,
+                         (const float*)nullptr, 0);
       DTS_CHECK_LAUNCH("dts_conv_out3");
     });
     return DTS_OK;
diff --git a/diffusion_tts_amd/csrc/dts_common.h b/diffusion_tts_amd/csrc/dts_common.h
--- a/diffusion_tts_amd/csrc/dts_common.h
+++ b/diffusion_tts_amd/csrc/dts_common.h
@@ -144,6 +144,20 @@
 
 __device__ __forceinline__ float silu_f(float x) { return x / (1.0f + __expf(-x)); }
 
+template <typename T> __device__ __forceinline__ void mean2x2_vec(const uint4& v00, const uint4& v01, const uint4& v10, const uint4& v11, float* r) {
+  constexpr int E = 16 / sizeof(T);
+  const uint4 q[4] = {v00, v01, v10, v11};
+#pragma unroll
+  for (int e = 0; e < E; ++e) r[e] = 0.f;
+#pragma unroll
+  for (int k = 0; k < 4; ++k) {
+    float f[E];
+    unpack16<T>(q[k], f);
+#pragma unroll
+    for (int e = 0; e < E; ++e) r[e] += 0.25f * f[e];
+  }
+}
+
 template <typename F> __device__ __forceinline__ F wave_sum(F v) {
 #pragma unroll
   for (int o = 32; o > 0; o >>= 1) v += __shfl_xor(v, o, 64);
diff --git a/diffusion_tts_amd/csrc/groupnorm.hip b/diffusion_tts_amd/csrc/groupnorm.hip
--- a/diffusion_tts_amd/csrc/groupnorm.hip
+++ b/diffusion_tts_amd/csrc/groupnorm.hip
@@ -384,18 +384,10 @@
       o = *reinterpret_cast<const uint4*>(x + (((size_t)n * h + (yo >> 1)) * w + (xo >> 1)) * c + chunk * EPV);
     } else {
       float r[EPV];
-#pragma unroll
-      for (int e = 0; e < EPV; ++e) r[e] = 0.f;
-#pragma unroll
-      for (int dy = 0; dy < 2; ++dy)
-#pragma unroll
-        for (int dx = 0; dx < 2; ++dx) {
-          const uint4 v = *reinterpret_cast<const uint4*>(x + (((size_t)n * h + 2 * yo + dy) * w + 2 * xo + dx) * c + chunk * EPV);
-          float f[EPV];
-          unpack16<T>(v, f);
-#pragma unroll
-          for (int e = 0; e < EPV; ++e) r[e] += 0.25f * f[e];
-        }
+      const T* s0 = x + (((size_t)n * h + 2 * yo) * w + 2 * xo) * c + chunk * EPV;
+      const T* s1 = s0 + (size_t)w * c;
+      mean2x2_vec<T>(*reinterpret_cast<const uint4*>(s0), *reinterpret_cast<const uint4*>(s0 + c), *reinterpret_cast<const uint4*>(s1),
+                     *reinterpret_cast<const uint4*>(s1 + c), r);
       o = pack16<T>(r);
     }
     *reinterpret_cast<uint4*>(out + (((size_t)n * ho + yo) * wo + xo) * c + chunk * EPV) = o;
diff --git a/diffusion_tts_amd/networks.py b/diffusion_tts_amd/networks.py
--- a/diffusion_tts_amd/networks.py
+++ b/diffusion_tts_amd/networks.py
@@ -188,6 +188,7 @@
             coef1 = ops.gn_coefficients(h, G(b.cout), self.eps, P.g1, P.b1, scale_shift=ss if self.adm else None)
         else:
             h = ops.group_norm(h, G(b.cout), self.eps, P.g1, P.b1, scale_shift=ss if self.adm else None, silu=True, split_out=self.x3)
+        rmap = None
         if P.skip_w is not None and skip_src is not None and ops.conv_folds_skip(h, P.w1, (skip_src, P.skip_w, up)):
             sk = None
         elif P.skip_w is not None and skip_src is not None:
@@ -196,13 +197,17 @@
             src1, src2 = (ops.resample2x(x1, up=False), None) if b.down else (x1, x2)
             sk = ops.conv2d(src1, P.skip_w, P.skip_b, x2=src2, up=b.up)
         elif b.up or b.down:
-            sk = ops.resample2x(x1, up=b.up)
+            rmap = 'up' if b.up else 'mean'
+            if x2 is None and not fuse1 and ops.residual_map_enabled(rmap) and ops.conv_maps_residual(h, P.w1, x1, rmap):
+                sk = x1
+            else:
+                sk, rmap = ops.resample2x(x1, up=b.up), None
         else:
             sk = x1
         if sk is None:
             x = ops.conv2d(h, P.w1, P.cb1_skip, skip=(skip_src, P.skip_w, up), out_scale=self.skip_scale, gn_stats=True)
         else:
-            x = ops.conv2d(h, P.w1, P.cb1, residual=sk, out_scale=self.skip_scale, gn_stats=True,
+            x = ops.conv2d(h, P.w1, P.cb1, residual=sk, residual_map=rmap, out_scale=self.skip_scale, gn_stats=True,
                            gn_coef=coef1 if fuse1 else None, gn_silu=True)
         if b.heads:
             n, hh, ww, c = x.shape
@@ -220,7 +225,7 @@
         emb = self._embedding(c_noise, class_labels, n)
         e = ops.cast_from_f32(emb, self.act_dtype)
         aff = ops.conv2d(e.view(1, n, 1, -1), self.aff_w, self.aff_b).view(n, self.aff_total)
-        x = ops.conv_in3(xin, self.conv_in_w, self.conv_in_b, self.enc[0].cout, self.act_dtype)
+        x = ops.conv_in3(xin, self.conv_in_w, self.conv_in_b, self.enc[0].cout, self.act_dtype, gn_stats=ops.in3_stats_enabled())
         skips = [x]
         aux, aux_nchw = xin, True
         for b in self.enc[1:]:
@@ -236,7 +241,11 @@
         for b in self.dec:
             x2 = skips.pop() if x.shape[-1] != b.cin else None
             x = self._block(b, x, x2, aff)
-        h = ops.group_norm(x, self._groups(self.cfin), 1e-5 if self.adm else 1e-6, self.out_g, self.out_b, silu=True)
+        eps = 1e-5 if self.adm else 1e-6
+        if ops.out3_gn_enabled() and ops.conv_out3_fuses_gn(x):
+            coef = ops.gn_coefficients(x, self._groups(self.cfin), eps, self.out_g, self.out_b)
+            return ops.conv_out3_gn(x, coef, self.out_w, self.out_cb, silu=True)
+        h = ops.group_norm(x, self._groups(self.cfin), eps, self.out_g, self.out_b, silu=True)
         return ops.conv_out3(h, self.out_w, self.out_cb)
 
     @torch.no_grad()
diff --git a/diffusion_tts_amd/ops.py b/diffusion_tts_amd/ops.py
--- a/diffusion_tts_amd/ops.py
+++ b/diffusion_tts_amd/ops.py
@@ -243,8 +243,44 @@
     return bool(L.load().dts_conv_folds_skip(C.byref(a)))
 
 
+def residual_map_enabled(mode):
+    return mode in os.environ.get('DTS_RESIDUAL_MAP', 'up,mean').split(',')
+
+
+def out3_gn_enabled():
+    return os.environ.get('DTS_OUT3_GN', '1') != '0'
+
+
+def in3_stats_enabled():
+    return os.environ.get('DTS_IN3_STATS', '1') != '0'
+
+
+RESIDUAL_MAPS = {None: 0, 0: 0, 'up': 1, 1: 1, 'mean': 2, 2: 2}
+
+
+def _residual_shape(n, ho, wo, cout, rmap):
+    return {0: (n, ho, wo, cout), 1: (n, ho // 2, wo // 2, cout), 2: (n, 2 * ho, 2 * wo, cout)}[rmap]
+
+
+def conv_maps_residual(x1, w, residual, residual_map, *, gn_stats=True):
+    rmap = RESIDUAL_MAPS[residual_map]
+    n, hin, win, c1 = x1.shape
+    if rmap == 0 or residual is None or residual.dtype != torch.float32 or (hin | win) & 1 or \
+            tuple(residual.shape) != _residual_shape(n, hin, win, w.shape[0], rmap):
+        return False
+    a = _conv_args(x1, w, None, False)
+    if isinstance(w, X3Weight):
+        a.c1, a.c2, a.dtype = 2 * a.c1, 0, L.DTS_F16X3
+    a.residual, a.residual_map = 16, rmap
+    a.workspace, a.workspace_bytes = 16, CONV_WS_BYTES
+    if gn_stats and (hin * win) % 64 == 0:
+        a.stats_out = 16
+    info = L.ConvPlanInfo()
+    return L.load().dts_conv_plan(C.byref(a), C.byref(info)) == 0 and not info.refused
+
+
 def _conv2d_args(x1, w, bias=None, *, x2=None, bias_nc=None, residual=None, up=False, out_scale=1.0, out=None, gn_stats=False,
-                 timing_events=None, gn_coef=None, gn_silu=True, out_split2=False, skip=None, phases=None):
+                 timing_events=None, gn_coef=None, gn_silu=True, out_split2=False, skip=None, phases=None, residual_map=None):
     n, hin, win, c1 = x1.shape
     c2 = 0 if x2 is None else x2.shape[-1]
     cout, kh, kw, cin = w.shape
@@ -275,8 +311,9 @@
     a.bias = _ptr(bias, 'bias', torch.float32)
     a.bias_nc, a.ld_bias_nc = _rows(bias_nc, 'bias_nc', x1.dtype)
     a.residual = _ptr(residual, 'residual', x1.dtype)
-    if residual is not None and tuple(residual.shape) != (n, ho, wo, cout):
-        raise ValueError(f'conv2d: residual shape {tuple(residual.shape)} != {(n, ho, wo, cout)}')
+    a.residual_map = RESIDUAL_MAPS[residual_map]
+    if residual is not None and tuple(residual.shape) != _residual_shape(n, ho, wo, cout, a.residual_map):
+        raise ValueError(f'conv2d: residual shape {tuple(residual.shape)} != {_residual_shape(n, ho, wo, cout, a.residual_map)} (residual_map={residual_map})')
     a.out = _ptr(out, 'out', torch.float16 if out_split2 else x1.dtype)
     a.n, a.hin, a.win, a.cout, a.ksize = n, hin, win, cout, kh
     a.up, a.out_scale, a.dtype = int(up), float(out_scale), (L.DTS_F16X3 if x3 else dt_code(x1.dtype))
@@ -309,10 +346,10 @@
 
 
 def conv2d(x1, w, bias=None, *, x2=None, bias_nc=None, residual=None, up=False, out_scale=1.0, out=None, gn_stats=False,
-           timing_events=None, gn_coef=None, gn_silu=True, out_split2=False, skip=None, phases=None):
+           timing_events=None, gn_coef=None, gn_silu=True, out_split2=False, skip=None, phases=None, residual_map=None):
     a, out, st, out_split2, _keep = _conv2d_args(x1, w, bias, x2=x2, bias_nc=bias_nc, residual=residual, up=up, out_scale=out_scale, out=out,
                                                  gn_stats=gn_stats, timing_events=timing_events, gn_coef=gn_coef, gn_silu=gn_silu,
-                                                 out_split2=out_split2, skip=skip, phases=phases)
+                                                 out_split2=out_split2, skip=skip, phases=phases, residual_map=residual_map)
     _call('dts_conv2d', C.byref(a))
     if out_split2:
         return SplitQKV(out, (out.shape[0], out.shape[1], out.shape[2], out.shape[3] // 2))
@@ -335,12 +372,38 @@
     return out
 
 
-def conv_in3(x, w, bias, cout, dtype):
+def conv_in3(x, w, bias, cout, dtype, gn_stats=False):
     n, c, h, wd = x.shape
     assert c == 3
     out = torch.empty((n, h, wd, cout), dtype=dtype, device=x.device)
+    if gn_stats and conv_in3_emits_stats(dtype, h, wd, cout, bias):
+        st = torch.empty(((n * h * wd) // 64, cout, 2), dtype=torch.float32, device=x.device)
+        _call('dts_conv_in3_stats', _ptr(x, 'x', torch.float32), _ptr(w, 'w', torch.float32), _ptr(bias, 'bias', torch.float32),
+              _ptr(out), _ptr(st), n, h, wd, cout)
+        out._gn_stats = st
+        return out
     _call('dts_conv_in3', _ptr(x, 'x', torch.float32), _ptr(w, 'w', torch.float32), _ptr(bias, 'bias', torch.float32),
           _ptr(out), dt_code(dtype), n, h, wd, cout)
+    return out
+
+
+def conv_in3_emits_stats(dtype, h, wd, cout, bias=None):
+    return dtype == torch.float32 and wd % 16 == 0 and (h * wd) % 64 == 0 and cout in (64, 128, 192) and \
+        (bias is None or bias.data_ptr() % 16 == 0)
+
+
+def conv_out3_fuses_gn(x):
+    n, h, wd, c = x.shape
+    return x.dtype == torch.float32 and h % 16 == 0 and wd % 16 == 0 and c % 16 == 0
+
+
+def conv_out3_gn(x, coef, w_ohwi, bias, silu=True):
+    n, h, wd, c = x.shape
+    if tuple(coef.shape) != (n, c, 2):
+        raise ValueError(f'conv_out3_gn: coef shape {tuple(coef.shape)} != {(n, c, 2)}')
+    out = torch.empty((n, 3, h, wd), dtype=torch.float32, device=x.device)
+    _call('dts_conv_out3_gn', _ptr(x, 'x', torch.float32), _ptr(coef, 'coef', torch.float32), int(bool(silu)), _ptr(w_ohwi, 'w', torch.float32),
+          _ptr(bias, 'bias', torch.float32), _ptr(out), n, h, wd, c)
     return out
 
 
diff --git a/include/dts.h b/include/dts.h
--- a/include/dts.h
+++ b/include/dts.h
@@ -13,7 +13,7 @@
                  DTS_F16X3 = 3 };
 enum dts_status { DTS_OK = 0, DTS_ERR_ARG = -1, DTS_ERR_LAUNCH = -2, DTS_ERR_UNSUPPORTED = -3 };
 
-#define DTS_ABI_VERSION 120
+#define DTS_ABI_VERSION 121
 int dts_version(void);
 const char* dts_last_error(void);
 int dts_set_tuning(int knob, int value);
@@ -54,6 +54,7 @@
   const void* skip_w;
   float skip_acc_scale;
   int32_t skip_up;
+  int32_t residual_map;
 } dts_conv_args;
 int dts_conv_fuses_gn(const dts_conv_args* a);
 int dts_conv_folds_skip(const dts_conv_args* a);
@@ -79,6 +80,10 @@
                  int n, int h, int w_, int cout, dts_stream s);
 int dts_conv_out3(const void* x, int dtype, const float* w, const float* bias, float* out,
                   int n, int h, int w_, int c, dts_stream s);
+int dts_conv_in3_stats(const float* x, const float* w, const float* bias, float* out, float* stats, int n, int h, int w_, int cout,
+                       dts_stream s);
+int dts_conv_out3_gn(const float* x, const float* coef, int silu, const float* w, const float* bias, float* out,
+                     int n, int h, int w_, int c, dts_stream s);
 
 int64_t dts_gn_ws_floats(int n, int groups);
 int dts_gn_coef(const void* x1, int c1, const void* x2, int c2, int dtype, int n, int hw, int groups, float eps,
```
